# martinruenz/maskfusion

Hardware: AMD Instinct MI355X
Metric: frames/sec (640x480 RGB-D, single background model, ICP + surfel fusion) (higher is better)
Workload: dtype f32; 1 GPU; configs[1]: synthetic 640x480 RGB-D stream (S1: 600 frames, Kinect-like noise), 1 background model per GPU, icpWeight=100 (geometric ICP 4/5/10 iterations) + surfel fusion, empty masks; frames_in_hbm=600, models=1, surfels=429320, parallelism=context-per-gpu x1

## Files before the change

### maskfusion_amd/api.py

```python
from __future__ import annotations

import ctypes as C
import numpy as np

from .lib import load, MFError, Config, ModelInfo, RenderView, MF_N_TIMINGS, TIMING_LABELS, MF_N_PASSES, PASS_LABELS


class Model:

    def __init__(self, owner: "MaskFusion", index: int):
        self._o = owner
        self._i = index

    def info(self) -> ModelInfo:
        out = ModelInfo()
        self._o._chk(self._o._L.mf_model_info(self._o._h, self._i, C.byref(out)))
        return out

    def getID(self) -> int:
        return int(self.info().id)

    def getClassID(self) -> int:
        return int(self.info().class_id)

# ... 219 lines not shown

    def getBackgroundModel(self) -> Model:
        return Model(self, 0)

    def getModels(self):
        n = C.c_int32(0)
        self._chk(self._L.mf_num_models(self._h, C.byref(n)))
        return [Model(self, i) for i in range(n.value)]

    def getCurrPose(self) -> np.ndarray:
        return self.getBackgroundModel().getPose()

    def downloadSegmentation(self) -> np.ndarray:
        out = np.zeros((self.height, self.width), np.uint8)
        self._chk(self._L.mf_download_segmentation(self._h, out.ctypes.data))
        return out

    def exportSegmentation(self, path: str):
        self._chk(self._L.mf_export_segmentation_png(self._h, path.encode()))

    def getLastFillIn(self) -> bool:
        u = C.c_int32(0)
        self._chk(self._L.mf_get_last_fillin(self._h, C.byref(u)))
        return bool(u.value)

    def setParam(self, key: str, value: float):
        self._chk(self._L.mf_set_param(self._h, key.encode(), float(value)))

    def getParam(self, key: str) -> float:
        v = C.c_double(0)
        self._chk(self._L.mf_get_param(self._h, key.encode(), C.byref(v)))
        return v.value

    def setDepthCutoff(self, v): self.setParam("depthCutoff", v)
    def setIcpWeight(self, v): self.setParam("icpWeight", v)
    def setConfidenceThreshold(self, v): self.setParam("confidenceThreshold", v)
    def setOutlierCoefficient(self, v): self.setParam("outlierCoefficient", v)
    def setFastOdom(self, v): self.setParam("fastOdom", int(v))
    def setSo3(self, v): self.setParam("so3", int(v))
    def setFrameToFrameRGB(self, v): self.setParam("frameToFrameRGB", int(v))
    def setRgbOnly(self, v): self.setParam("rgbOnly", int(v))

    def trackStats(self, model: int = 0) -> dict:
        out = np.zeros(8, np.float32)
        self._chk(self._L.mf_get_track_stats(self._h, model, out.ctypes.data))
        keys = ("lastICPError", "lastICPCount", "lastRGBError", "lastRGBCount", "lastSO3Error", "lastSO3Count", "so3Iterations",
                "rejected")
        return dict(zip(keys, out.tolist()))
    def gnIllIterations(self, model: int = 0) -> int:
        n = C.c_int32(0)
        self._chk(self._L.mf_get_gn_condition(self._h, model, C.byref(n)))
        return n.value

    def setPyramid(self, v): self.setParam("pyramid", int(v))
    def setEnableMultipleModels(self, v): self.setParam("enableMultipleModels", int(v))

    def enableTimings(self, on=True):
        self.setParam("timings", 1 if on else 0)

    def timings(self) -> dict:
        t = np.zeros(MF_N_TIMINGS, np.float32)
        self._chk(self._L.mf_get_timings(self._h, t.ctypes.data))
        return dict(zip(TIMING_LABELS, t.tolist()))

    def passTimings(self) -> dict:
        t = np.zeros(MF_N_PASSES, np.float32)
        self._chk(self._L.mf_get_pass_timings(self._h, t.ctypes.data))
        return dict(zip(PASS_LABELS, t.tolist()))

    def stream(self) -> int:
        return int(self._L.mf_get_stream(self._h) or 0)

    def inputStream(self) -> int:
        return int(self._L.mf_get_input_stream(self._h) or 0)

    def defaultRenderView(self, width: int = 1280, height: int = 980, icl: bool = False) -> RenderView:
        v = RenderView()
        self._chk(self._L.mf_default_render_view(self._h, int(width), int(height), int(bool(icl)), C.byref(v)))
        return v

    def sensorRenderView(self) -> RenderView:
        v = RenderView()
        self._chk(self._L.mf_sensor_render_view(self._h, C.byref(v)))
        return v

    @staticmethod
    def defaultPalette() -> np.ndarray:
        L, n = load(), C.c_int32(0)
        if L.mf_default_palette(None, 0, C.byref(n)) != 0:
            raise MFError("mf_default_palette failed")
        out = np.zeros((n.value, 3), np.float32)
        if L.mf_default_palette(out.ctypes.data, n.value, C.byref(n)) != 0:
            raise MFError("mf_default_palette failed")
        return out

    def renderView(self, view: RenderView | None = None, palette=None, depth: bool = False, models: bool = False):
        if view is None:
            view = self.defaultRenderView()
        H, W = int(view.height), int(view.width)
        rgba = np.zeros((max(H, 1), max(W, 1), 4), np.uint8)
        dep = np.zeros((max(H, 1), max(W, 1)), np.float32) if depth else None
        mod = np.zeros((max(H, 1), max(W, 1)), np.int32) if models else None
        if palette is None:
            pal_ptr, n_pal = None, 0
        else:
            pal = np.ascontiguousarray(np.asarray(palette, np.float32).reshape(-1, 3))
            n_pal = len(pal)
            if n_pal == 0:
                pal = np.zeros((1, 3), np.float32)
            pal_ptr = pal.ctypes.data
        self._chk(self._L.mf_render_view(self._h, C.byref(view), pal_ptr, n_pal, rgba.ctypes.data,
                                         dep.ctypes.data if dep is not None else None, mod.ctypes.data if mod is not None else None))
        out = [rgba]
        if depth:
            out.append(dep)
        if models:
            out.append(mod)
        return out[0] if len(out) == 1 else tuple(out)

    def renderViewDevice(self, view: RenderView, d_rgba: int, d_depth: int = 0, d_model: int = 0, palette=None):
        pal_ptr, n_pal, keep = None, 0, None
        if palette is not None:
            keep = np.ascontiguousarray(np.asarray(palette, np.float32).reshape(-1, 3))
            pal_ptr, n_pal = keep.ctypes.data, len(keep)
        self._chk(self._L.mf_render_view_dev(self._h, C.byref(view), pal_ptr, n_pal, d_rgba, d_depth or None, d_model or None))

    def modelCloudNN(self, model: int, points, radius: float, transform=None, confThreshold=None):
        import torch
        from .lib import torch_device
        as_numpy = not isinstance(points, torch.Tensor)
        q = torch.as_tensor(np.ascontiguousarray(points, np.float32)) if as_numpy else points
        if q.dtype != torch.float32 or q.dim() != 2 or q.shape[1] < 3:
            raise MFError("modelCloudNN: points must be (n, >= 3) float32")
        q = q.to(torch_device()).contiguous()
        n = int(q.shape[0])
        dist = torch.empty(max(n, 1), dtype=torch.float32, device=q.device)
        idx = torch.empty(max(n, 1), dtype=torch.int32, device=q.device)
        thr = Model(self, model).getConfidenceThreshold() if confThreshold is None else float(confThreshold)
        T = None if transform is None else np.ascontiguousarray(np.asarray(transform, np.float32).T.reshape(16))
        if q.device.type == "cuda":
            torch.cuda.current_stream(q.device).synchronize()
        self._chk(self._L.mf_model_cloud_nn_dev(self._h, int(model), thr, q.data_ptr() if n else None, int(q.shape[1]), n,
                                                T.ctypes.data if T is not None else None, float(radius), dist.data_ptr(), idx.data_ptr()))
        dist, idx = dist[:n], idx[:n]
        if as_numpy:
            return dist.cpu().numpy(), idx.cpu().numpy()
        return dist, idx

    def debugRead(self, what: str, model: int = 0, count: int | None = None) -> np.ndarray:
        W, H = self.width, self.height
        shapes = {"depthF": ((H, W), np.float32), "pred_vertex": ((H, W, 4), np.float32),
                  "pred_normal": ((H, W, 4), np.float32), "pred_image": ((H, W, 4), np.uint8), "pred_time": ((H, W), np.uint16),
                  "index": ((H, W), np.int32), "index_vc": ((H, W, 4), np.float32), "index_nr": ((H, W, 4), np.float32),
                  "index_ct": ((H, W, 4), np.float32), "index_packed": ((W, H, 2, 4), np.float32), "icp_log": ((19, 32), np.float32), "gn_trace": ((20, 64), np.float64),
                  "icp_prof": ((19, 16), np.uint64), "splat_prof": ((((H + 15) // 16) * ((W + 15) // 16), 8), np.uint64),
                  "edge_map": ((H, W), np.float32),
                  "edge_binary": ((H, W), np.uint8), "projected_ids": ((H, W), np.uint8)}
        for i in range(3):
            shapes.update({f"gray{i}": ((H >> i, W >> i), np.uint8), f"dIdx{i}": ((H >> i, W >> i), np.int16), f"dIdy{i}": ((H >> i, W >> i), np.int16),
                           f"rgb_gate{i}": ((H >> i, W >> i), np.uint8)})
        if count is not None:
            shapes.update({"cand_op": ((count,), np.uint8), "cand_rec": ((count, 12), np.float32),
                           "clean_flags": ((count,), np.uint8), "clean_newconf": ((count,), np.float32)})
        for pre in ("vmap_g", "nmap_g", "vmap", "nmap"):
            for i in range(3):
                shapes[f"{pre}{i}"] = ((3, H >> i, W >> i), np.float32)
        shape, dt = shapes[what]
        out = np.zeros(shape, dt)
        self._chk(self._L.mf_debug_read_model(self._h, model, what.encode(), out.ctypes.data, out.nbytes))
        return out
```

### maskfusion_amd/csrc/mf_context.hip

```cpp
#include "../../include/maskfusion_amd.h"
#include "mf_internal.h"
#include "mf_labels.h"

#include <float.h>
#include <math.h>
#include <algorithm>
#include <cmath>
#include <stdio.h>
#include <string.h>
#include <memory>
#include <chrono>
#include <string>
#include <vector>

using namespace mf;

namespace {

struct SurfelBufferState {
    int cur = 0;
    bool table_valid = false;
    bool sparse = false;
    long phys_ub = -1, runs_ub = -1;
    unsigned clean_seq = 0, mirror_from = 1;
    unsigned gen = 0;

    void reset_empty() { became_dense(0); }
    void became_dense(int live) { cur = live; sparse = false; table_valid = false; phys_ub = runs_ub = -1; mirror_from = clean_seq + 1; gen++; }
    void fresh_table(int live, long n) { became_dense(live); table_valid = true; exact_count(n); }
    void exact_count(long n) { phys_ub = n; runs_ub = (n + kRun - 1) / kRun; }
    void table_built() { table_valid = true; gen++; }
    void cleaned_in_place(long cand_max, long new_runs_max) { sparse = true; table_valid = true; phys_ub += cand_max; runs_ub += new_runs_max; clean_seq++; gen++; }
    void touched() { gen++; }
};

struct ModelState : SurfelBufferState {
    int id = 0, classID = -1;
    bool isStatic = true, allowFillIn = false;
    unsigned age = 0;
    float confThr = 0.f, maxDepth = FLT_MAX;
    Surfels surf[2];
    int cap = 0;
    unsigned long long* h_append = nullptr;
    PoseDev* d_pose = nullptr; FrameDev* d_frame = nullptr;
    float4* d_predV = nullptr; float4* d_predN = nullptr; uchar4* d_predImage = nullptr; uint16_t* d_predTime = nullptr;
    uint8_t* d_predGray = nullptr; uint8_t* d_fillGray = nullptr;
    bool pred_gray_valid = false;
    float* d_vmap_g[3] = {}; float* d_nmap_g[3] = {}; GNState* d_gn = nullptr; float* d_partials[2] = {nullptr, nullptr};
    TrackModelDev* d_track = nullptr;
    int* d_track_rect = nullptr;
    float* d_icp_log = nullptr;
    double* d_gn_trace = nullptr;
    struct ObjScratch {
        unsigned long long* keys = nullptr; int* index = nullptr; float4* ivc = nullptr; float4* inr = nullptr; float4* iclean = nullptr;
        uint8_t* cand_op = nullptr; float4* cand_rec = nullptr; int* upd_first = nullptr; int* cand_best = nullptr;
        int* clean_ctl = nullptr;
        uint8_t* flags = nullptr; float* newconf = nullptr; int* block_counts = nullptr;
    } scr;
    float* d_poselog = nullptr;
    std::vector<int64_t> log_ts;
    PoseDev* h_pose = nullptr; FrameDev* h_frame = nullptr; int* h_count = nullptr;
    TrackModelDev track_host;
    std::vector<void*> allocs;
    ~ModelState() {
        for (void* p : allocs) (void)hipFree(p);
        if (h_pose) (void)hipHostFree(h_pose);
        if (h_frame) (void)hipHostFree(h_frame);
        if (h_count) (void)hipHostFree(h_count);
        if (h_append) (void)hipHostFree(h_append);
    }
};

struct LabelsScratch {
    int P = 0, table_cap = 0;
    uint8_t* ignoreMap = nullptr; uint8_t* tmp_u8 = nullptr;
    int* L = nullptr; int* compId = nullptr; int* area = nullptr; int* lab[2] = {nullptr, nullptr}; int* blockCounts = nullptr;
    int4* bbox = nullptr;
    int* compMask = nullptr; int* compModel = nullptr; int* compToMask = nullptr; int* compFollow = nullptr;
    unsigned* overlap = nullptr; void* tables = nullptr;
    int* d_small = nullptr;
    const PoseDev** d_poses = nullptr;
    int* h_small = nullptr; const PoseDev** h_poses = nullptr; int* h_result = nullptr;
    std::vector<void*> dev, host;
    ~LabelsScratch() {
        for (void* p : dev) (void)hipFree(p);
        for (void* p : host) (void)hipHostFree(p);
    }
    template <typename T> bool dalloc(T** p, size_t n) {
        void* q = nullptr;
        if (hipMalloc(&q, n * sizeof(T)) != hipSuccess) return false;
        if (hipMemset(q, 0, n * sizeof(T)) != hipSuccess) return false;
        dev.push_back(q); *p = reinterpret_cast<T*>(q);
        return true;
    }
    template <typename T> bool halloc(T** p, size_t n) {
        void* q = nullptr;
        if (hipHostMalloc(&q, n * sizeof(T)) != hipSuccess) return false;
        memset(q, 0, n * sizeof(T));
        host.push_back(q); *p = reinterpret_cast<T*>(q);
        return true;
    }
    bool init(int P_) {
        P = P_;
        table_cap = 8 << 20;
        return dalloc(&ignoreMap, (size_t)P) && dalloc(&tmp_u8, (size_t)P) && dalloc(&L, (size_t)P) && dalloc(&compId, (size_t)P) &&
               dalloc(&area, (size_t)P + 1) && dalloc(&bbox, (size_t)P + 1) && dalloc(&lab[0], (size_t)P) && dalloc(&lab[1], (size_t)P) &&
               dalloc(&blockCounts, (size_t)(P + 255) / 256) && dalloc(&compMask, (size_t)table_cap) &&
               dalloc(&compModel, (size_t)table_cap) && dalloc(&compToMask, (size_t)P + 1) && dalloc(&compFollow, (size_t)P + 1) &&
               dalloc(&overlap, (size_t)64 * 256) && dalloc((char**)&tables, labels_gpu_table_bytes()) && dalloc(&d_small, 384) &&
               dalloc(&d_poses, 64) && halloc(&h_small, 384) && halloc(&h_poses, 64) && halloc(&h_result, 4);
    }
    int enqueue(const SegParams& prm, int W, int H, const uint8_t* d_binary, const float* d_depth, const uint8_t* d_mask,
                const int32_t* class_ids, int n_masks, const uint8_t* d_proj, const std::vector<SegModelInfo>& models,
                const std::vector<const PoseDev*>& poses, int nextModelID, bool allowNew, uint8_t* d_full, hipStream_t s) {
        if (models.size() > 64 || n_masks > 256) return MF_EINVAL;
        memset(h_small, 0, 384 * sizeof(int));
        for (int k = 0; k < n_masks; ++k) h_small[k] = class_ids[k];
        for (size_t m = 0; m < models.size(); ++m) { h_small[256 + m] = models[m].id; h_small[320 + m] = models[m].classID; h_poses[m] = poses[m]; }
        if (hipMemcpyAsync(d_small, h_small, 384 * sizeof(int), hipMemcpyHostToDevice, s) != hipSuccess ||
            hipMemcpyAsync(d_poses, h_poses, 64 * sizeof(PoseDev*), hipMemcpyHostToDevice, s) != hipSuccess)
            return MF_EHIP;
        LabelsGpuArgs a;
        a.prm = prm; a.W = W; a.H = H; a.binary = d_binary; a.depth = d_depth; a.mask = d_mask; a.proj = d_proj;
        a.class_ids = d_small; a.nMasks = n_masks; a.model_ids = d_small + 256; a.model_cls = d_small + 320; a.model_poses = d_poses;
        a.nModels = (int)models.size(); a.nextModelID = nextModelID; a.allowNew = allowNew; a.ignoreMap = ignoreMap; a.full = d_full;
        a.tmp_u8 = tmp_u8; a.L = L; a.compId = compId; a.area = area; a.bbox = bbox; a.lab[0] = lab[0]; a.lab[1] = lab[1]; a.blockCounts = blockCounts;
        a.compMask = compMask; a.compModel = compModel; a.table_cap = table_cap; a.compToMask = compToMask; a.compFollow = compFollow;
        a.overlap = overlap; a.tables = tables; a.result_host = h_result;
        launch_labels_gpu(a, s);
        return MF_OK;
    }
};

}

struct RenderScratch;
static void render_free(RenderScratch* r);
struct EvalScratch;
static void eval_free(EvalScratch* e);

struct mf_ctx {
    mf_config cfg;
    int W, H, P;
    Intr K;
    hipStream_t stream = nullptr;
    bool clean_literal = true;
    bool global_tiles = true;
    bool early_bg_fusion = true;
    hipEvent_t ev_labels = nullptr;
    long frame_no = 0;
    long bg_fused_frame = -1;
    bool labels_pending = false;
    int lastF = 0;
    std::string err;
    int host_tick = 1;
    bool map_ready = false;
    bool tracked_once = false;
    bool timings_on = false, icp_prof_on = false;
    bool object_small_grids = true;
    bool object_scatter_splat = true;
#ifndef MF_DEFAULT_LITERAL_FUSION_WEIGHT
#define MF_DEFAULT_LITERAL_FUSION_WEIGHT 1
#endif
    bool weight_literal = MF_DEFAULT_LITERAL_FUSION_WEIGHT != 0;
    bool bbox_limit = true;
    bool batch_objects = true;
    static constexpr int kObjArgSlots = 8;
    ObjPassArgs* d_obj_args[kObjArgSlots] = {}; ObjPassArgs* h_obj_args[kObjArgSlots] = {}; hipEvent_t ev_obj_args[kObjArgSlots] = {};
    unsigned obj_arg_slot = 0;
    bool fused_preprocess = true;
    bool object_stream = true;
    hipStream_t stream_obj = nullptr, obj_s = nullptr;
    hipEvent_t ev_obj_dep = nullptr, ev_obj_done = nullptr;
    bool obj_dep_main = false;
    uint8_t* d_maskT_obj = nullptr;
    bool ftf_rgb = false;
    double host_us[5] = {0, 0, 0, 0, 0}; long host_calls = 0;
    bool host_lockstep = true;
    bool host_wait_upload = true;

    uint8_t* d_rgb = nullptr; float* d_depth = nullptr; uint8_t* d_mask_in = nullptr; uint8_t* d_zero_mask = nullptr;
    bool host_async = true;
    hipStream_t stream_in = nullptr;
    uint8_t* h_in[2] = {nullptr, nullptr};
    uint8_t* d_in_block[2] = {nullptr, nullptr};
    size_t in_off_rgb = 0, in_off_mask = 0, in_bytes = 0;
    uint8_t* d_in_rgb[2] = {}; float* d_in_depth[2] = {}; uint8_t* d_in_mask[2] = {};
    hipEvent_t ev_in_copied[2] = {nullptr, nullptr};
    hipEvent_t ev_in_consumed[2] = {nullptr, nullptr};
    unsigned in_slot = 0;
    uint8_t* d_mask_tex = nullptr;
    float* d_depthF[3] = {nullptr, nullptr, nullptr};
    float* d_vmap[2][3] = {}; float* d_nmap[2][3] = {};
    uint8_t* d_gray[2][3] = {};
    long gray_frame[2] = {-1, -1};
    long deriv_frame = -1;
    int16_t* d_dIdx[3] = {}; int16_t* d_dIdy[3] = {}; uint8_t* d_rgb_gate[3] = {};
    float* d_lastDepth[3] = {}; uint8_t* d_lastImage[3] = {};
    RgbCorr* d_corres = nullptr; float* d_rgb_partials[2] = {nullptr, nullptr}; int2* d_cnt[2] = {nullptr, nullptr};
    So3Result* d_so3 = nullptr; char* d_so3_scratch = nullptr;
    SplatTuning splat_tune;
    int* d_tile_count = nullptr; int* d_tile_entries = nullptr; int tile_entries_cap = 0; int tile_entries_alloc = 0; int splat_tiles = 1;
    float4* d_splat_rec0 = nullptr; float4* d_splat_rec1 = nullptr; uint2* d_splat_bbox = nullptr;
    const uint8_t* cur_rgb = nullptr;
    const float* cur_depth = nullptr;
    bool batch_solve_fused = true;
    int batch_tracking = 1;
    int model_api_packed = 0;
    std::vector<int32_t> mask_classes;
    std::vector<int> trackable;
    struct RetiredLog { int id; std::vector<int64_t> ts; std::vector<float> p; size_t arena_off = 0, n = 0; bool in_arena = false; };
    std::vector<RetiredLog> retired;
    float* d_retired = nullptr; size_t retired_cap = 0, retired_used = 0;
    std::vector<std::unique_ptr<ModelState>> pool;
    unsigned long long* d_keys = nullptr;
    int* d_index = nullptr; float4* d_ivc = nullptr; float4* d_ict = nullptr; float4* d_inr = nullptr;
    float4* d_iclean = nullptr;
    uint8_t* d_maskT = nullptr;
    uint8_t* d_cand_op = nullptr; float4* d_cand_rec = nullptr; int* d_upd_first = nullptr;
    uint8_t* d_flags = nullptr; float* d_newconf = nullptr; int* d_block_counts = nullptr;
    int* d_cand_best = nullptr;
    int* d_clean_ctl = nullptr;
    int* d_clean_list = nullptr; int* d_clean_count = nullptr;
    int* d_decay_stats = nullptr;
    int* d_run_offs = nullptr;
    int* d_vis_list = nullptr; int* d_vis_count = nullptr; int* d_cull_ctl = nullptr; int vis_max_runs = 0;
    struct { const void* model = nullptr; long frame = -1; int cur = -1; unsigned gen = 0; float max_depth = 0.f; int time_delta = 0; } vis_tag;
    int densify_count = 0;
    bool fused_rgb_pyramid = true;
    float2* d_row_z = nullptr;
    bool slab_culling = true;
    int densify_every = 0;
    bool cull_runs = true;
    int big_map_elements = 6000000;
    int in_place_elements = 1000000;
    unsigned long long* d_icp_prof = nullptr;
    unsigned long long* d_splat_prof = nullptr; bool splat_prof_on = false;
    float* d_edge = nullptr; uint8_t* d_bin = nullptr; uint8_t* d_tmp_u8 = nullptr; uint8_t* d_proj_ids = nullptr;
    uint8_t* h_bin = nullptr; uint8_t* h_ids = nullptr; float* h_depth = nullptr; uint8_t* h_mask = nullptr; uint8_t* h_full = nullptr;
    std::vector<uint8_t> ignoreMap;
    std::unique_ptr<LabelsScratch> labels;
    int gpu_labels = 1;
    SegParams seg;
    int nextID = 0, spawnOffset = 0;
    int cap_max = 0;

    std::vector<std::unique_ptr<ModelState>> models;

    hipEvent_t ev[MF_N_TIMINGS + 1] = {};
    hipEvent_t ev_mm[5] = {};
    bool mm_marked = false; float mm_host_wait_ms = 0.f;
    hipEvent_t ev_icp[2] = {nullptr, nullptr};
    bool pass_timings_on = false;
    hipEvent_t ev_pass[MF_N_PASSES][2] = {};
    bool pass_recorded[MF_N_PASSES] = {};
    float pass_ms[MF_N_PASSES] = {};
    hipEvent_t ev_icp_mid = nullptr;
    bool icp_mid_recorded = false;
    float last_ms[MF_N_TIMINGS] = {};
    std::vector<void*> allocs;
    std::vector<void*> host_allocs;
    RenderScratch* render = nullptr;
    EvalScratch* eval = nullptr;
};

#define MF_HIP(ctx, call)                                                                         \
    do {                                                                                          \
        hipError_t e_ = (call);                                                                   \
        if (e_ != hipSuccess) {                                                                   \
            char buf_[512];                                                                       \
            snprintf(buf_, sizeof(buf_), "%s failed: %s (%s:%d)", #call, hipGetErrorString(e_), __FILE__, __LINE__); \
            if (ctx) (ctx)->err = buf_;                                                           \
            return MF_EHIP;                                                                       \
        }                                                                                         \
    } while (0)

template <typename T>
static int dev_alloc(mf_ctx* c, std::vector<void*>& owner, T** p, size_t n, int fill = 0) {
    void* q = nullptr;
    MF_HIP(c, hipMalloc(&q, n * sizeof(T)));
    MF_HIP(c, hipMemsetAsync(q, fill, n * sizeof(T), c->stream));
    owner.push_back(q);
    *p = reinterpret_cast<T*>(q);
    return MF_OK;
}
template <typename T>
static int host_alloc(mf_ctx* c, T** p, size_t n) {
    void* q = nullptr;
    MF_HIP(c, hipHostMalloc(&q, n * sizeof(T)));
    memset(q, 0, n * sizeof(T));
    c->host_allocs.push_back(q);
    *p = reinterpret_cast<T*>(q);
    return MF_OK;
}

extern "C" int mf_default_config(mf_config* cfg, int32_t width, int32_t height, float fx, float fy, float cx, float cy) {
    if (!cfg) return MF_EINVAL;
    memset(cfg, 0, sizeof(*cfg));
    cfg->width = width; cfg->height = height; cfg->fx = fx; cfg->fy = fy; cfg->cx = cx; cfg->cy = cy;
    cfg->device = 0;
    cfg->time_delta = 200; cfg->conf_global = 4.f; cfg->conf_object = 2.f; cfg->depth_cutoff = 3.f;
    cfg->icp_weight = 10.f; cfg->fast_odom = 0; cfg->so3 = 1; cfg->pyramid = 1; cfg->max_depth_processed = 20.f;
    cfg->outlier_coefficient = 0.9f;
    cfg->num_gsurfels = 9437184; cfg->num_osurfels = 1048576;
    cfg->enable_multiple_models = 1;
    cfg->model_spawn_offset = 20; cfg->track_all_models = 1; cfg->max_models = 32;
    cfg->rgb_only = 0;
    cfg->pose_log_capacity = 65536;
    return MF_OK;
}

static __global__ void k_set_weight_literal(PoseDev* p, int literal, PoseDev* host_mirror) {
    if (threadIdx.x != 0 || blockIdx.x != 0) return;
    p->weightLiteral = literal;
    if (host_mirror) host_mirror->weightLiteral = literal;
}
static __global__ void k_pose_identity(PoseDev* p, int weight_literal) {
    if (threadIdx.x != 0 || blockIdx.x != 0) return;
    PoseDev q;
    memset(&q, 0, sizeof(q));
    q.weightLiteral = weight_literal;
    for (int k = 0; k < 9; ++k) q.R[k] = q.Ri[k] = q.lastR[k] = q.initR[k] = (k % 4 == 0) ? 1.f : 0.f;
    q.fusionWeight = 1.f;
    q.alive = 1;
    *p = q;
}
static __global__ void k_frame_init(FrameDev* f, int tick) {
// ... 48 lines not shown
    }
    A(dev_alloc(c, m->allocs, &m->d_pose, 1));
    A(dev_alloc(c, m->allocs, &m->d_frame, 1));
    A(dev_alloc(c, m->allocs, &m->d_predV, P));
    A(dev_alloc(c, m->allocs, &m->d_predN, P));
    A(dev_alloc(c, m->allocs, &m->d_predImage, P));
    A(dev_alloc(c, m->allocs, &m->d_predTime, P));
    A(dev_alloc(c, m->allocs, &m->d_predGray, P));
    if (allowFillIn) A(dev_alloc(c, m->allocs, &m->d_fillGray, P));
    if (c->cfg.pose_log_capacity > 0) A(dev_alloc(c, m->allocs, &m->d_poselog, (size_t)c->cfg.pose_log_capacity * 8));
    for (int i = 0; i < 3; ++i) {
        const size_t lp = (size_t)(c->W >> i) * (c->H >> i);
        A(dev_alloc(c, m->allocs, &m->d_vmap_g[i], lp * 3));
        A(dev_alloc(c, m->allocs, &m->d_nmap_g[i], lp * 3));
    }
    {
        int nbm = icp_batch_max_blocks(c->W, c->H);
        for (int i = 0; i < 3; ++i) nbm = std::max(nbm, std::max(icp_grid_blocks(c->W >> i, c->H >> i), icp_geo_grid_blocks(c->W >> i, c->H >> i)));
        const size_t nbmax = (size_t)nbm;
        for (int b = 0; b < 2; ++b) A(dev_alloc(c, m->allocs, &m->d_partials[b], nbmax * kIcpSlots));
    }
    A(dev_alloc(c, m->allocs, &m->d_gn, 2));
    A(dev_alloc(c, m->allocs, &m->d_track, 1));
    A(dev_alloc(c, m->allocs, &m->d_track_rect, 12));
    A(dev_alloc(c, m->allocs, &m->d_icp_log, (size_t)20 * 32));
    A(dev_alloc(c, m->allocs, &m->d_gn_trace, (size_t)20 * kGnTraceRow));
    if (!allowFillIn && with_scratch) A(ensure_obj_scratch(c, *m));
#undef A
    {
        TrackModelDev t;
        memset(&t, 0, sizeof(t));
        t.predV = m->d_predV; t.predN = m->d_predN; t.pose = m->d_pose; t.frame = m->d_frame;
        for (int i = 0; i < 3; ++i) { t.vm[i] = m->d_vmap_g[i]; t.nm[i] = m->d_nmap_g[i]; }
        t.partials[0] = m->d_partials[0]; t.partials[1] = m->d_partials[1]; t.st = m->d_gn;
        t.log = m->d_icp_log;
        t.trace = m->d_gn_trace;
        t.jump_limit = allowFillIn ? 0.f : 0.2f;
        t.allow_fill = allowFillIn ? 1 : 0;
        t.rect = m->d_track_rect;
        m->track_host = t;
    }
    hipLaunchKernelGGL(k_pose_identity, dim3(1), dim3(64), 0, c->stream, m->d_pose, c->weight_literal ? 1 : 0);
    hipLaunchKernelGGL(k_frame_init, dim3(1), dim3(64), 0, c->stream, m->d_frame, c->host_tick);
    if (hipHostMalloc((void**)&m->h_pose, sizeof(PoseDev)) != hipSuccess || hipHostMalloc((void**)&m->h_frame, sizeof(FrameDev)) != hipSuccess ||
        hipHostMalloc((void**)&m->h_count, sizeof(int)) != hipSuccess || hipHostMalloc((void**)&m->h_append, sizeof(unsigned long long)) != hipSuccess)
        return MF_ENOMEM;
    *m->h_append = 0ull;
    memset(m->h_pose, 0, sizeof(PoseDev));
    for (int k = 0; k < 9; ++k) m->h_pose->R[k] = m->h_pose->Ri[k] = (k % 4 == 0) ? 1.f : 0.f;
    m->h_pose->alive = 1;
    m->h_pose->fusionWeight = 1.f;
    m->h_pose->weightLiteral = c->weight_literal ? 1 : 0;
    memset(m->h_frame, 0, sizeof(FrameDev));
    m->h_frame->tick = c->host_tick;
    *m->h_count = 0;
    m->track_host.pose_host = m->h_pose;
    MF_HIP(c, hipMemcpyAsync(m->d_track, &m->track_host, sizeof(TrackModelDev), hipMemcpyHostToDevice, c->stream));
    {
        int armed[12];
        for (int q = 0; q < 12; ++q) armed[q] = (q & 2) ? (int)0x80000000 : 0x7FFFFFFF;
        MF_HIP(c, hipMemcpyAsync(m->d_track_rect, armed, sizeof(armed), hipMemcpyHostToDevice, c->stream));
    }
    MF_HIP(c, hipStreamSynchronize(c->stream));
    out = std::move(m);
    return MF_OK;
}

extern "C" int mf_create(const mf_config* cfg, mf_ctx** out) {
    if (!cfg || !out) return MF_EINVAL;
    *out = nullptr;
    if (cfg->width <= 0 || cfg->height <= 0 || (cfg->width % 8) || (cfg->height % 8)) return MF_EINVAL;
    int ndev = 0;
    if (hipGetDeviceCount(&ndev) != hipSuccess || ndev <= 0 || cfg->device >= ndev) return MF_ENODEV;
    mf_ctx* c = new mf_ctx();
    c->cfg = *cfg;
    if (c->cfg.model_spawn_offset <= 0) c->cfg.model_spawn_offset = 20;
    if (c->cfg.max_models <= 0) c->cfg.max_models = 32;
    c->W = cfg->width; c->H = cfg->height; c->P = c->W * c->H;
    c->K = Intr{cfg->fx, cfg->fy, cfg->cx, cfg->cy};
    auto fail = [&](int code) { mf_destroy(c); return code; };
    if (hipSetDevice(cfg->device) != hipSuccess) return fail(MF_ENODEV);
    if (hipStreamCreateWithFlags(&c->stream, hipStreamNonBlocking) != hipSuccess) return fail(MF_ENODEV);
    const int W = c->W, H = c->H, P = c->P;
    const int cap_bg = surfel_capacity(cfg->num_gsurfels), cap_obj = surfel_capacity(cfg->num_osurfels);
    if (cap_bg <= 0 || cap_obj <= 0) return fail(MF_EINVAL);
    c->cap_max = cap_bg > cap_obj ? cap_bg : cap_obj;
    int rc = MF_OK;
#define A(call) do { rc = (call); if (rc != MF_OK) return fail(rc); } while (0)
    auto up256 = [](size_t v) { return (v + 255) & ~(size_t)255; };
    c->in_off_rgb = up256((size_t)P * sizeof(float));
    c->in_off_mask = up256(c->in_off_rgb + (size_t)P * 3);
    c->in_bytes = up256(c->in_off_mask + (size_t)P);
    for (int i = 0; i < 2; ++i) {
        A(dev_alloc(c, c->allocs, &c->d_in_block[i], c->in_bytes));
        c->d_in_depth[i] = reinterpret_cast<float*>(c->d_in_block[i]);
        c->d_in_rgb[i] = c->d_in_block[i] + c->in_off_rgb;
        c->d_in_mask[i] = c->d_in_block[i] + c->in_off_mask;
    }
    c->d_rgb = c->d_in_rgb[0]; c->d_depth = c->d_in_depth[0]; c->d_mask_in = c->d_in_mask[0];
    for (int i = 0; i < 2; ++i) {
        A(host_alloc(c, &c->h_in[i], c->in_bytes));
        if (hipEventCreateWithFlags(&c->ev_in_copied[i], hipEventDisableTiming) != hipSuccess ||
            hipEventCreateWithFlags(&c->ev_in_consumed[i], hipEventDisableTiming) != hipSuccess) return fail(MF_EHIP);
    }
    if (hipStreamCreateWithFlags(&c->stream_in, hipStreamNonBlocking) != hipSuccess) return fail(MF_EHIP);
    if (hipStreamCreateWithFlags(&c->stream_obj, hipStreamNonBlocking) != hipSuccess) return fail(MF_EHIP);
    if (hipEventCreateWithFlags(&c->ev_obj_dep, hipEventDisableTiming) != hipSuccess ||
        hipEventCreateWithFlags(&c->ev_obj_done, hipEventDisableTiming) != hipSuccess) return fail(MF_EHIP);
    c->obj_s = c->stream;
    A(dev_alloc(c, c->allocs, &c->d_zero_mask, (size_t)P));
    A(dev_alloc(c, c->allocs, &c->d_mask_tex, (size_t)P));
    for (int b = 0; b < 3; ++b) A(dev_alloc(c, c->allocs, &c->d_depthF[b], (size_t)P));
    for (int i = 0; i < 3; ++i) {
        const size_t lp = (size_t)(W >> i) * (H >> i);
        for (int set = 0; set < 2; ++set) {
            A(dev_alloc(c, c->allocs, &c->d_vmap[set][i], lp * 3));
            A(dev_alloc(c, c->allocs, &c->d_nmap[set][i], lp * 3));
        }
    }
    for (int i = 0; i < 3; ++i) {
        const size_t lp = (size_t)(W >> i) * (H >> i);
        for (int set = 0; set < 2; ++set) A(dev_alloc(c, c->allocs, &c->d_gray[set][i], lp));
        A(dev_alloc(c, c->allocs, &c->d_dIdx[i], lp));
        A(dev_alloc(c, c->allocs, &c->d_dIdy[i], lp));
        A(dev_alloc(c, c->allocs, &c->d_rgb_gate[i], lp));
        A(dev_alloc(c, c->allocs, &c->d_lastDepth[i], lp));
        A(dev_alloc(c, c->allocs, &c->d_lastImage[i], lp));
    }
    A(dev_alloc(c, c->allocs, &c->d_corres, (size_t)P));
    for (int b = 0; b < 2; ++b) {
        A(dev_alloc(c, c->allocs, &c->d_rgb_partials[b], (size_t)icp_grid_blocks(W, H) * kIcpSlots));
        A(dev_alloc(c, c->allocs, &c->d_cnt[b], (size_t)icp_grid_blocks(W, H)));
    }
    A(dev_alloc(c, c->allocs, &c->d_so3, 1));
    A(dev_alloc(c, c->allocs, &c->d_so3_scratch, so3_scratch_bytes(W >> 2, H >> 2)));
    {
        const size_t nt = splat_tiles_scratch_ints(W, H);
        const size_t maxcap = (size_t)std::max(surfel_capacity(cfg->num_gsurfels), surfel_capacity(cfg->num_osurfels));
        A(dev_alloc(c, c->allocs, &c->d_tile_count, nt));
        c->tile_entries_cap = (int)std::min<size_t>(std::max<size_t>(4 * maxcap, (size_t)16 * P), (size_t)1 << 30);
        c->tile_entries_alloc = c->tile_entries_cap;
        A(dev_alloc(c, c->allocs, &c->d_tile_entries, (size_t)c->tile_entries_cap));
        A(dev_alloc(c, c->allocs, &c->d_splat_rec0, maxcap));
        A(dev_alloc(c, c->allocs, &c->d_splat_rec1, maxcap));
        A(dev_alloc(c, c->allocs, &c->d_splat_bbox, maxcap));
    }
    A(dev_alloc(c, c->allocs, &c->d_keys, (size_t)P, 0xFF));
    A(dev_alloc(c, c->allocs, &c->d_index, (size_t)P));
    A(dev_alloc(c, c->allocs, &c->d_ivc, (size_t)P));
    A(dev_alloc(c, c->allocs, &c->d_ict, (size_t)P));
    A(dev_alloc(c, c->allocs, &c->d_iclean, (size_t)P * 2));
    A(dev_alloc(c, c->allocs, &c->d_maskT, (size_t)P));
    A(dev_alloc(c, c->allocs, &c->d_maskT_obj, (size_t)P));
    A(dev_alloc(c, c->allocs, &c->d_inr, (size_t)P));
    A(dev_alloc(c, c->allocs, &c->d_cand_op, (size_t)P));
    A(dev_alloc(c, c->allocs, &c->d_cand_rec, (size_t)P * 3));
    A(dev_alloc(c, c->allocs, &c->d_upd_first, (size_t)c->cap_max));
    A(dev_alloc(c, c->allocs, &c->d_flags, (size_t)c->cap_max + P));
    A(dev_alloc(c, c->allocs, &c->d_newconf, (size_t)c->cap_max + P));
    A(dev_alloc(c, c->allocs, &c->d_block_counts, (size_t)kCompactBlocks));
    A(dev_alloc(c, c->allocs, &c->d_cand_best, (size_t)P));
    A(dev_alloc(c, c->allocs, &c->d_clean_ctl, (size_t)kCleanCtlInts));
    A(dev_alloc(c, c->allocs, &c->d_row_z, (size_t)(c->H + (c->H >> 1) + (c->H >> 2))));
    c->vis_max_runs = (int)run_table_runs((long)c->cap_max, (long)P);
    A(dev_alloc(c, c->allocs, &c->d_vis_list, (size_t)c->vis_max_runs));
    A(dev_alloc(c, c->allocs, &c->d_clean_list, (size_t)c->vis_max_runs));
    A(dev_alloc(c, c->allocs, &c->d_clean_count, 1));
    A(dev_alloc(c, c->allocs, &c->d_run_offs, (size_t)c->vis_max_runs + 1));
    A(dev_alloc(c, c->allocs, &c->d_decay_stats, (size_t)kDecayStats + 3));
    launch_arm_decay_stats(c->d_decay_stats, c->stream);
    A(dev_alloc(c, c->allocs, &c->d_vis_count, 1));
    A(dev_alloc(c, c->allocs, &c->d_cull_ctl, 2));
    A(dev_alloc(c, c->allocs, &c->d_icp_prof, (size_t)20 * 16));
    A(dev_alloc(c, c->allocs, &c->d_edge, (size_t)P));
    A(dev_alloc(c, c->allocs, &c->d_bin, (size_t)P));
    A(dev_alloc(c, c->allocs, &c->d_tmp_u8, (size_t)P));
    A(dev_alloc(c, c->allocs, &c->d_proj_ids, (size_t)P));
    A(host_alloc(c, &c->h_bin, (size_t)P));
    A(host_alloc(c, &c->h_ids, (size_t)P));
    A(host_alloc(c, &c->h_depth, (size_t)P));
    A(host_alloc(c, &c->h_mask, (size_t)P));
    A(host_alloc(c, &c->h_full, (size_t)P));
    launch_fill_int(c->d_upd_first, kNoUpdate, c->cap_max, c->stream);
    std::unique_ptr<ModelState> bg;
    A(create_model(c, c->nextID++, cfg->conf_global, true, cap_bg, bg));
    c->models.push_back(std::move(bg));
#undef A
    c->ignoreMap.assign(P, 0);
    c->labels.reset(new LabelsScratch());
    if (!c->labels->init(P)) return fail(MF_ENOMEM);
    for (int i = 0; i <= MF_N_TIMINGS; ++i)
        if (hipEventCreate(&c->ev[i]) != hipSuccess) return fail(MF_EHIP);
    for (int i = 0; i < 2; ++i)
        if (hipEventCreate(&c->ev_icp[i]) != hipSuccess) return fail(MF_EHIP);
    for (int i = 0; i < 5; ++i)
        if (hipEventCreate(&c->ev_mm[i]) != hipSuccess) return fail(MF_EHIP);
    if (hipEventCreate(&c->ev_icp_mid) != hipSuccess) return fail(MF_EHIP);
    for (int i = 0; i < mf_ctx::kObjArgSlots; ++i) {
        if (hipMalloc((void**)&c->d_obj_args[i], sizeof(ObjPassArgs) * 64) != hipSuccess ||
            hipHostMalloc((void**)&c->h_obj_args[i], sizeof(ObjPassArgs) * 64) != hipSuccess ||
            hipEventCreateWithFlags(&c->ev_obj_args[i], hipEventDisableTiming) != hipSuccess)
            return fail(MF_ENOMEM);
    }
    if (hipStreamSynchronize(c->stream) != hipSuccess) return fail(MF_EHIP);
    *out = c;
    return MF_OK;
}

extern "C" void mf_destroy(mf_ctx* c) {
    if (!c) return;
    if (c->stream) (void)hipStreamSynchronize(c->stream);
    c->models.clear();
    if (c->render) render_free(c->render);
    if (c->eval) eval_free(c->eval);
    for (void* p : c->allocs) (void)hipFree(p);
    if (c->d_splat_prof) (void)hipFree(c->d_splat_prof);
    for (void* p : c->host_allocs) (void)hipHostFree(p);
    for (int i = 0; i <= MF_N_TIMINGS; ++i)
        if (c->ev[i]) (void)hipEventDestroy(c->ev[i]);
    for (int i = 0; i < 2; ++i) {
        if (c->ev_icp[i]) (void)hipEventDestroy(c->ev_icp[i]);
        for (int q = 0; q < MF_N_PASSES; ++q) if (c->ev_pass[q][i]) (void)hipEventDestroy(c->ev_pass[q][i]);
    }
    if (c->ev_icp_mid) (void)hipEventDestroy(c->ev_icp_mid);
    for (int i = 0; i < 5; ++i)
        if (c->ev_mm[i]) (void)hipEventDestroy(c->ev_mm[i]);
    if (c->ev_labels) (void)hipEventDestroy(c->ev_labels);
    for (int i = 0; i < 2; ++i) {
        if (c->ev_in_copied[i]) (void)hipEventDestroy(c->ev_in_copied[i]);
        if (c->ev_in_consumed[i]) (void)hipEventDestroy(c->ev_in_consumed[i]);
    }
    if (c->stream_in) { (void)hipStreamSynchronize(c->stream_in); (void)hipStreamDestroy(c->stream_in); }
    if (c->stream_obj) { (void)hipStreamSynchronize(c->stream_obj); (void)hipStreamDestroy(c->stream_obj); }
    if (c->ev_obj_dep) (void)hipEventDestroy(c->ev_obj_dep);
    if (c->ev_obj_done) (void)hipEventDestroy(c->ev_obj_done);
    for (int i = 0; i < mf_ctx::kObjArgSlots; ++i) {
        if (c->d_obj_args[i]) (void)hipFree(c->d_obj_args[i]);
        if (c->h_obj_args[i]) (void)hipHostFree(c->h_obj_args[i]);
        if (c->ev_obj_args[i]) (void)hipEventDestroy(c->ev_obj_args[i]);
    }
    if (c->stream) (void)hipStreamDestroy(c->stream);
    delete c;
}

extern "C" const char* mf_last_error(const mf_ctx* c) { return c ? c->err.c_str() : "null context"; }

#include "mf_frame.inl"

extern "C" int mf_preallocate_models(mf_ctx* c, uint32_t count) {
    if (!c) return MF_EINVAL;
    for (uint32_t i = 0; i < count; ++i) {
        std::unique_ptr<ModelState> m;
        int rc = create_model(c, -1, c->cfg.conf_object, false, surfel_capacity(c->cfg.num_osurfels), m, c->batch_objects);
        if (rc != MF_OK) return rc;
        c->pool.push_back(std::move(m));
    }
    return check_launch(c);
}

static __global__ void k_set_tick(FrameDev* f, int tick, FrameDev* host_mirror) {
    if (threadIdx.x != 0 || blockIdx.x != 0) return;
    f->tick = tick;
    if (host_mirror) *host_mirror = *f;
}
extern "C" int mf_set_tick(mf_ctx* c, int32_t tick) {
    if (!c || tick < 1) return MF_EINVAL;
    if (!c->map_ready && tick != 1) { c->err = "setTick before the first frame would skip the map initialisation"; return MF_ESTATE; }
    c->host_tick = tick;
    for (auto& m : c->models) hipLaunchKernelGGL(k_set_tick, dim3(1), dim3(64), 0, c->stream, m->d_frame, tick, m->h_frame);
    return check_launch(c);
}

#include "mf_model_api.inl"

extern "C" int mf_get_tick(mf_ctx* c, int32_t* tick) {
    if (!c || !tick) return MF_EINVAL;
    *tick = c->host_tick;
    return MF_OK;
}
extern "C" int mf_num_models(mf_ctx* c, int32_t* n) {
    if (!c || !n) return MF_EINVAL;
    *n = (int32_t)c->models.size();
    return MF_OK;
}
static ModelState* model_at(mf_ctx* c, int32_t i) {
    if (!c || i < 0 || i >= (int32_t)c->models.size()) return nullptr;
    return c->models[i].get();
}
extern "C" int mf_get_model_ids(mf_ctx* c, int32_t* ids, int32_t capacity, int32_t* n) {
    if (!c || !ids || !n || capacity < (int32_t)c->models.size()) return MF_EINVAL;
    for (size_t i = 0; i < c->models.size(); ++i) ids[i] = c->models[i]->id;
    *n = (int32_t)c->models.size();
    return MF_OK;
}
extern "C" int mf_get_pose(mf_ctx* c, int32_t model, float* out) {
    ModelState* m = model_at(c, model);
    if (!m || !out) return MF_EINVAL;
    int rc = mf_sync(c);
    if (rc != MF_OK) return rc;
    const PoseDev& p = *m->h_pose;
    for (int r = 0; r < 3; ++r) {
        for (int col = 0; col < 3; ++col) out[col * 4 + r] = p.R[r * 3 + col];
        out[12 + r] = p.t[r];
        out[r * 4 + 3] = 0.f;
    }
    out[15] = 1.f;
// ... 188 lines not shown
    for (int y = 0; y < H; ++y) {
        raw.push_back(0);
        raw.insert(raw.end(), img + (size_t)y * W, img + (size_t)(y + 1) * W);
    }
    std::vector<uint8_t> z = {0x78, 0x01};
    uint32_t a = 1, b = 0;
    for (uint8_t v : raw) { a = (a + v) % 65521u; b = (b + a) % 65521u; }
    for (size_t off = 0; off < raw.size(); off += 65535) {
        const size_t n = std::min<size_t>(65535, raw.size() - off);
        z.push_back(off + n == raw.size() ? 1 : 0);
        z.push_back((uint8_t)(n & 255)); z.push_back((uint8_t)(n >> 8));
        z.push_back((uint8_t)(~n & 255)); z.push_back((uint8_t)((~n >> 8) & 255));
        z.insert(z.end(), raw.begin() + off, raw.begin() + off + n);
    }
    const uint32_t adler = (b << 16) | a;
    for (int k = 3; k >= 0; --k) z.push_back((uint8_t)(adler >> (8 * k)));
    std::vector<uint8_t> f = {0x89, 'P', 'N', 'G', 0x0D, 0x0A, 0x1A, 0x0A};
    std::vector<uint8_t> hdr;
    for (uint32_t v : {(uint32_t)W, (uint32_t)H}) for (int k = 3; k >= 0; --k) hdr.push_back((uint8_t)(v >> (8 * k)));
    hdr.insert(hdr.end(), {8, 0, 0, 0, 0});
    png_chunk(f, "IHDR", hdr);
    png_chunk(f, "IDAT", z);
    png_chunk(f, "IEND", {});
    FILE* fp = fopen(path, "wb");
    if (!fp) return MF_EINVAL;
    const bool ok = fwrite(f.data(), 1, f.size(), fp) == f.size();
    fclose(fp);
    return ok ? MF_OK : MF_EINVAL;
}
extern "C" int mf_export_segmentation_png(mf_ctx* c, const char* path) {
    if (!c || !path) return MF_EINVAL;
    std::vector<uint8_t> img((size_t)c->P);
    int rc = mf_download_segmentation(c, img.data());
    if (rc != MF_OK) return rc;
    for (auto& v : img) v = v > 254 ? 0 : v;
    rc = mf_write_png_gray8(path, img.data(), c->W, c->H);
    if (rc != MF_OK) c->err = std::string("cannot write ") + path;
    return rc;
}

extern "C" int mf_download_map(mf_ctx* c, int32_t model, float* out, uint32_t max_count, uint32_t* count) {
    ModelState* ms = model_at(c, model);
    if (!ms || !out || !count) return MF_EINVAL;
    require_dense(c, *ms);
    int rc = mf_sync(c);
    if (rc != MF_OK) return rc;
    const uint32_t n = (uint32_t)*ms->h_count;
    *count = n;
    const uint32_t m = n < max_count ? n : max_count;
    if (m == 0) return MF_OK;
    std::vector<float4> a(m), b(m), d(m);
    const Surfels& s = ms->surf[ms->cur];
    MF_HIP(c, hipMemcpy(a.data(), s.pc, m * sizeof(float4), hipMemcpyDeviceToHost));
    MF_HIP(c, hipMemcpy(b.data(), s.ct, m * sizeof(float4), hipMemcpyDeviceToHost));
    MF_HIP(c, hipMemcpy(d.data(), s.nr, m * sizeof(float4), hipMemcpyDeviceToHost));
    for (uint32_t i = 0; i < m; ++i) {
        memcpy(out + (size_t)i * 12, &a[i], 16);
        memcpy(out + (size_t)i * 12 + 4, &b[i], 16);
        memcpy(out + (size_t)i * 12 + 8, &d[i], 16);
    }
    return MF_OK;
}

struct ParamRef { const char* key; int kind; size_t off; };
static const ParamRef kParams[] = {
    {"depthCutoff", 0, offsetof(mf_config, depth_cutoff)},
    {"icpWeight", 0, offsetof(mf_config, icp_weight)},
    {"outlierCoefficient", 0, offsetof(mf_config, outlier_coefficient)},
    {"maxDepthProcessed", 0, offsetof(mf_config, max_depth_processed)},
    {"fastOdom", 1, offsetof(mf_config, fast_odom)},
    {"so3", 1, offsetof(mf_config, so3)},
    {"rgbOnly", 1, offsetof(mf_config, rgb_only)},
    {"pyramid", 1, offsetof(mf_config, pyramid)},
    {"timeDelta", 1, offsetof(mf_config, time_delta)},
    {"enableMultipleModels", 1, offsetof(mf_config, enable_multiple_models)},
    {"trackAllModels", 1, offsetof(mf_config, track_all_models)},
    {"modelSpawnOffset", 1, offsetof(mf_config, model_spawn_offset)},
};
struct SegRef { const char* key; int kind; size_t off; };
static const SegRef kSegParams[] = {
    {"mfThreshold", 0, offsetof(SegParams, threshold)},
    {"mfWeightDistance", 0, offsetof(SegParams, weightDistance)},
    {"mfWeightConvexity", 0, offsetof(SegParams, weightConvexity)},
    {"mfMorphEdgeIterations", 1, offsetof(SegParams, morphEdgeIterations)},
    {"mfMorphEdgeRadius", 1, offsetof(SegParams, morphEdgeRadius)},
    {"mfMorphMaskIterations", 1, offsetof(SegParams, morphMaskIterations)},
    {"mfMorphMaskRadius", 1, offsetof(SegParams, morphMaskRadius)},
    {"newModelMinRelativeSize", 0, offsetof(SegParams, minRelSizeNew)},
    {"newModelMaxRelativeSize", 0, offsetof(SegParams, maxRelSizeNew)},
};

extern "C" int mf_set_param(mf_ctx* c, const char* key, double value) {
    if (!c || !key) return MF_EINVAL;
    if (!strcmp(key, "hostProfileReset")) { for (double& v : c->host_us) v = 0; c->host_calls = 0; return MF_OK; }
    if (!strcmp(key, "timings")) { c->timings_on = value != 0; return MF_OK; }
    if (!strcmp(key, "passTimings")) {
        c->pass_timings_on = value != 0;
        for (int q = 0; q < MF_N_PASSES; ++q) { c->pass_recorded[q] = false; c->pass_ms[q] = 0.f; }
        return MF_OK;
    }
    if (!strcmp(key, "icpProfile")) { c->icp_prof_on = value != 0; return MF_OK; }
    if (!strcmp(key, "hostInputAsync")) {
        if (hipStreamSynchronize(c->stream) != hipSuccess || hipStreamSynchronize(c->stream_in) != hipSuccess) return MF_EHIP;
        c->host_async = value != 0; return MF_OK;
    }
    if (!strcmp(key, "hostLockstep")) { c->host_lockstep = value != 0; return MF_OK; }
    if (!strcmp(key, "hostWaitUpload")) { c->host_wait_upload = value != 0; return MF_OK; }
    if (!strcmp(key, "splatProfile")) {
        if (value != 0 && !c->d_splat_prof) {
            if (hipMalloc(&c->d_splat_prof, splat_tiles_scratch_ints(c->W, c->H) * 8 * sizeof(unsigned long long)) != hipSuccess) return MF_ENOMEM;
        }
        c->splat_prof_on = value != 0;
        return MF_OK;
    }
    if (!strcmp(key, "gpuLabels")) { c->gpu_labels = value != 0; return MF_OK; }
    if (!strcmp(key, "splatTiles")) { c->splat_tiles = value != 0; return MF_OK; }
    if (!strcmp(key, "splatTileEntries")) {
        const long long v = (long long)value;
        if (v < 1 || v > c->tile_entries_alloc) return MF_EINVAL;
        c->tile_entries_cap = (int)v;
        return MF_OK;
    }
    if (!strcmp(key, "batchTracking")) { c->batch_tracking = value != 0; return MF_OK; }
    if (!strcmp(key, "frameToFrameRGB")) { c->ftf_rgb = value != 0; return MF_OK; }
    if (!strcmp(key, "batchSolveInPixelPass")) { c->batch_solve_fused = value != 0; return MF_OK; }
    if (!strcmp(key, "fusedPreprocessLaunch")) { c->fused_preprocess = value != 0; return MF_OK; }
    if (!strcmp(key, "objectStream")) { c->object_stream = value != 0; return MF_OK; }
    if (!strcmp(key, "batchObjectPasses")) { c->batch_objects = value != 0; return MF_OK; }
    if (!strcmp(key, "objectBoundingBoxLimit")) { c->bbox_limit = value != 0; return MF_OK; }
    if (!strcmp(key, "literalFusionWeight")) {
        c->weight_literal = value != 0;
        for (auto& m : c->models) hipLaunchKernelGGL(k_set_weight_literal, dim3(1), dim3(64), 0, c->stream, m->d_pose, c->weight_literal ? 1 : 0, m->h_pose);
        for (auto& m : c->pool) hipLaunchKernelGGL(k_set_weight_literal, dim3(1), dim3(64), 0, c->stream, m->d_pose, c->weight_literal ? 1 : 0, m->h_pose);
        return check_launch(c);
    }
    if (!strcmp(key, "objectSmallGrids")) { c->object_small_grids = value != 0; return MF_OK; }
    if (!strcmp(key, "objectScatterSplat")) { c->object_scatter_splat = value != 0; return MF_OK; }
    if (!strcmp(key, "globalTiles")) { c->global_tiles = value != 0; return MF_OK; }
    if (!strcmp(key, "cullRuns")) { c->cull_runs = value != 0; c->vis_tag.model = nullptr; return MF_OK; }
    if (!strcmp(key, "densifyEvery")) { c->densify_every = (int)value; return MF_OK; }
    if (!strcmp(key, "slabCulling")) { c->slab_culling = value != 0; return MF_OK; }
    if (!strcmp(key, "bigMapElements")) { c->big_map_elements = (int)value; c->vis_tag.model = nullptr; return MF_OK; }
    if (!strcmp(key, "fusedRgbPyramid")) { c->fused_rgb_pyramid = value != 0; return MF_OK; }
    if (!strcmp(key, "inPlaceElements")) { c->in_place_elements = (int)value; return MF_OK; }
    if (!strcmp(key, "rebuildRunTable")) {
        ModelState& bg = *c->models[0];
        require_dense(c, bg);
        MF_HIP(c, hipStreamSynchronize(c->stream));
        launch_run_table(bg.surf[bg.cur], bg.d_frame, c->stream);
        bg.fresh_table(bg.cur, (long)*bg.h_count);
        c->vis_tag.model = nullptr;
        return check_launch(c);
    }
    if (!strcmp(key, "cleanLiteralWindow")) { c->clean_literal = value != 0; return MF_OK; }
    if (!strcmp(key, "earlyBackgroundFusion")) { c->early_bg_fusion = value != 0; return MF_OK; }
    if (!strcmp(key, "modelApiPackedIndex")) { c->model_api_packed = value != 0; return MF_OK; }
    if (!strcmp(key, "tileHeight")) { c->splat_tune.tile_h = (int)value; return MF_OK; }
    if (!strcmp(key, "tileThreads")) { c->splat_tune.tile_threads = (int)value; return MF_OK; }
    if (!strcmp(key, "spriteLanes")) { c->splat_tune.sprite_lanes = (int)value; return MF_OK; }
    if (!strcmp(key, "confidenceThreshold")) { c->cfg.conf_global = (float)value; c->models[0]->confThr = (float)value; return MF_OK; }
    for (const ParamRef& p : kParams)
        if (!strcmp(key, p.key)) {
            char* base = reinterpret_cast<char*>(&c->cfg);
            if (p.kind == 0) *reinterpret_cast<float*>(base + p.off) = (float)value;
            else *reinterpret_cast<int32_t*>(base + p.off) = (int32_t)value;
            return MF_OK;
        }
    for (const SegRef& p : kSegParams)
        if (!strcmp(key, p.key)) {
            char* base = reinterpret_cast<char*>(&c->seg);
            if (p.kind == 0) *reinterpret_cast<float*>(base + p.off) = (float)value;
            else *reinterpret_cast<int*>(base + p.off) = (int)value;
            return MF_OK;
        }
    c->err = std::string("unknown parameter: ") + key;
    return MF_EINVAL;
}
extern "C" int mf_get_param(mf_ctx* c, const char* key, double* value) {
    if (!c || !key || !value) return MF_EINVAL;
    if (!strcmp(key, "confidenceThreshold")) { *value = c->models[0]->confThr; return MF_OK; }
    if (!strcmp(key, "splatTileEntries")) { *value = c->tile_entries_cap; return MF_OK; }
    if (!strcmp(key, "cullRuns")) { *value = c->cull_runs ? 1 : 0; return MF_OK; }
    if (!strcmp(key, "densifyCount")) { *value = (float)c->densify_count; return MF_OK; }
    if (!strcmp(key, "unstampedRuns")) {
        MF_HIP(c, hipStreamSynchronize(c->stream));
        ModelState& bg = *c->models[0];
        FrameDev f; MF_HIP(c, hipMemcpy(&f, bg.d_frame, sizeof(FrameDev), hipMemcpyDeviceToHost));
        const size_t cap_runs = run_table_runs((long)bg.cap, (long)c->P);
        const size_t runs = bg.table_valid ? std::min((size_t)std::max(f.runs, 0), cap_runs) : 0;
        std::vector<int4> box(kBoxStride * runs);
        if (runs) MF_HIP(c, hipMemcpy(box.data(), bg.surf[bg.cur].box, box.size() * sizeof(int4), hipMemcpyDeviceToHost));
        int v = 0;
        for (size_t r = 0; r < runs; ++r) v += (box[kBoxStride * r + 2].x > 0 && box[kBoxStride * r + 2].z != 0) ? 1 : 0;
        *value = v;
        return MF_OK;
    }
    if (!strcmp(key, "visibleRuns") || !strcmp(key, "backgroundRuns") || !strcmp(key, "cleanRuns")) {
        MF_HIP(c, hipStreamSynchronize(c->stream));
        int v = 0;
        if (!strcmp(key, "visibleRuns")) MF_HIP(c, hipMemcpy(&v, c->d_vis_count, sizeof(int), hipMemcpyDeviceToHost));
        else if (!strcmp(key, "cleanRuns")) MF_HIP(c, hipMemcpy(&v, c->d_clean_count, sizeof(int), hipMemcpyDeviceToHost));
        else { FrameDev f; MF_HIP(c, hipMemcpy(&f, c->models[0]->d_frame, sizeof(FrameDev), hipMemcpyDeviceToHost)); v = f.runs; }
        *value = v;
        return MF_OK;
    }
    if (!strcmp(key, "hostStageUs")) { *value = c->host_calls ? c->host_us[0] / c->host_calls : 0; return MF_OK; }
    if (!strcmp(key, "hostUploadUs")) { *value = c->host_calls ? c->host_us[1] / c->host_calls : 0; return MF_OK; }
    if (!strcmp(key, "hostEnqueueUs")) { *value = c->host_calls ? c->host_us[2] / c->host_calls : 0; return MF_OK; }
    if (!strcmp(key, "hostCallUs")) { *value = c->host_calls ? c->host_us[3] / c->host_calls : 0; return MF_OK; }
    if (!strcmp(key, "hostWaitUs")) { *value = c->host_calls ? c->host_us[4] / c->host_calls : 0; return MF_OK; }
    if (!strcmp(key, "frameToFrameRGB")) { *value = c->ftf_rgb ? 1 : 0; return MF_OK; }
    if (!strcmp(key, "objectBoundingBoxLimit")) { *value = c->bbox_limit ? 1 : 0; return MF_OK; }
    for (const ParamRef& p : kParams)
        if (!strcmp(key, p.key)) {
            const char* base = reinterpret_cast<const char*>(&c->cfg);
            *value = p.kind == 0 ? (double)*reinterpret_cast<const float*>(base + p.off) : (double)*reinterpret_cast<const int32_t*>(base + p.off);
            return MF_OK;
        }
    for (const SegRef& p : kSegParams)
        if (!strcmp(key, p.key)) {
            const char* base = reinterpret_cast<const char*>(&c->seg);
            *value = p.kind == 0 ? (double)*reinterpret_cast<const float*>(base + p.off) : (double)*reinterpret_cast<const int*>(base + p.off);
            return MF_OK;
        }
    return MF_EINVAL;
}

extern "C" int mf_get_timings(mf_ctx* c, float* ms) {
    if (!c || !ms) return MF_EINVAL;
    int rc = mf_sync(c);
    if (rc != MF_OK) return rc;
    memcpy(ms, c->last_ms, sizeof(c->last_ms));
    return MF_OK;
}
extern "C" int mf_get_pass_timings(mf_ctx* c, float* ms) {
    if (!c || !ms) return MF_EINVAL;
    int rc = mf_sync(c);
    if (rc != MF_OK) return rc;
    memcpy(ms, c->pass_ms, sizeof(c->pass_ms));
    return MF_OK;
}
extern "C" void* mf_get_stream(mf_ctx* c) { return c ? (void*)c->stream : nullptr; }
extern "C" void* mf_get_input_stream(mf_ctx* c) { return c ? (void*)c->stream : nullptr; }

static int debug_read_impl(mf_ctx* c, ModelState& mdl, const char* what, void* out, uint64_t out_bytes) {
    int rc = mf_sync(c);
    if (rc != MF_OK) return rc;
    const void* src = nullptr;
    size_t bytes = 0;
    bool variable = false;
    const size_t P = (size_t)c->P;
    std::string w(what);
    auto lvl = [&](const std::string& pre, float* const arr[3]) -> bool {
        for (int i = 0; i < 3; ++i)
            if (w == pre + std::to_string(i)) {
                src = arr[i]; bytes = (size_t)(c->W >> i) * (c->H >> i) * 3 * sizeof(float);
                return true;
            }
        return false;
    };
    const int lastSet = (int)((c->frame_no + 1) & 1);
    auto img = [&](const std::string& pre, const void* const arr[3], size_t elem) -> bool {
        for (int i = 0; i < 3; ++i)
            if (w == pre + std::to_string(i)) {
                src = arr[i]; bytes = (size_t)(c->W >> i) * (c->H >> i) * elem;
                return true;
            }
        return false;
    };
    const void* const gray3[3] = {c->d_gray[lastSet][0], c->d_gray[lastSet][1], c->d_gray[lastSet][2]};
    const void* const dx3[3] = {c->d_dIdx[0], c->d_dIdx[1], c->d_dIdx[2]}, * const dy3[3] = {c->d_dIdy[0], c->d_dIdy[1], c->d_dIdy[2]};
    const void* const gate3[3] = {c->d_rgb_gate[0], c->d_rgb_gate[1], c->d_rgb_gate[2]};
    if (w == "depthF") { src = c->d_depthF[c->lastF]; bytes = P * 4; }
    else if (img("gray", gray3, 1) || img("dIdx", dx3, 2) || img("dIdy", dy3, 2) || img("rgb_gate", gate3, 1)) {}
    else if (lvl("vmap_g", mdl.d_vmap_g) || lvl("nmap_g", mdl.d_nmap_g) || lvl("vmap", c->d_vmap[lastSet]) || lvl("nmap", c->d_nmap[lastSet])) {}
    else if (w == "pred_vertex") { src = mdl.d_predV; bytes = P * 16; }
    else if (w == "pred_normal") { src = mdl.d_predN; bytes = P * 16; }
    else if (w == "pred_image") { src = mdl.d_predImage; bytes = P * 4; }
    else if (w == "pred_time") { src = mdl.d_predTime; bytes = P * 2; }
    else if (w == "index") { src = c->d_index; bytes = P * 4; }
    else if (w == "index_vc") { src = c->d_ivc; bytes = P * 16; }
    else if (w == "index_nr") { src = c->d_inr; bytes = P * 16; }
    else if (w == "index_ct") { src = c->d_ict; bytes = P * 16; }
    else if (w == "index_packed") { src = c->d_iclean; bytes = P * 32; }
    else if (w == "cand_op") { src = c->d_cand_op; bytes = P; variable = true; }
    else if (w == "cand_rec") { src = c->d_cand_rec; bytes = P * 48; variable = true; }
    else if (w == "clean_flags") { src = c->d_flags; bytes = (size_t)c->cap_max + P; variable = true; }
    else if (w == "clean_newconf") { src = c->d_newconf; bytes = ((size_t)c->cap_max + P) * 4; variable = true; }
    else if (w == "icp_log") { src = mdl.d_icp_log; bytes = 19 * 32 * 4; }
    else if (w == "gn_trace") { src = mdl.d_gn_trace; bytes = 20 * kGnTraceRow * 8; }
    else if (w == "icp_prof") { src = c->d_icp_prof; bytes = 19 * 16 * 8; }
    else if (w == "splat_prof") {
        if (!c->d_splat_prof) { c->err = "splat_prof: switch splatProfile on first"; return MF_ESTATE; }
        src = c->d_splat_prof; bytes = splat_tiles_scratch_ints(c->W, c->H) * 8 * 8;
    }
    else if (w == "edge_map") { src = c->d_edge; bytes = P * 4; }
    else if (w == "edge_binary") { src = c->d_bin; bytes = P; }
    else if (w == "projected_ids") { src = c->d_proj_ids; bytes = P; }
    else { c->err = "unknown debug tap: " + w; return MF_EINVAL; }
    if (variable) bytes = out_bytes < bytes ? (size_t)out_bytes : bytes;
    if (out_bytes < bytes) { c->err = "debug_read: buffer too small"; return MF_EINVAL; }
    MF_HIP(c, hipMemcpy(out, src, bytes, hipMemcpyDeviceToHost));
    return MF_OK;
}
extern "C" int mf_debug_read(mf_ctx* c, const char* what, void* out, uint64_t out_bytes) {
    if (!c || !what || !out) return MF_EINVAL;
    return debug_read_impl(c, *c->models[0], what, out, out_bytes);
}
extern "C" int mf_debug_read_model(mf_ctx* c, int32_t model, const char* what, void* out, uint64_t out_bytes) {
    ModelState* m = model_at(c, model);
    if (!m || !what || !out) return MF_EINVAL;
    return debug_read_impl(c, *m, what, out, out_bytes);
}

#include "mf_ktest.inl"
#include "mf_render.inl"
#include "mf_eval.inl"
```

### maskfusion_amd/csrc/mf_internal.h

```cpp
#pragma once

#include <hip/hip_runtime.h>
#include <stdint.h>

namespace mf {

constexpr int kLevels = 3;
constexpr int kIcpSlots = 32;
constexpr int kCompactBlocks = 2048;
constexpr unsigned long long kEmptyKey = 0xFFFFFFFFFFFFFFFFull;
constexpr int kNoUpdate = 0x7FFFFFFF;

struct Intr {
    float fx, fy, cx, cy;
};

struct PoseDev {
    float R[9], t[3];
    float Ri[9], ti[3];
    float lastR[9], lastT[3];
    float fusionWeight;
    float lastICPError, lastICPCount;
    float initR[9], initT[3];
    float incT[3];
// ... 30 lines not shown
    int runs;
    int cover;
    int useFillIn;
    int pad[3];
    int bbox[6], bbox_acc[6];
    int bbox_tmp[6];
    int phys;
    int first;
    int runsNext;
    int first_run;
    unsigned long long done_cover;
};

constexpr int kBBoxEmptyMin = 100000, kBBoxEmptyMax = -100000;
constexpr int kBBoxNotRun = 0x7FFFFFFF;
#define MF_FRAME_BBOX_RESET(f) do { for (int q_ = 0; q_ < 3; ++q_) { (f)->bbox[q_] = (f)->bbox_acc[q_] = (f)->bbox_tmp[q_] = mf::kBBoxEmptyMin; \
                                                                     (f)->bbox[3 + q_] = (f)->bbox_acc[3 + q_] = (f)->bbox_tmp[3 + q_] = mf::kBBoxEmptyMax; } \
                                    (f)->bbox_acc[0] = mf::kBBoxNotRun; } while (0)
#define MF_FRAME_BBOX_ADVANCE(f) do { if ((f)->bbox_acc[0] != mf::kBBoxNotRun) for (int q_ = 0; q_ < 6; ++q_) (f)->bbox[q_] = (f)->bbox_acc[q_]; \
                                      (f)->bbox_acc[0] = mf::kBBoxNotRun; } while (0)

struct Surfels {
    float4* pc;
    float4* ct;
    float4* nr;
    int cap;
    int4* box;
};
constexpr int kRun = 512;
constexpr int kBoxStride = 3;
__host__ __device__ inline int run_start(const int4* box, int r) { return box[kBoxStride * r + 1].w; }
__host__ __device__ inline int run_len(const int4* box, int r) { return box[kBoxStride * r + 2].x; }
struct VisList { const int* list; const int* count; };
constexpr int kBoxEmptyMin = 0x7FFFFFFF, kBoxEmptyMax = (int)0x80000000;

struct TrackModelDev {
    const float4* predV; const float4* predN;
    PoseDev* pose; PoseDev* pose_host; const FrameDev* frame;
    float* vm[3]; float* nm[3];
    float* partials[2]; GNState* st;
    float* log;
    double* trace;
    float jump_limit;
    int allow_fill;
    int* rect;
};
constexpr int kMaxTrackBatch = 32;
constexpr int kGnTraceRow = 64;
struct TrackBatch { const TrackModelDev* m[kMaxTrackBatch]; int n; };

void launch_bilateral_model_pyramid(const float* depth, float* depthF, const float4* predV, const float4* predN, const float* fillDepth,
                                    const FrameDev* frame, const PoseDev* pose, float* const vmaps[3], float* const nmaps[3], int W, int H, Intr k,
                                    hipStream_t s);
void launch_bilateral(const float* depth, float* out, int W, int H, hipStream_t s);
void launch_pyrdown_f(const float* src, float* dst, int sw, int sh, hipStream_t s);
void launch_vmap_nmap(const float* depth, float* vmap, float* nmap, int W, int H, Intr k, float cutoff, hipStream_t s);
void launch_frame_pyramid(const float* depth, float* const vmap[3], float* const nmap[3], int W, int H, Intr k, float cutoff,
                          hipStream_t s);

void launch_model_pyramid(const float4* predV, const float4* predN, const float* fillDepth, const FrameDev* frame,
                          const PoseDev* pose, const float* R9t3_host_or_null, float* const vmaps[3],
                          float* const nmaps[3], int W, int H, Intr k, hipStream_t s);
struct IcpLaunch {
    const float* vmap_curr; const float* nmap_curr; const float* vmap_prev; const float* nmap_prev;
    int W, H; Intr k;
    float distThres, angleThres;
    const float* partials_in; int nblocks_in;
    float* partials_out;
    const GNState* state_in; GNState* state_out;
    float* log_out;
    double* trace = nullptr; int it = 0;
    unsigned long long* prof_out = nullptr;
    const PoseDev* pose_in = nullptr;
    const So3Result* so3_in = nullptr;
};
int icp_grid_blocks(int W, int H);
int icp_geo_grid_blocks(int W, int H);
void launch_icp_iteration(const IcpLaunch& a, hipStream_t s);
int icp_batch_max_blocks(int W, int H);
int icp_batch_blocks(int W, int H, int n_models);
void launch_model_pyramid_batch(const TrackBatch& b, const float* fillDepth, int W, int H, Intr k, hipStream_t s);
void launch_bilateral_model_pyramid_batch(const float* depth, float* depthF, const TrackBatch& b, const float* fillDepth, int W, int H, Intr k,
                                          hipStream_t s);
void launch_icp_batch_solve(const TrackBatch& b, int it, int nb_in, const So3Result* so3_or_null, hipStream_t s);
void launch_icp_batch_pixels(const TrackBatch& b, int it, int level, const float* vmap_curr, const float* nmap_curr, int W, int H, Intr k,
                             float distThres, float angleThres, hipStream_t s, const float2* row_z = nullptr, bool fused = false, int nb_in = 0,
                             const So3Result* so3_or_null = nullptr);
void launch_row_zrange(const float* const vmap[3], int W, int H, float2* out, hipStream_t s);
void launch_icp_batch_finalize(const TrackBatch& b, int n_it, int nb_in, const So3Result* so3_or_null, hipStream_t s);
void launch_icp_finalize(const float* partials_in, int nblocks_in, const GNState* state_in, PoseDev* pose,
                         PoseDev* host_mirror, float* log_out, float jump_limit, const So3Result* so3, hipStream_t s,
                         double* trace = nullptr, int n_it = 0);
void launch_icp_step_standalone(const float* Rcurr, const float* tcurr, const float* vc, const float* nc,
                                const float* Rpi, const float* tprev, Intr k, const float* vp, const float* np,
                                float distThres, float angleThres, int W, int H, float* partials, GNState* st2,
                                float* out32, hipStream_t s);

struct RgbCorr { int16_t u0, v0; float diff; };

struct RgbLevel {
    const int16_t* dIdx; const int16_t* dIdy;
    const float* lastDepth; const float* nextDepth;
    const uint8_t* lastImage; const uint8_t* nextImage;
    int W, H;
    float minScale;
    float maxDepthDelta;
    const uint8_t* gate;
};

void launch_intensity(const uint8_t* img, int channels, uint8_t* dst, int n, hipStream_t s);
void launch_pyrdown_u8(const uint8_t* src, uint8_t* dst, int sw, int sh, hipStream_t s);
void launch_derivative(const uint8_t* src, int16_t* dx, int16_t* dy, int W, int H, float minScale, uint8_t* gate , hipStream_t s);
struct SmallJob { int kind; const void* src; void* dst; void* dst2; uint8_t* gate; int W, H; float minScale; };
struct SmallJobs { SmallJob j[3]; int n; };
void launch_small_jobs(const SmallJobs& a, hipStream_t s);
bool launch_rgb_pyramid(const uint8_t* rgb, int W, int H, uint8_t* const gray[3], int16_t* const dIdx[3], int16_t* const dIdy[3], uint8_t* const gate[3],
                        const float minScale[3], bool derivatives, hipStream_t s);
void launch_rgbd_last_l0(const float4* predV, const float* fillDepth, const uint8_t* predGray, const uint8_t* fillGray,
                         const FrameDev* frame, float* depth0, uint8_t* image0, int n, hipStream_t s, int frameToFrameRGB = 0);
size_t so3_scratch_bytes(int W2, int H2);
int launch_so3_prealign(const uint8_t* lastImage2, const uint8_t* nextImage2, int W2, int H2, Intr k2, So3Result* out, void* scratch,
                        hipStream_t s);
void launch_rgb_residual_only(const RgbLevel& L, const float* krk_kt, RgbCorr* corres, int* sums, hipStream_t s);
void launch_rgb_step_only(const RgbLevel& L, const RgbCorr* corres, float sigma, Intr k, float sobelScale, double* out32, hipStream_t s);
struct RgbdLaunch {
    IcpLaunch icp;
    RgbLevel L;
    RgbCorr* corres;
    const float* rgb_partials_in; float* rgb_partials_out;
    const int2* cnt_in; int2* cnt_out;
    float icpWeight; int icpOn; int rgbOnly; float sobelScale;
    int level, prev_level;
    const So3Result* so3_in;
};
void launch_rgbd_iteration(const RgbdLaunch& l, hipStream_t s);
void launch_rgbd_finalize(const float* icp_partials, const float* rgb_partials, const int2* cnt, int nb, float icpWeight, int icpOn,
                          int rgbOnly, int rgbOn, int prev_level, const GNState* st_in, const So3Result* so3, PoseDev* pose,
                          PoseDev* host_mirror, float* log_out, float jump_limit, hipStream_t s);

void launch_init_surfels(const uint8_t* rgb, const float* depthRaw, const float* depthF, int W, int H, Intr k,
                         float maxDepth, const FrameDev* frame, float4* rec , uint8_t* flags, hipStream_t s);
constexpr int kSurfelGridBlocks = 2048;
void launch_index_scatter(Surfels src, const FrameDev* frame, const PoseDev* pose, int W, int H, Intr k,
                          float maxDepth, int timeDelta, unsigned long long* keys, bool transposed , hipStream_t s,
                          int blocks = kSurfelGridBlocks, const VisList* vis = nullptr);
void launch_run_table(Surfels s, FrameDev* frame, hipStream_t st, bool refresh = false);
size_t run_table_runs(long capacity, long pixels);
size_t run_table_entries(long capacity, long pixels);
void launch_cull(Surfels s, const FrameDev* frame, const PoseDev* pose, int W, int H, Intr k, float maxDepth, int timeDelta, int* list, int* count,
                 int* ctl, int max_runs, hipStream_t st);
void launch_index_resolve(Surfels src, const FrameDev* frame, const PoseDev* pose, unsigned long long* keys, int W, int H, int* index,
                          float4* vc, float4* nr, float4* ct , float4* packed ,
                          const float* depthF, const uint8_t* mask, uint8_t* maskT ,
                          bool keys_transposed , hipStream_t s, int* decay_stats = nullptr, int maskID = 0);
void launch_fuse_data(const uint8_t* rgb, const float* depthRaw, const float* depthF, const uint8_t* mask,
                      int maskID, const FrameDev* frame, const PoseDev* pose, float weightMultiplier, float maxDepth,
                      int W, int H, Intr k, const int* index, const float4* vc, const float4* nr, uint8_t* cand_op,
                      float4* cand_rec, int* upd_first, int* cand_best, hipStream_t s, int bboxLimit = 1);
void launch_fuse_update(Surfels s, const FrameDev* frame, int* upd_first, const uint8_t* cand_op, const int* cand_best, const float4* cand_rec,
                        int W, int H, hipStream_t st);
void launch_fuse_update_copy(Surfels src, Surfels dst, const FrameDev* frame, int* upd_first, const float4* cand_rec, const PoseDev* pose,
                             int W, int H, Intr k, float maxDepth, int timeDelta, unsigned long long* keys_or_null, bool transposed,
                             hipStream_t s, int blocks = kSurfelGridBlocks);
struct CleanIn {
    FrameDev* frame; const PoseDev* pose; int W, H; Intr k; int timeDelta; float confThreshold, outlierCoeff; int maskID;
    const int* index; const float4* vc; const float4* ct;
    const float4* packed; const uint8_t* maskT;
    const float* depthF; const uint8_t* mask;
    const uint8_t* cand_op; const float4* cand_rec;
    uint8_t* flags; float* newconf; int* block_counts;
    int* host_count;
    unsigned long long* host_append; unsigned seq;
    bool transposed;
    bool literalWindow;
};
constexpr int kAppendSeqBits = 20, kAppendRunBits = 18, kAppendPhysBits = 26;
__host__ __device__ inline unsigned long long append_mirror(unsigned seq, int runs, int phys) {
    return ((unsigned long long)(seq & ((1u << kAppendSeqBits) - 1u)) << (kAppendRunBits + kAppendPhysBits)) | ((unsigned long long)(unsigned)runs << kAppendPhysBits) |
           (unsigned long long)(unsigned)phys;
}
int compact_blocks_for(long elements);
void launch_clean_small(const CleanIn& in, Surfels src, Surfels dst, hipStream_t s, int blocks = kCompactBlocks);
constexpr int kCleanGridMax = 2048;
constexpr int kCleanCtlInts = 8;
int clean_runs_grid(long elements);
void launch_clean_runs(const CleanIn& in, Surfels buf, const VisList* runs, int* ctl, int blocks, hipStream_t s);
void launch_clean_append(const CleanIn& in, Surfels buf, hipStream_t s);
constexpr int kDecayStats = 9;
void launch_arm_decay_stats(int* stats , hipStream_t st);
void launch_cull_clean(Surfels s, const FrameDev* frame, const PoseDev* pose, int W, int H, Intr k, int timeDelta, float confThreshold, int* decay_stats,
                       int* list, int* count, int* ctl, int max_runs, hipStream_t st);
void launch_densify(Surfels src, Surfels dst, FrameDev* frame, int* offs, int* host_count, hipStream_t st);
void launch_run_offsets(Surfels s, const FrameDev* frame, int* offs, int* total, hipStream_t st);
void launch_compact_records(const float4* rec, const uint8_t* flags, int n, Surfels dst, FrameDev* frame,
                            int* block_counts, int* host_count_mirror, hipStream_t s);
void launch_splat_scatter(Surfels src, const FrameDev* frame, const PoseDev* pose, int W, int H, Intr k,
                          float maxDepth, float confThreshold, int timeDelta, unsigned long long* keys,
                          hipStream_t s, int blocks = kSurfelGridBlocks);
void launch_splat_resolve(Surfels src, const PoseDev* pose, unsigned long long* keys, int W, int H, Intr k,
                          float4* predV, float4* predN, uchar4* predImage, uint16_t* predTime, FrameDev* frame,
                          const uint8_t* rgb , uint8_t* predGray , uint8_t* fillGray ,
                          hipStream_t s, int fillPassthrough = 0 );
size_t splat_tiles_scratch_ints(int W, int H);
struct SplatTuning { int sprite_lanes = 4, tile_threads = 512, tile_h = 24; };
struct FrameAdvance { FrameDev* host_mirror; const PoseDev* bg_pose; float* log_slot; };
int launch_splat_tiled(Surfels src, FrameDev* frame, const PoseDev* pose, int W, int H, Intr k, float maxDepth, float confThreshold,
                       int timeDelta, int* tile_count, int* entries , int entries_cap,
                       float4* rec0 , float4* rec1 , void* bbox , float4* predV, float4* predN,
                       uchar4* predImage, uint16_t* predTime, const uint8_t* rgb, uint8_t* predGray, uint8_t* fillGray, hipStream_t s,
                       const FrameAdvance* advance = nullptr, int fillPassthrough = 0, unsigned long long* prof = nullptr ,
                       SplatTuning tune = SplatTuning(), const VisList* vis = nullptr);
struct ObjPassArgs {
    Surfels a, b;
    FrameDev* frame; PoseDev* pose;
    int maskID; float confThreshold, fuseMaxDepth, weightMultiplier;
    unsigned long long* keys; int* index; float4* ivc; float4* inr; float4* iclean;
    uint8_t* cand_op; float4* cand_rec; int* upd_first; int* cand_best; int* clean_ctl; int* host_count;
    unsigned long long* host_append; unsigned clean_seq;
    uint8_t* flags; float* newconf; int* block_counts;
    float4* predV; float4* predN; uchar4* predImage; uint16_t* predTime; uint8_t* predGray;
    FrameDev* host_frame; float* log_slot;
    unsigned global_payload;
};
struct ObjBatch {
    const ObjPassArgs* m; int n;
    int W, H; Intr k; float maxDepthProcessed, globalMaxDepth; int timeDelta; float outlierCoeff; int cleanLiteral, bboxLimit;
    int denseSprites;
    int updateCopy;
    int cleanSmall;
    const uint8_t* rgb; const float* depthRaw; const float* depthF; const uint8_t* mask; const PoseDev* bg_pose;
    uint8_t* maskT;
    unsigned long long* global_keys;
};
void launch_obj_global_scatter(const ObjBatch& b, int blocks, hipStream_t s);
void launch_obj_fuse_clean(const ObjBatch& b, int blocks, int clean_blocks, hipStream_t s, int compact_blocks = kCompactBlocks);
void launch_obj_predict_advance(const ObjBatch& b, int blocks, hipStream_t s);
void launch_fill_keys(unsigned long long* keys, int n, hipStream_t s);
void launch_fill_int(int* p, int v, int n, hipStream_t s);
void launch_edge_map(const float* vmap, const float* nmap, float* out, int W, int H, float wD, float wC, hipStream_t s);
void launch_edge_binary(const float* edge, uint8_t* out, uint8_t* tmp, int W, int H, float threshold, int radius,
                        int iterations, hipStream_t s);
void launch_global_scatter(Surfels src, const FrameDev* frame, const PoseDev* pose, int W, int H, Intr k, float maxDepth,
                           float confThreshold, int timeDelta, int order, int id, unsigned long long* keys, hipStream_t s,
                           int blocks = kSurfelGridBlocks);
void launch_global_resolve(unsigned long long* keys, uint8_t* ids, int P, hipStream_t s);
int gn_solve_standalone(const double* sys29, const double* resultRt16, const float* Rprev9, const float* tprev3, double* x_serial, double* x_wave,
                        double* resultRt_out, float* Rcurr9, float* tcurr3, float* stats2, hipStream_t s);
int launch_global_tiled(Surfels src, FrameDev* frame, const PoseDev* pose, int W, int H, Intr k, float maxDepth, float confThreshold,
                        int timeDelta, int order, int id, int* tile_count, int* entries, int entries_cap, float4* rec0, float4* rec1, void* bbox,
                        unsigned long long* keys, hipStream_t s, SplatTuning tune = SplatTuning(), const VisList* vis = nullptr);
void launch_spawn_pose(PoseDev* obj, const PoseDev* bg, FrameDev* objFrame, const FrameDev* bgFrame, PoseDev* host_mirror,
                       hipStream_t s);
void launch_static_pose(PoseDev* obj, const PoseDev* bg, PoseDev* host_mirror, hipStream_t s);
void launch_override_pose(PoseDev* pose, const float* in_pose16_colmajor, int mode, PoseDev* host_mirror, hipStream_t s);
void launch_model_state(const PoseDev* pose, const FrameDev* frame, float* out16, hipStream_t s);

constexpr int kMaxRenderModels = 256;
struct RenderModel {
    Surfels s; const FrameDev* frame; const PoseDev* pose;
    unsigned base;
    int max_runs;
    float thr; int class_id, color_type, index, is_background;
    float M[12];
};
struct RenderView { float Vi[12]; };
struct RenderArgs {
    RenderModel* models; int n_models;
    int W, H; Intr k; float near_z, far_z;
    int drawUnstable, drawPoints, drawWindow, timeDelta;
    const FrameDev* tick_frame;
    const float* palette; int n_palette;
    uchar4 clear;
    int* work; int* work_count;
    int tilesX, tilesY, tile_cap;
    int* tile_count;
    uint2* entries;
    int* overflow;
    uchar4* out_rgba; float* out_depth; int* out_model;
};
void launch_render(RenderArgs a, const RenderView& v, const PoseDev* bg_pose, int max_runs, hipStream_t s);

uint64_t nn_workspace_bytes(int64_t n_target);
int nn_run(const float* d_target, int target_stride, int64_t n_target, const float* d_query, int query_stride, int64_t n_query,
           const float* T16 , float radius, float* d_dist, int32_t* d_idx, void* d_ws, uint64_t ws_bytes, hipStream_t s,
           const char** why);
void launch_nn_gather(Surfels s, const FrameDev* frame, const int* offs, float thr, float4* out, int n, int max_runs, hipStream_t st);

void launch_pose_log(const PoseDev* pose, const PoseDev* bg_pose , float* slot, hipStream_t s);
void launch_frame_advance(FrameDev* frame, int W, int H, FrameDev* host_mirror, const PoseDev* pose, const PoseDev* bg_pose,
                          float* log_slot, hipStream_t s);

}
```

### maskfusion_amd/csrc/mf_surfel.hip

```cpp
#pragma clang fp contract(off)
#include "mf_device.h"
#include "mf_walk.h"
#include "mf_rgbd_device.h"

namespace mf {

__global__ void k_fill_keys(unsigned long long* keys, int n) {
    for (int i = blockIdx.x * blockDim.x + threadIdx.x; i < n; i += gridDim.x * blockDim.x) keys[i] = kEmptyKey;
}
void launch_fill_keys(unsigned long long* keys, int n, hipStream_t s) {
    hipLaunchKernelGGL(k_fill_keys, dim3(min((n + 255) / 256, 2048)), dim3(256), 0, s, keys, n);
}
__global__ void k_fill_int(int* p, int v, int n) {
    for (int i = blockIdx.x * blockDim.x + threadIdx.x; i < n; i += gridDim.x * blockDim.x) p[i] = v;
}
void launch_fill_int(int* p, int v, int n, hipStream_t s) {
    hipLaunchKernelGGL(k_fill_int, dim3(min((n + 255) / 256, 2048)), dim3(256), 0, s, p, v, n);
}

__device__ __forceinline__ int cand_count(int W, int H, int tick) {
    const int par = tick & 1;
    return ((W - par + 1) / 2) * ((H - par + 1) / 2);
}

// ... 132 lines not shown
                                                   bool pretest = false) {
    const float time = (float)frame->tick;
    float Ri[9];
#pragma unroll
    for (int q = 0; q < 9; ++q) Ri[q] = pose->Ri[q];
    const float3 ti = f3(pose->ti[0], pose->ti[1], pose->ti[2]);
    for_each_surfel_slice<1>(src, frame, vis_list, vis_count, [&](int i, bool live) {
        index_scatter_one(src, i, live, time, Ri, ti, W, H, k, maxDepth, timeDelta, keys, transposed, pretest);
    });
}

__global__ __launch_bounds__(256) void k_index_scatter(Surfels src, const FrameDev* __restrict__ frame,
                                                       const PoseDev* __restrict__ pose, int W, int H, Intr k, float maxDepth,
                                                       int timeDelta, unsigned long long* __restrict__ keys, int transposed,
                                                       const int* __restrict__ vis_list, const int* __restrict__ vis_count) {
    index_scatter_body(src, frame, pose, W, H, k, maxDepth, timeDelta, keys, transposed, vis_list, vis_count);
}

void launch_index_scatter(Surfels src, const FrameDev* frame, const PoseDev* pose, int W, int H, Intr k, float maxDepth,
                          int timeDelta, unsigned long long* keys, bool transposed, hipStream_t s, int blocks, const VisList* vis) {
    hipLaunchKernelGGL(k_index_scatter, dim3(blocks), dim3(256), 0, s, src, frame, pose, W, H, k, maxDepth, timeDelta, keys,
                       transposed ? 1 : 0, vis ? vis->list : nullptr, vis ? vis->count : nullptr);
}

struct RunAcc {
    int lo[3], hi[3], tmax, cmin, unstamped;
    __device__ __forceinline__ void reset() {
        lo[0] = lo[1] = lo[2] = kBoxEmptyMin; hi[0] = hi[1] = hi[2] = kBoxEmptyMax; tmax = kBoxEmptyMax; cmin = kBoxEmptyMin; unstamped = 0;
    }
    __device__ __forceinline__ void add(float4 pc, float lastTime) {
        if (pc.x == pc.x && pc.y == pc.y && pc.z == pc.z) {
            const int ex = box_enc(pc.x), ey = box_enc(pc.y), ez = box_enc(pc.z);
            lo[0] = min(lo[0], ex); lo[1] = min(lo[1], ey); lo[2] = min(lo[2], ez);
            hi[0] = max(hi[0], ex); hi[1] = max(hi[1], ey); hi[2] = max(hi[2], ez);
        }
        tmax = max(tmax, lastTime == lastTime ? box_enc(lastTime) : 0x7F800000);
        if (pc.w == pc.w) cmin = min(cmin, box_enc(pc.w));
        if (lastTime <= 0.f) unstamped = 1;
    }
};
constexpr int kRunRed = 9;
__device__ __forceinline__ void run_box_reduce(const RunAcc& t, int (*s_red)[kRunRed]) {
    const int lane = threadIdx.x & 63, wave = threadIdx.x >> 6;
    int lo[3], hi[3];
#pragma unroll
    for (int q = 0; q < 3; ++q) { lo[q] = wave_min_i(t.lo[q]); hi[q] = wave_max_i(t.hi[q]); }
    const int tmax = wave_max_i(t.tmax), cmin = wave_min_i(t.cmin);
    const int unstamped = __ballot(t.unstamped != 0) != 0ull ? 1 : 0;
    if (lane == 0) {
#pragma unroll
        for (int q = 0; q < 3; ++q) { s_red[wave][q] = lo[q]; s_red[wave][4 + q] = hi[q]; }
        s_red[wave][3] = tmax; s_red[wave][7] = cmin; s_red[wave][8] = unstamped;
    }
}
__device__ __forceinline__ void run_box_store(int4* __restrict__ box, int r, int start, int len, const int (*s_red)[kRunRed]) {
    int4 a, b;
    a.x = min(min(s_red[0][0], s_red[1][0]), min(s_red[2][0], s_red[3][0]));
    a.y = min(min(s_red[0][1], s_red[1][1]), min(s_red[2][1], s_red[3][1]));
    a.z = min(min(s_red[0][2], s_red[1][2]), min(s_red[2][2], s_red[3][2]));
    a.w = max(max(s_red[0][3], s_red[1][3]), max(s_red[2][3], s_red[3][3]));
    b.x = max(max(s_red[0][4], s_red[1][4]), max(s_red[2][4], s_red[3][4]));
    b.y = max(max(s_red[0][5], s_red[1][5]), max(s_red[2][5], s_red[3][5]));
    b.z = max(max(s_red[0][6], s_red[1][6]), max(s_red[2][6], s_red[3][6]));
    b.w = start;
    const int cmin = min(min(s_red[0][7], s_red[1][7]), min(s_red[2][7], s_red[3][7]));
    const int unstamped = s_red[0][8] | s_red[1][8] | s_red[2][8] | s_red[3][8];
    box[kBoxStride * r] = a; box[kBoxStride * r + 1] = b; box[kBoxStride * r + 2] = make_int4(len, cmin, unstamped, 0);
}

__global__ __launch_bounds__(256) void k_run_table(Surfels s, FrameDev* __restrict__ frame, int refresh) {
    __shared__ int s_red[4][kRunRed];
    const int n = frame->count;
    const int runs = refresh ? frame->runs : (n + kRun - 1) / kRun;
    for (int r = blockIdx.x; r < runs; r += gridDim.x) {
        const int start = refresh ? run_start(s.box, r) : r * kRun, len = refresh ? run_len(s.box, r) : min(n - r * kRun, kRun);
        RunAcc acc;
        acc.reset();
        for (int i = start + (int)threadIdx.x; i < start + len; i += 256) acc.add(s.pc[i], s.ct[i].w);
        run_box_reduce(acc, s_red);
        __syncthreads();
        if (threadIdx.x == 0) run_box_store(s.box, r, start, len, s_red);
        __syncthreads();
    }
    if (blockIdx.x == 0 && threadIdx.x == 0 && !refresh) {
        frame->runs = runs; frame->phys = n; frame->first = 0; frame->first_run = 0;
    }
}
void launch_run_table(Surfels s, FrameDev* frame, hipStream_t st, bool refresh) {
    hipLaunchKernelGGL(k_run_table, dim3(1024), dim3(256), 0, st, s, frame, refresh ? 1 : 0);
}
size_t run_table_runs(long capacity, long pixels) { return (size_t)(2 * ((capacity + kRun - 1) / kRun) + 4 * ((pixels / 4 + kRun - 1) / kRun + 2) + 64); }
size_t run_table_entries(long capacity, long pixels) { return (size_t)kBoxStride * run_table_runs(capacity, pixels); }

__device__ __forceinline__ bool run_box_in_frustum(int4 a, int4 b, const PoseDev* __restrict__ pose, int W, int H, Intr k, float maxDepth, float& zlo, float& zhi,
                                                   int* outside = nullptr) {
    const float lo[3] = {box_dec(a.x), box_dec(a.y), box_dec(a.z)}, hi[3] = {box_dec(b.x), box_dec(b.y), box_dec(b.z)};
    int out_near = 1, out_far = 1, out_l = 1, out_r = 1, out_t = 1, out_b = 1;
    zlo = INFINITY; zhi = -INFINITY;
#pragma unroll
    for (int c = 0; c < 8; ++c) {
        const float3 p = f3((c & 1) ? hi[0] : lo[0], (c & 2) ? hi[1] : lo[1], (c & 4) ? hi[2] : lo[2]);
        const float3 h = mul33(pose->Ri, p) + f3(pose->ti[0], pose->ti[1], pose->ti[2]);
        zlo = fminf(zlo, h.z); zhi = fmaxf(zhi, h.z);
        out_near &= h.z < -0.01f;
        out_far &= h.z > maxDepth + 0.01f;
        out_l &= k.fx * h.x + (k.cx + 2.f) * h.z < 0.f;
        out_r &= k.fx * h.x + (k.cx - (float)W - 2.f) * h.z > 0.f;
        out_t &= k.fy * h.y + (k.cy + 2.f) * h.z < 0.f;
        out_b &= k.fy * h.y + (k.cy - (float)H - 2.f) * h.z > 0.f;
    }
    if (outside) *outside = out_l | (out_r << 1) | (out_t << 2) | (out_b << 3);
    return !(out_near | out_far | out_l | out_r | out_t | out_b);
}
__device__ __forceinline__ void run_list_append(bool listed, int r, int* __restrict__ list, int* __restrict__ count, int* __restrict__ ctl) {
    const unsigned long long m = __ballot(listed);
    int base = 0;
    if ((threadIdx.x & 63) == 0 && m) base = atomicAdd(&ctl[0], __popcll(m));
    base = __shfl(base, 0, 64);
    if (listed) list[base + lane_rank(m)] = r;
}
__device__ __forceinline__ bool run_list_finish(int* __restrict__ count, int* __restrict__ ctl) {
    __syncthreads();
    if (threadIdx.x != 0) return false;
    const int done = atomicAdd(&ctl[1], 1);
    if (done != (int)gridDim.x - 1) return false;
    count[0] = __hip_atomic_load(&ctl[0], __ATOMIC_RELAXED, __HIP_MEMORY_SCOPE_AGENT);
    __hip_atomic_store(&ctl[0], 0, __ATOMIC_RELAXED, __HIP_MEMORY_SCOPE_AGENT);
    __hip_atomic_store(&ctl[1], 0, __ATOMIC_RELAXED, __HIP_MEMORY_SCOPE_AGENT);
    return true;
}

__global__ __launch_bounds__(256) void k_cull(Surfels s, const FrameDev* __restrict__ frame, const PoseDev* __restrict__ pose, int W, int H, Intr k,
                                              float maxDepth, int timeDelta, int* __restrict__ list, int* __restrict__ count, int* __restrict__ ctl) {
    const int runs = frame->runs;
    const float time = (float)frame->tick;
    const int r = blockIdx.x * 256 + threadIdx.x;
    bool vis = false;
    if (r < runs) {
        const int4 a = s.box[kBoxStride * r], b = s.box[kBoxStride * r + 1];
        if (run_len(s.box, r) > 0 && a.x <= b.x && a.y <= b.y && a.z <= b.z && !(time - box_dec(a.w) > (float)timeDelta)) {
            float zlo, zhi;
            vis = run_box_in_frustum(a, b, pose, W, H, k, maxDepth, zlo, zhi);
        }
    }
    run_list_append(vis, r, list, count, ctl);
    (void)run_list_finish(count, ctl);
}
void launch_cull(Surfels s, const FrameDev* frame, const PoseDev* pose, int W, int H, Intr k, float maxDepth, int timeDelta, int* list, int* count,
                 int* ctl, int max_runs, hipStream_t st) {
    hipLaunchKernelGGL(k_cull, dim3((max_runs + 255) / 256), dim3(256), 0, st, s, frame, pose, W, H, k, maxDepth, timeDelta, list, count, ctl);
}

struct ResolvedTexel { int index; float4 vc, nr, ct, p0, p1; };
template <bool kPacked>
__device__ __forceinline__ ResolvedTexel resolve_texel(const Surfels& src, const PoseDev* __restrict__ pose, unsigned long long key, bool want_ct, int first) {
    ResolvedTexel r;
    r.index = 0;
    r.vc = r.nr = r.ct = r.p0 = r.p1 = make_float4(0, 0, 0, 0);
    if (key == kEmptyKey) return r;
    const int i = (int)(unsigned)(key & 0xFFFFFFFFull);
    const int id = i == first ? 0 : i;
    const float4 pc = src.pc[i];
    const float3 h = mul33(pose->Ri, f3(pc.x, pc.y, pc.z)) + f3(pose->ti[0], pose->ti[1], pose->ti[2]);
    if (kPacked) {
        const float4 c4 = src.ct[i];
        r.p0 = make_float4(h.x, h.y, h.z, pc.w);
        r.p1 = make_float4(c4.z, c4.w, __int_as_float(id), 0.f);
    } else {
        const float4 n4 = src.nr[i];
        const float3 n = normalize_gl(mul33(pose->Ri, f3(n4.x, n4.y, n4.z)));
        r.index = id;
        r.vc = make_float4(h.x, h.y, h.z, pc.w);
        r.nr = make_float4(n.x, n.y, n.z, n4.w);
        if (want_ct) r.ct = src.ct[i];
    }
    return r;
}
struct ResolveOut {
    int* index; float4* vc; float4* nr; float4* ct; float4* packed; const float* depthF; const uint8_t* mask; uint8_t* maskT;
    const FrameDev* frame;
    int* decay_stats; int maskID;
};
__device__ __forceinline__ void decay_stats_add(const ResolveOut& o, bool in_image, int x, int y, int W, int H, float depth, int maskValue) {
    if (!o.decay_stats) return;
    const bool foreign = in_image && maskValue != o.maskID && maskValue < 255 && depth == depth;
    const int e = box_enc(depth);
    const bool side[4] = {foreign && x == 0, foreign && x == W - 1, foreign && y == 0, foreign && y == H - 1};
#pragma unroll
    for (int q = 0; q < 4; ++q) {
        if (__ballot(side[q]) == 0ull) continue;
        const int lo = wave_min_i(side[q] ? e : kBoxEmptyMin), hi = wave_max_i(side[q] ? e : kBoxEmptyMax);
        if ((threadIdx.x & 63) == 0) { atomicMin(&o.decay_stats[2 * q], lo); atomicMax(&o.decay_stats[2 * q + 1], hi); }
    }
    if (__ballot(foreign) != 0ull) {
        const int amin = wave_min_i(foreign ? e : kBoxEmptyMin);
        if ((threadIdx.x & 63) == 0) atomicMin(&o.decay_stats[8], amin);
    }
}
template <bool kPacked>
__device__ __forceinline__ void index_resolve_same_body(Surfels src, const PoseDev* __restrict__ pose, unsigned long long* __restrict__ keys, int P, ResolveOut o) {
    static_assert(!kPacked, "the packed map goes through a tile kernel");
    const int p = blockIdx.x * 256 + threadIdx.x;
    if (p >= P) return;
    const unsigned long long key = keys[p];
    keys[p] = kEmptyKey;
    const ResolvedTexel r = resolve_texel<false>(src, pose, key, o.ct != nullptr, o.frame->first);
    o.index[p] = r.index; o.vc[p] = r.vc; o.nr[p] = r.nr;
    if (o.ct) o.ct[p] = r.ct;
}
constexpr int kResolveTile = 16;
template <bool kPacked>
__device__ __forceinline__ void index_resolve_transposing_body(Surfels src, const PoseDev* __restrict__ pose, unsigned long long* __restrict__ keys, int W, int H,
                                                               ResolveOut o, int tile) {
    __shared__ float4 s_a[kResolveTile][kResolveTile + 1], s_b[kResolveTile][kResolveTile + 1], s_c[kPacked ? 1 : kResolveTile][kResolveTile + 1];
    __shared__ int s_i[kPacked ? 1 : kResolveTile][kResolveTile + 1];
    __shared__ uint8_t s_mk[kPacked ? kResolveTile : 1][kResolveTile + 1];
    const int tilesX = (W + kResolveTile - 1) / kResolveTile;
    const int x0 = (tile % tilesX) * kResolveTile, y0 = (tile / tilesX) * kResolveTile;
    const int f = threadIdx.x & (kResolveTile - 1), g = threadIdx.x / kResolveTile;
    {
        const int lx = kPacked ? f : g, ly = kPacked ? g : f;
        const int x = x0 + lx, y = y0 + ly;
        ResolvedTexel r = resolve_texel<kPacked>(src, pose, kEmptyKey, false, 0);
        int mk = 0;
        if (x < W && y < H) {
            const int p = kPacked ? y * W + x : x * H + y;
            const unsigned long long key = keys[p];
            keys[p] = kEmptyKey;
            r = resolve_texel<kPacked>(src, pose, key, o.ct != nullptr, o.frame->first);
            if (kPacked) { r.p1.w = o.depthF[p]; mk = o.mask[p]; s_mk[lx][ly] = (uint8_t)mk; }
        }
        if (kPacked) decay_stats_add(o, x < W && y < H, x, y, W, H, r.p1.w, mk);
        if (kPacked) { s_a[lx][ly] = r.p0; s_b[lx][ly] = r.p1; }
        else { s_i[lx][ly] = r.index; s_a[lx][ly] = r.vc; s_b[lx][ly] = r.nr; if (o.ct) s_c[lx][ly] = r.ct; }
    }
    __syncthreads();
    {
        const int lx = kPacked ? g : f, ly = kPacked ? f : g;
        const int x = x0 + lx, y = y0 + ly;
        if (x < W && y < H) {
            if (kPacked) {
                const int tp = x * H + y;
                o.packed[2 * tp] = s_a[lx][ly];
                o.packed[2 * tp + 1] = s_b[lx][ly];
                o.maskT[tp] = s_mk[lx][ly];
            } else {
                const int p = y * W + x;
                o.index[p] = s_i[lx][ly]; o.vc[p] = s_a[lx][ly]; o.nr[p] = s_b[lx][ly];
                if (o.ct) o.ct[p] = s_c[lx][ly];
            }
        }
    }
}
__device__ __forceinline__ void index_resolve_packed_body(Surfels src, const PoseDev* __restrict__ pose, unsigned long long* __restrict__ keys, int W, int H,
                                                          ResolveOut o, int tile) {
    __shared__ float s_d[kResolveTile][kResolveTile + 1];
    __shared__ uint8_t s_mk[kResolveTile][kResolveTile + 1];
    const int tilesX = (W + kResolveTile - 1) / kResolveTile;
    const int x0 = (tile % tilesX) * kResolveTile, y0 = (tile / tilesX) * kResolveTile;
    const int f = threadIdx.x & (kResolveTile - 1), g = threadIdx.x / kResolveTile;
    {
        const int x = x0 + f, y = y0 + g;
        float d = 0.f;
        int mk = 0;
        if (x < W && y < H) { d = o.depthF[y * W + x]; mk = o.mask[y * W + x]; s_d[f][g] = d; s_mk[f][g] = (uint8_t)mk; }
        decay_stats_add(o, x < W && y < H, x, y, W, H, d, mk);
    }
    __syncthreads();
    const int x = x0 + g, y = y0 + f;
    if (x < W && y < H) {
        const int tp = x * H + y;
        const unsigned long long key = keys[tp];
        keys[tp] = kEmptyKey;
        ResolvedTexel r = resolve_texel<true>(src, pose, key, false, o.frame->first);
        r.p1.w = s_d[g][f];
        o.packed[2 * tp] = r.p0;
        o.packed[2 * tp + 1] = r.p1;
        o.maskT[tp] = s_mk[g][f];
    }
}
__global__ __launch_bounds__(256) void k_index_resolve(Surfels src, const PoseDev* __restrict__ pose, unsigned long long* __restrict__ keys, int P, ResolveOut o) {
    index_resolve_same_body<false>(src, pose, keys, P, o);
}
__global__ __launch_bounds__(256) void k_index_resolve_packed(Surfels src, const PoseDev* __restrict__ pose, unsigned long long* __restrict__ keys, int W, int H,
                                                              ResolveOut o) {
    index_resolve_packed_body(src, pose, keys, W, H, o, (int)blockIdx.x);
}
template <bool kPacked>
__global__ __launch_bounds__(256) void k_index_resolve_transposing(Surfels src, const PoseDev* __restrict__ pose, unsigned long long* __restrict__ keys, int W, int H,
                                                                   ResolveOut o) {
    index_resolve_transposing_body<kPacked>(src, pose, keys, W, H, o, (int)blockIdx.x);
}
int resolve_tiles(int W, int H) { return ((W + kResolveTile - 1) / kResolveTile) * ((H + kResolveTile - 1) / kResolveTile); }

void launch_index_resolve(Surfels src, const FrameDev* frame, const PoseDev* pose, unsigned long long* keys, int W, int H, int* index, float4* vc,
                          float4* nr, float4* ct, float4* packed, const float* depthF, const uint8_t* mask, uint8_t* maskT, bool keys_transposed,
                          hipStream_t s, int* decay_stats, int maskID) {
    const int P = W * H;
    const ResolveOut o{index, vc, nr, ct, packed, depthF, mask, maskT, frame, packed ? decay_stats : nullptr, maskID};
    const dim3 flat((P + 255) / 256), tiles(resolve_tiles(W, H));
    if (packed) {
        if (keys_transposed) hipLaunchKernelGGL(k_index_resolve_packed, tiles, dim3(256), 0, s, src, pose, keys, W, H, o);
        else hipLaunchKernelGGL(k_index_resolve_transposing<true>, tiles, dim3(256), 0, s, src, pose, keys, W, H, o);
    } else {
        if (keys_transposed) hipLaunchKernelGGL(k_index_resolve_transposing<false>, tiles, dim3(256), 0, s, src, pose, keys, W, H, o);
        else hipLaunchKernelGGL(k_index_resolve, flat, dim3(256), 0, s, src, pose, keys, P, o);
    }
}

struct FuseDataArgs {
    const uint8_t* rgb; const float* depthRaw; const float* depthF; const uint8_t* mask; int maskID;
    const FrameDev* frame; const PoseDev* pose; float weightMultiplier; float maxDepth;
    int bboxLimit;
    int W, H; Intr k;
    const int* index; const float4* vc; const float4* nr;
    uint8_t* cand_op; float4* cand_rec; int* upd_first;
    int* cand_best;
};

__device__ __forceinline__ void fuse_data_body(const FuseDataArgs& a) {
    const int time = a.frame->tick;
    const int par = time & 1;
    const int W = a.W, H = a.H;
    const int nxc = (W - par + 1) / 2, nyc = (H - par + 1) / 2;
    const int xi = blockIdx.x * 64 + (threadIdx.x & 63);
    const int yi = blockIdx.y * 4 + (threadIdx.x >> 6);
    if (xi >= nxc || yi >= nyc) return;
    const int c = xi * nyc + yi;
    const int px = 2 * xi + par, py = 2 * yi + par;
    const Intr k = a.k;
    uint8_t op = 0;
    const float x = (float)px + 0.5f, y = (float)py + 0.5f;
    const float3 vLocal = get_vertex(a.depthRaw, W, H, px, py, x, y, k);
    bool valid = a.mask[py * W + px] == a.maskID;
    valid = valid && !(texf(a.depthRaw, W, H, px - 1, py) == 0 || texf(a.depthRaw, W, H, px, py - 1) == 0 ||
                       texf(a.depthRaw, W, H, px + 1, py) == 0 || texf(a.depthRaw, W, H, px, py + 1) == 0);
    float maxDepth = a.maxDepth;
    if (a.maskID != 0 && a.bboxLimit) {
        const FrameDev* f = a.frame;
        if (f->bbox[0] <= f->bbox[3] && f->bbox[1] <= f->bbox[4] && f->bbox[2] <= f->bbox[5]) {
            const float* Ri = a.pose->Ri; const float* ti = a.pose->ti;
            const float bbscale = 0.001f;
            const float zmin = ((Ri[6] * (bbscale * (float)f->bbox[0]) + Ri[7] * (bbscale * (float)f->bbox[1])) + Ri[8] * (bbscale * (float)f->bbox[2])) + ti[2];
            const float zmax = ((Ri[6] * (bbscale * (float)f->bbox[3]) + Ri[7] * (bbscale * (float)f->bbox[4])) + Ri[8] * (bbscale * (float)f->bbox[5])) + ti[2];
            const float lo = zmin < zmax ? zmin : zmax, hi = zmin < zmax ? zmax : zmin;
            maxDepth = fminf(maxDepth, hi + 0.05f * fabsf(hi - lo));
        }
    }
    valid = valid && (vLocal.z > 0 && vLocal.z <= maxDepth);
    if (valid) {
        float R[9];
#pragma unroll
        for (int q = 0; q < 9; ++q) R[q] = a.pose->R[q];
        const float3 t = f3(a.pose->t[0], a.pose->t[1], a.pose->t[2]);
        const float3 vGlobal = mul33(R, vLocal) + t;
        const float3 vF = get_vertex(a.depthF, W, H, px, py, x, y, k);
        const float3 nLocal = get_normal_central(a.depthF, W, H, px, py, x, y, vF, k);
        const float3 nGlobal = mul33(R, nLocal);
        const uint8_t* pc = a.rgb + (size_t)(py * W + px) * 3;
        const float weighting = a.pose->fusionWeight * a.weightMultiplier;

        const float xl = (x - k.cx) * (1.0f / k.fx), yl = (y - k.cy) * (1.0f / k.fy);
        const float lambda = sqrtf(xl * xl + yl * yl + 1);
        const float3 ray = f3(xl, yl, 1);
        float bestDist = 1000;
        int best = 0;
        bool merge = false;
        int cur9[9]; float4 vc9[9], nr9[9];
#pragma unroll
        for (int q = 0; q < 9; ++q) {
            const int da = q / 3 - 1, db = q % 3 - 1;
            const int tp = clampi(py + db, 0, H - 1) * W + clampi(px + da, 0, W - 1);
            cur9[q] = a.index[tp];
            vc9[q] = a.vc[tp];
            nr9[q] = a.nr[tp];
        }
#pragma unroll
        for (int q = 0; q < 9; ++q) {
            const int current = cur9[q];
            if (current > 0) {
                const float4 vc = vc9[q];
                const float zdiff = vc.z - vLocal.z;
                if (fabsf(zdiff * lambda) < 0.05f) {
                    const float dist = norm3(cross3(ray, f3(vc.x, vc.y, vc.z)));
                    const float4 nr = nr9[q];
                    const float3 nn = f3(nr.x, nr.y, nr.z);
                    const float ang = shader_acos(dot3(nn, nLocal) / (norm3(nn) * norm3(nLocal)));
                    if (dist < bestDist && (fabsf(nr.z) < 0.75f || fabsf(ang) < 0.5f)) {
                        merge = true; bestDist = dist; best = current;
                    }
                }
            }
        }
        op = merge ? 1 : 2;
        a.cand_rec[c * 3 + 0] = make_float4(vGlobal.x, vGlobal.y, vGlobal.z, surfel_confidence(x, y, weighting, k));
        a.cand_rec[c * 3 + 1] = make_float4((float)((pc[0] << 16) + (pc[1] << 8) + pc[2]), 0.f, (float)time, merge ? -1.f : -2.f);
        a.cand_rec[c * 3 + 2] = make_float4(nGlobal.x, nGlobal.y, nGlobal.z, surfel_radius(vF.z, nLocal.z, k));
        if (merge) {
            atomicMin(&a.upd_first[best], c);
            a.cand_best[c] = best;
        }
    }
    a.cand_op[c] = op;
}

__global__ __launch_bounds__(256) void k_fuse_data(const FuseDataArgs a) { fuse_data_body(a); }

void launch_fuse_data(const uint8_t* rgb, const float* depthRaw, const float* depthF, const uint8_t* mask, int maskID,
                      const FrameDev* frame, const PoseDev* pose, float weightMultiplier, float maxDepth, int W, int H, Intr k,
                      const int* index, const float4* vc, const float4* nr, uint8_t* cand_op, float4* cand_rec, int* upd_first,
                      int* cand_best, hipStream_t s, int bboxLimit) {
    FuseDataArgs a{rgb, depthRaw, depthF, mask, maskID, frame, pose, weightMultiplier, maxDepth, bboxLimit, W, H, k,
                   index, vc, nr, cand_op, cand_rec, upd_first, cand_best};
    dim3 grid(((W + 1) / 2 + 63) / 64, ((H + 1) / 2 + 3) / 4);
    hipLaunchKernelGGL(k_fuse_data, grid, dim3(256), 0, s, a);
}

__device__ __forceinline__ void surfel_merge(float4& pc, float4& ct, float4& nr, float4 mp, float4 mc, float4 mn, float time) {
    const float c_k = pc.w, a = mp.w;
    if (mn.w < (1.0f + 0.5f) * nr.w) {
        pc = make_float4(((c_k * pc.x) + (a * mp.x)) / (c_k + a), ((c_k * pc.y) + (a * mp.y)) / (c_k + a),
                         ((c_k * pc.z) + (a * mp.z)) / (c_k + a), c_k + a);
        const float3 oc = decode_color(ct.x), nc = decode_color(mc.x);
        ct = make_float4(encode_color(((c_k * oc.x) + (a * nc.x)) / (c_k + a), ((c_k * oc.y) + (a * nc.y)) / (c_k + a),
                                      ((c_k * oc.z) + (a * nc.z)) / (c_k + a)),
                         ct.y, ct.z, time);
        const float4 av = make_float4(((c_k * nr.x) + (a * mn.x)) / (c_k + a), ((c_k * nr.y) + (a * mn.y)) / (c_k + a),
                                      ((c_k * nr.z) + (a * mn.z)) / (c_k + a), ((c_k * nr.w) + (a * mn.w)) / (c_k + a));
        const float3 nn = normalize_gl(f3(av.x, av.y, av.z));
        nr = make_float4(nn.x, nn.y, nn.z, av.w);
    } else {
        pc.w = c_k + a;
        ct.w = time;
    }
}

__device__ __forceinline__ void fuse_update_body(Surfels s, const FrameDev* __restrict__ frame, int* __restrict__ upd_first,
                                                 const uint8_t* __restrict__ cand_op, const int* __restrict__ cand_best,
                                                 const float4* __restrict__ cand_rec, int W, int H) {
    const int c = blockIdx.x * 256 + threadIdx.x;
    if (c >= cand_count(W, H, frame->tick)) return;
    if (cand_op[c] != 1) return;
    const int i = cand_best[c];
    if (i < 0 || i >= frame->phys) return;
    if (upd_first[i] != c) return;
    upd_first[i] = kNoUpdate;
    float4 pc = s.pc[i], ct = s.ct[i], nr = s.nr[i];
    surfel_merge(pc, ct, nr, cand_rec[c * 3 + 0], cand_rec[c * 3 + 1], cand_rec[c * 3 + 2], (float)frame->tick);
    s.pc[i] = pc; s.ct[i] = ct; s.nr[i] = nr;
}

struct IndexScatterArgs { const PoseDev* pose; int W, H; Intr k; float maxDepth; int timeDelta; unsigned long long* keys; int transposed; };
__device__ __forceinline__ void fuse_update_copy_body(Surfels src, Surfels dst, const FrameDev* __restrict__ frame, int* __restrict__ upd_first,
                                                      const float4* __restrict__ cand_rec, const IndexScatterArgs& ix) {
    const int n = frame->count;
    const float time = (float)frame->tick;
    float Ri[9];
    float3 ti = f3(0, 0, 0);
    if (ix.keys) {
#pragma unroll
        for (int q = 0; q < 9; ++q) Ri[q] = ix.pose->Ri[q];
        ti = f3(ix.pose->ti[0], ix.pose->ti[1], ix.pose->ti[2]);
    }
    for (int i = blockIdx.x * 256 + threadIdx.x; i < n; i += gridDim.x * 256) {
        float4 pc = src.pc[i], ct = src.ct[i], nr = src.nr[i];
        const int m = upd_first[i];
        if (m != kNoUpdate) {
            upd_first[i] = kNoUpdate;
            surfel_merge(pc, ct, nr, cand_rec[m * 3 + 0], cand_rec[m * 3 + 1], cand_rec[m * 3 + 2], time);
        }
        dst.pc[i] = pc; dst.ct[i] = ct; dst.nr[i] = nr;
        if (ix.keys) {
            const float3 h = mul33(Ri, f3(pc.x, pc.y, pc.z)) + ti;
            if (!(h.z > ix.maxDepth || h.z <= 0 || time - ct.w > (float)ix.timeDelta)) {
                const float u = ((ix.k.fx * h.x) / h.z) + ix.k.cx;
                const float v = ((ix.k.fy * h.y) / h.z) + ix.k.cy;
                if (u >= 0.f && u < (float)ix.W && v >= 0.f && v < (float)ix.H) {
                    const int p = ix.transposed ? (int)floorf(u) * ix.H + (int)floorf(v) : (int)floorf(v) * ix.W + (int)floorf(u);
                    zmin_key(&ix.keys[p], ((unsigned long long)__float_as_uint(h.z) << 32) | (unsigned)i);
                }
            }
        }
    }
}
__global__ __launch_bounds__(256) void k_fuse_update_copy(Surfels src, Surfels dst, const FrameDev* __restrict__ frame, int* __restrict__ upd_first,
                                                          const float4* __restrict__ cand_rec, const IndexScatterArgs ix) {
    fuse_update_copy_body(src, dst, frame, upd_first, cand_rec, ix);
}
void launch_fuse_update_copy(Surfels src, Surfels dst, const FrameDev* frame, int* upd_first, const float4* cand_rec, const PoseDev* pose,
                             int W, int H, Intr k, float maxDepth, int timeDelta, unsigned long long* keys_or_null, bool transposed,
                             hipStream_t s, int blocks) {
    IndexScatterArgs ix{pose, W, H, k, maxDepth, timeDelta, keys_or_null, transposed ? 1 : 0};
    hipLaunchKernelGGL(k_fuse_update_copy, dim3(blocks), dim3(256), 0, s, src, dst, frame, upd_first, cand_rec, ix);
}

__global__ __launch_bounds__(256) void k_fuse_update(Surfels s, const FrameDev* __restrict__ frame, int* __restrict__ upd_first,
                                                     const uint8_t* __restrict__ cand_op, const int* __restrict__ cand_best,
                                                     const float4* __restrict__ cand_rec, int W, int H) {
    fuse_update_body(s, frame, upd_first, cand_op, cand_best, cand_rec, W, H);
}

static inline int cand_blocks(int W, int H) { return (((W + 1) / 2) * ((H + 1) / 2) + 255) / 256; }

void launch_fuse_update(Surfels s, const FrameDev* frame, int* upd_first, const uint8_t* cand_op, const int* cand_best, const float4* cand_rec,
                        int W, int H, hipStream_t st) {
    hipLaunchKernelGGL(k_fuse_update, dim3(cand_blocks(W, H)), dim3(256), 0, st, s, frame, upd_first, cand_op, cand_best, cand_rec, W, H);
}

struct CleanArgs {
    Surfels src, dst; FrameDev* frame; const PoseDev* pose; int W, H; Intr k;
    int timeDelta; float confThreshold; float outlierCoeff; int maskID; int transposed;
    int literal;
    const int* index; const float4* vc; const float4* ct;
    const float4* packed;
    const float* depthF; const uint8_t* mask;
    const uint8_t* maskT;
    const uint8_t* cand_op; const float4* cand_rec;
    uint8_t* flags; float* newconf;
    int* block_counts;
    int* host_count;
    unsigned long long* host_append; unsigned seq;
    int append;
    const int* run_list; const int* run_count;
    int* ctl;
};

__device__ __forceinline__ void window_slots_literal(float c, int size, int (&u)[3], int (&m)[3]) {
    const float fs = (float)size;
    const float step = (1.0f / (fs * 1.0f)) * 0.5f;
    const float half = (1.0f * step) * 2.0f;
    const float end = c + half;
    u[0] = u[1] = u[2] = 0; m[0] = m[1] = m[2] = 0;
    int s = -1, last = -1;
    float i = c - half;
#pragma unroll
    for (int k = 0; k < 5; ++k) {
        if (i < end) {
            const int t = clampi((int)floorf(rintf(i * fs * 256.0f) * (1.0f / 256.0f)), 0, size - 1);
            if (t != last) { s = min(s + 1, 2); u[s] = t; last = t; }
            m[s] += 1;
        }
        i += step;
    }
}

__device__ __forceinline__ bool clean_test(const CleanArgs& a, float4 pc, float4 ct, float4 nr, float time, const float* Ri,
                                           float3 ti, float& newconf, int& decay, const float4* nr_lazy = nullptr) {
    const int W = a.W, H = a.H;
    bool test = true;
    const float3 lp = mul33(Ri, f3(pc.x, pc.y, pc.z)) + ti;
    const float x = ((a.k.fx * lp.x) / lp.z) + a.k.cx;
    const float y = ((a.k.fy * lp.y) / lp.z) + a.k.cy;
    int count = 0, zCount = 0;
    if (time - ct.w < (float)a.timeDelta && lp.z > 0 && x > 0 && y > 0 && x < (float)W && y < (float)H) {
        if (nr_lazy) nr = *nr_lazy;
        const float3 ln = normalize_gl(mul33(Ri, f3(nr.x, nr.y, nr.z)));
        int txs[4], tys[4];
        txs[0] = clampi((int)floorf(x - 1.0f), 0, W - 1); txs[1] = clampi((int)floorf(x - 0.5f), 0, W - 1);
        txs[2] = clampi((int)floorf(x), 0, W - 1);        txs[3] = clampi((int)floorf(x + 0.5f), 0, W - 1);
        tys[0] = clampi((int)floorf(y - 1.0f), 0, H - 1); tys[1] = clampi((int)floorf(y - 0.5f), 0, H - 1);
        tys[2] = clampi((int)floorf(y), 0, H - 1);        tys[3] = clampi((int)floorf(y + 0.5f), 0, H - 1);
        int ux[3] = {txs[0], txs[2], txs[3]};
        int mx[3] = {1 + (txs[1] == txs[0]), 1 + (txs[1] != txs[0]) + (txs[3] == txs[2]), (txs[3] != txs[2]) ? 1 : 0};
        int uy[3] = {tys[0], tys[2], tys[3]};
        int my[3] = {1 + (tys[1] == tys[0]), 1 + (tys[1] != tys[0]) + (tys[3] == tys[2]), (tys[3] != tys[2]) ? 1 : 0};
        if (a.literal) {
            window_slots_literal(x / (float)W, W, ux, mx);
            window_slots_literal(y / (float)H, H, uy, my);
        }
#pragma unroll
        for (int ia = 0; ia < 3; ++ia) {
#pragma unroll
            for (int ib = 0; ib < 3; ++ib) {
                const int tp = a.transposed ? ux[ia] * H + uy[ib] : uy[ib] * W + ux[ia];
                const int mult = mx[ia] * my[ib];
                if (mult <= 0) continue;
                float4 v, c;
                int idx;
                if (a.packed) {
                    v = a.packed[2 * tp];
                    const float4 r1 = a.packed[2 * tp + 1];
                    c = make_float4(0.f, 0.f, r1.x, r1.y);
                    idx = __float_as_int(r1.z);
                } else {
                    idx = a.index[tp];
                    v = a.vc[tp];
                    c = a.ct[tp];
                }
                if (idx > 0) {
                    const float dx = v.x - lp.x, dy = v.y - lp.y;
                    if (c.z < ct.z && v.w > a.confThreshold && v.z > lp.z && v.z - lp.z < 0.01f &&
                        sqrtf(dx * dx + dy * dy) < nr.w * 1.4f)
                        count += mult;
                    if (c.w == time && v.w > a.confThreshold && v.z > lp.z && v.z - lp.z > 0.01f && fabsf(ln.z) > 0.85f)
                        zCount += mult;
                }
            }
        }
    }
    if (count > 8 || zCount > 4) test = false;
    float w = ct.w;
    if (w == -2.f) w = time;
    if (w == -1.f || ((time - w) > 20 && pc.w < a.confThreshold)) test = false;
    if (w > 0 && time - w > (float)a.timeDelta) test = true;
    const int fx_ = isnan(x) ? 0 : clampi((int)fminf(fmaxf(floorf(x), -1.f), (float)W), 0, W - 1);
    const int fy_ = isnan(y) ? 0 : clampi((int)fminf(fmaxf(floorf(y), -1.f), (float)H), 0, H - 1);
    const float wDepth = a.packed ? a.packed[2 * (fx_ * H + fy_) + 1].w : a.depthF[fy_ * W + fx_];
    const int maskValue = a.packed ? a.maskT[fx_ * H + fy_] : a.mask[fy_ * W + fx_];
    newconf = pc.w;
    decay = 0;
    if (maskValue != a.maskID && maskValue < 255 && (wDepth > lp.z - 0.05f && wDepth < lp.z + 0.05f)) {
        const float kk = 0.5f + 0.5f * (1 - a.outlierCoeff / 10.0f);
        if (maskValue == 0) { newconf *= kk; decay = 1; }
        else if (a.maskID == 0) { newconf *= 0.25f * kk; decay = 2; }
        else { newconf *= kk; decay = 1; }
    }
    return test;
}
__device__ __forceinline__ float clean_decayed(const CleanArgs& a, float conf, int decay) {
    const float kk = 0.5f + 0.5f * (1 - a.outlierCoeff / 10.0f);
    if (decay == 1) conf *= kk;
    else if (decay == 2) conf *= 0.25f * kk;
    return conf;
}

__device__ __forceinline__ void clean_small_flags_body(const CleanArgs& a) {
    __shared__ int s_w[4];
    const int count = a.append ? a.frame->phys : a.frame->count;
    const int first = a.append ? count : 0;
    const int ncand = cand_count(a.W, a.H, a.frame->tick);
    const int total = count + ncand;
    const float time = (float)a.frame->tick;
    float Ri[9];
#pragma unroll
    for (int q = 0; q < 9; ++q) Ri[q] = a.pose->Ri[q];
    const float3 ti = f3(a.pose->ti[0], a.pose->ti[1], a.pose->ti[2]);
    const int chunk = chunk_size(total - first);
    const int beg = first + blockIdx.x * chunk, end = min(total, beg + chunk);
    int kept = 0;
    for (int i = beg + threadIdx.x; i < end; i += 256) {
        bool keep = false;
        float nc = 0.f;
        int dk = 0;
        if (i < count) {
            keep = clean_test(a, a.src.pc[i], a.src.ct[i], a.src.nr[i], time, Ri, ti, nc, dk);
        } else {
            const int c = i - count;
            if (a.cand_op[c] == 2)
                keep = clean_test(a, a.cand_rec[c * 3 + 0], a.cand_rec[c * 3 + 1], a.cand_rec[c * 3 + 2], time, Ri, ti, nc, dk);
        }
        a.flags[i - first] = keep ? 1 : 0;
        a.newconf[i - first] = nc;
        kept += keep ? 1 : 0;
    }
    const int tot = block_sum_i(kept, s_w);
    if (threadIdx.x == 0) {
        a.block_counts[blockIdx.x] = tot;
        if (blockIdx.x == 0) {
            a.frame->countNext = count;
            a.frame->runsNext = a.frame->runs;
            if (a.maskID != 0 && !a.append)
                for (int q = 0; q < 6; ++q) a.frame->bbox_acc[q] = q < 3 ? kBBoxEmptyMin : kBBoxEmptyMax;
        }
    }
    if (a.append) {
        const int r0 = a.frame->runs, nnew = (ncand + kRun - 1) / kRun + 1;
        for (int j = blockIdx.x * 256 + threadIdx.x; j < nnew; j += gridDim.x * 256) {
            a.dst.box[kBoxStride * (r0 + j)] = make_int4(kBoxEmptyMin, kBoxEmptyMin, kBoxEmptyMin, kBoxEmptyMax);
            a.dst.box[kBoxStride * (r0 + j) + 1] = make_int4(kBoxEmptyMax, kBoxEmptyMax, kBoxEmptyMax, count + j * kRun);
            a.dst.box[kBoxStride * (r0 + j) + 2] = make_int4(0, kBoxEmptyMin, 0, 0);
        }
    }
}

__global__ __launch_bounds__(256) void k_clean_small_flags(const CleanArgs a) { clean_small_flags_body(a); }

__device__ __forceinline__ void clean_small_compact_body(const CleanArgs& a) {
    __shared__ int s_w[4];
    __shared__ int s_bb[6];
    const bool bbox_on = a.maskID != 0;
    int bmin[3] = {kBBoxEmptyMin, kBBoxEmptyMin, kBBoxEmptyMin}, bmax[3] = {kBBoxEmptyMax, kBBoxEmptyMax, kBBoxEmptyMax};
    if (bbox_on && threadIdx.x < 6) s_bb[threadIdx.x] = threadIdx.x < 3 ? kBBoxEmptyMin : kBBoxEmptyMax;
    const int count = a.frame->countNext;
    const int first = a.append ? count : 0;
    const int total = count + cand_count(a.W, a.H, a.frame->tick);
    const int r0 = a.frame->runsNext;
    const float time = (float)a.frame->tick;
    const int chunk = chunk_size(total - first);
    const int beg = first + blockIdx.x * chunk, end = min(total, beg + chunk);
    const int lane = threadIdx.x & 63, wave = threadIdx.x >> 6;
    int base = 0;
    for (int i0 = beg; i0 < end; i0 += 256) {
        const int i = i0 + threadIdx.x;
        const bool in = i < end;
        uint8_t flag = 0;
        float nc = 0.f;
        float4 pc = make_float4(0, 0, 0, 0), ct = pc, nr = pc;
        if (in) {
            flag = a.flags[i - first];
            nc = a.newconf[i - first];
            if (i < count) { pc = a.src.pc[i]; ct = a.src.ct[i]; nr = a.src.nr[i]; }
            else { const int c = i - count; pc = a.cand_rec[c * 3 + 0]; ct = a.cand_rec[c * 3 + 1]; nr = a.cand_rec[c * 3 + 2]; }
        }
        if (i0 == beg) base = block_base(a.block_counts, s_w) + first;
        const bool keep = in && flag;
        const unsigned long long m = __ballot(keep);
        if (lane == 0) s_w[wave] = __popcll(m);
        __syncthreads();
        int off = base;
        for (int w = 0; w < wave; ++w) off += s_w[w];
        const int tot = s_w[0] + s_w[1] + s_w[2] + s_w[3];
        const int o = off + lane_rank(m);
        const bool written = keep && o < a.dst.cap;
        if (written) {
            pc.w = nc;
            if (ct.w == -2.f) ct.w = time;
            a.dst.pc[o] = pc; a.dst.ct[o] = ct; a.dst.nr[o] = nr;
            if (bbox_on && pc.w > a.confThreshold) {
                const int x = (int)(1000.f * pc.x), y = (int)(1000.f * pc.y), z = (int)(1000.f * pc.z);
                bmin[0] = min(bmin[0], x); bmin[1] = min(bmin[1], y); bmin[2] = min(bmin[2], z);
                bmax[0] = max(bmax[0], x); bmax[1] = max(bmax[1], y); bmax[2] = max(bmax[2], z);
            }
        }
        if (a.append) {
            const int j = written ? (o - count) / kRun : 0x7FFFFFFF;
            const int j0 = wave_min_i(j);
            if (j0 != 0x7FFFFFFF) {
                for (int g = 0; g < 2; ++g) {
                    const bool mine = written && j == j0 + g;
                    const unsigned long long mm = __ballot(mine);
                    if (mm == 0ull) continue;
                    RunAcc acc;
                    acc.reset();
                    if (mine) acc.add(pc, ct.w);
                    int v[8] = {acc.lo[0], acc.lo[1], acc.lo[2], acc.tmax, acc.hi[0], acc.hi[1], acc.hi[2], acc.cmin};
#pragma unroll
                    for (int q = 0; q < 8; ++q) v[q] = (q < 3 || q == 7) ? wave_min_i(v[q]) : wave_max_i(v[q]);
                    const bool unstamped = __ballot(acc.unstamped != 0) != 0ull;
                    if (lane == 0) {
                        int* e = reinterpret_cast<int*>(&a.dst.box[kBoxStride * (r0 + j0 + g)]);
                        atomicMin(&e[0], v[0]); atomicMin(&e[1], v[1]); atomicMin(&e[2], v[2]); atomicMax(&e[3], v[3]);
                        atomicMax(&e[4], v[4]); atomicMax(&e[5], v[5]); atomicMax(&e[6], v[6]);
                        atomicAdd(&e[8], __popcll(mm)); atomicMin(&e[9], v[7]);
                        if (unstamped) atomicMax(&e[10], 1);
                    }
                }
            }
        }
        base += tot;
        __syncthreads();
    }
    if (bbox_on) {
        if (beg < end) {
#pragma unroll
            for (int q = 0; q < 3; ++q) {
                if (bmin[q] != kBBoxEmptyMin) atomicMin(&s_bb[q], bmin[q]);
                if (bmax[q] != kBBoxEmptyMax) atomicMax(&s_bb[3 + q], bmax[q]);
            }
            __syncthreads();
            if (threadIdx.x < 3 && s_bb[threadIdx.x] != kBBoxEmptyMin) atomicMin(&a.frame->bbox_acc[threadIdx.x], s_bb[threadIdx.x]);
            else if (threadIdx.x >= 3 && threadIdx.x < 6 && s_bb[threadIdx.x] != kBBoxEmptyMax) atomicMax(&a.frame->bbox_acc[threadIdx.x], s_bb[threadIdx.x]);
        }
    }
    if (blockIdx.x != gridDim.x - 1) return;
    if (beg >= end) base = block_base(a.block_counts, s_w) + first;
    if (threadIdx.x == 0) {
        const int end_slot = min(base, a.dst.cap);
        if (a.append) {
            const int n = a.frame->count + (end_slot - count);
            a.frame->count = n;
            a.frame->phys = end_slot;
            a.frame->runs = r0 + (end_slot - count + kRun - 1) / kRun;
            int fr = a.frame->first_run;
            while (fr < r0 && run_len(a.dst.box, fr) == 0) ++fr;
            a.frame->first_run = fr;
            a.frame->first = fr < r0 ? run_start(a.dst.box, fr) : count;
            if (a.host_count) *a.host_count = n;
            if (a.host_append) *a.host_append = append_mirror(a.seq, r0 + (end_slot - count + kRun - 1) / kRun, end_slot);
        } else {
            a.frame->count = a.frame->phys = end_slot;
            a.frame->runs = 0;
            a.frame->first = 0; a.frame->first_run = 0;
            if (a.host_count) *a.host_count = end_slot;
        }
    }
}

__global__ __launch_bounds__(256) void k_clean_small_compact(const CleanArgs a) { clean_small_compact_body(a); }

__global__ __launch_bounds__(256) void k_cull_clean(Surfels s, const FrameDev* __restrict__ frame, const PoseDev* __restrict__ pose, int W, int H, Intr k,
                                                    int timeDelta, float confThreshold, int* __restrict__ decay_stats, int* __restrict__ list,
                                                    int* __restrict__ count, int* __restrict__ ctl) {
    const int runs = frame->runs;
    const float time = (float)frame->tick;
    const int r = blockIdx.x * 256 + threadIdx.x;
    int e_side[8];
#pragma unroll
    for (int q = 0; q < 8; ++q) e_side[q] = decay_stats[q];
    const int e_amin = decay_stats[8];
    const bool has_any = e_amin != kBoxEmptyMin;
    bool visit = false;
    if (r < runs) {
        const int4 a = s.box[kBoxStride * r], b = s.box[kBoxStride * r + 1], c = s.box[kBoxStride * r + 2];
        if (c.x > 0) {
            const bool recent = !(time - box_dec(a.w) > (float)timeDelta);
            if (c.y != kBoxEmptyMin && box_dec(c.y) < confThreshold && recent) visit = true;
            else if (c.z != 0) visit = true;
            else if (a.x <= b.x && a.y <= b.y && a.z <= b.z) {
                float zlo, zhi;
                int outside = 0;
                if (run_box_in_frustum(a, b, pose, W, H, k, INFINITY, zlo, zhi, &outside)) visit = true;
                else if (zlo > 0.06f) {
                    visit = true;
#pragma unroll
                    for (int q = 0; q < 4; ++q)
                        if ((outside >> q) & 1) {
                            const bool has = e_side[2 * q] != kBoxEmptyMin;
                            if (!has || box_dec(e_side[2 * q + 1]) <= zlo - 0.06f || box_dec(e_side[2 * q]) >= zhi + 0.06f) visit = false;
                        }
                    if (outside == 0) visit = has_any;
                } else if (zhi < -0.06f)
                    visit = has_any && box_dec(e_amin) < zhi + 0.06f;
                else visit = has_any;
            }
        }
    }
    run_list_append(visit, r, list, count, ctl);
    if (run_list_finish(count, ctl)) {
        for (int q = 0; q < kDecayStats; ++q)
            __hip_atomic_store(&decay_stats[q], (q == 8 || (q & 1) == 0) ? kBoxEmptyMin : kBoxEmptyMax, __ATOMIC_RELAXED, __HIP_MEMORY_SCOPE_AGENT);
    }
}
__global__ void k_arm_decay_stats(int* st) {
    if (threadIdx.x == 0 && blockIdx.x == 0)
        for (int q = 0; q < kDecayStats; ++q) st[q] = (q == 8 || (q & 1) == 0) ? kBoxEmptyMin : kBoxEmptyMax;
}
void launch_arm_decay_stats(int* stats, hipStream_t st) { hipLaunchKernelGGL(k_arm_decay_stats, dim3(1), dim3(64), 0, st, stats); }
void launch_cull_clean(Surfels s, const FrameDev* frame, const PoseDev* pose, int W, int H, Intr k, int timeDelta, float confThreshold, int* decay_stats,
                       int* list, int* count, int* ctl, int max_runs, hipStream_t st) {
    hipLaunchKernelGGL(k_cull_clean, dim3((max_runs + 255) / 256), dim3(256), 0, st, s, frame, pose, W, H, k, timeDelta, confThreshold, decay_stats, list,
                       count, ctl);
}

__device__ __forceinline__ void clean_runs_body(const CleanArgs& a) {
    __shared__ int s_cnt[2][4];
    __shared__ int s_red[4][kRunRed];
    __shared__ int s_bb[6];
    static_assert(kRun == 512, "two slots per thread");
    const bool bbox_on = a.maskID != 0;
    int bmin[3] = {kBBoxEmptyMin, kBBoxEmptyMin, kBBoxEmptyMin}, bmax[3] = {kBBoxEmptyMax, kBBoxEmptyMax, kBBoxEmptyMax};
    if (bbox_on && threadIdx.x < 6) s_bb[threadIdx.x] = threadIdx.x < 3 ? kBBoxEmptyMin : kBBoxEmptyMax;
    const int nlist = a.run_list ? *a.run_count : a.frame->runs;
    const float time = (float)a.frame->tick;
    float Ri[9];
#pragma unroll
    for (int q = 0; q < 9; ++q) Ri[q] = a.pose->Ri[q];
    const float3 ti = f3(a.pose->ti[0], a.pose->ti[1], a.pose->ti[2]);
    const int lane = threadIdx.x & 63, wave = threadIdx.x >> 6;
    int wg_died = 0;
    for (int v = blockIdx.x; v < nlist; v += gridDim.x) {
        const int r = a.run_list ? a.run_list[v] : v;
        const int start = run_start(a.src.box, r), len = run_len(a.src.box, r);
        const int off0 = (int)threadIdx.x, off1 = 256 + (int)threadIdx.x;
        const bool live0 = off0 < len, live1 = off1 < len;
        float4 pc0 = make_float4(0, 0, 0, 0), pc1 = pc0;
        float2 tm0 = make_float2(0, 0), tm1 = tm0;
        if (live0) { pc0 = a.src.pc[start + off0]; tm0 = *reinterpret_cast<const float2*>(reinterpret_cast<const float*>(&a.src.ct[start + off0]) + 2); }
        if (live1) { pc1 = a.src.pc[start + off1]; tm1 = *reinterpret_cast<const float2*>(reinterpret_cast<const float*>(&a.src.ct[start + off1]) + 2); }
        float nc0 = 0.f, nc1 = 0.f;
        int dk = 0;
        const bool keep0 = live0 && clean_test(a, pc0, make_float4(0.f, 0.f, tm0.x, tm0.y), make_float4(0, 0, 0, 0), time, Ri, ti, nc0, dk, &a.src.nr[start + off0]);
        const bool keep1 = live1 && clean_test(a, pc1, make_float4(0.f, 0.f, tm1.x, tm1.y), make_float4(0, 0, 0, 0), time, Ri, ti, nc1, dk, &a.src.nr[start + off1]);
        RunAcc acc;
        acc.reset();
        const bool st0 = keep0 && tm0.y == -2.f, st1 = keep1 && tm1.y == -2.f;
        if (keep0) acc.add(make_float4(pc0.x, pc0.y, pc0.z, nc0), st0 ? time : tm0.y);
        if (keep1) acc.add(make_float4(pc1.x, pc1.y, pc1.z, nc1), st1 ? time : tm1.y);
        const unsigned long long m0 = __ballot(keep0), m1 = __ballot(keep1);
        if (lane == 0) { s_cnt[0][wave] = __popcll(m0); s_cnt[1][wave] = __popcll(m1); }
        int o0 = lane_rank(m0), o1 = lane_rank(m1);
        run_box_reduce(acc, s_red);
        __syncthreads();
        const int c0 = s_cnt[0][0] + s_cnt[0][1] + s_cnt[0][2] + s_cnt[0][3];
        const int kept = c0 + s_cnt[1][0] + s_cnt[1][1] + s_cnt[1][2] + s_cnt[1][3];
        for (int w = 0; w < wave; ++w) { o0 += s_cnt[0][w]; o1 += s_cnt[1][w]; }
        o1 += c0;
        const bool conf0 = keep0 && __float_as_int(nc0) != __float_as_int(pc0.w), conf1 = keep1 && __float_as_int(nc1) != __float_as_int(pc1.w);
        if (kept != len) {
            const bool mv0 = keep0 && o0 != off0, mv1 = keep1 && o1 != off1;
            float4 c40 = make_float4(0, 0, 0, 0), n40 = c40, c41 = c40, n41 = c40;
            if (mv0) { c40 = a.src.ct[start + off0]; n40 = a.src.nr[start + off0]; }
            if (mv1) { c41 = a.src.ct[start + off1]; n41 = a.src.nr[start + off1]; }
            asm volatile("s_waitcnt vmcnt(0)" ::: "memory");
            __syncthreads();
            if (st0) c40.w = time;
            if (st1) c41.w = time;
            if (mv0) { a.src.pc[start + o0] = make_float4(pc0.x, pc0.y, pc0.z, nc0); a.src.ct[start + o0] = c40; a.src.nr[start + o0] = n40; }
            else {
                if (conf0) reinterpret_cast<float*>(&a.src.pc[start + off0])[3] = nc0;
                if (st0) reinterpret_cast<float*>(&a.src.ct[start + off0])[3] = time;
            }
            if (mv1) { a.src.pc[start + o1] = make_float4(pc1.x, pc1.y, pc1.z, nc1); a.src.ct[start + o1] = c41; a.src.nr[start + o1] = n41; }
            else {
                if (conf1) reinterpret_cast<float*>(&a.src.pc[start + off1])[3] = nc1;
                if (st1) reinterpret_cast<float*>(&a.src.ct[start + off1])[3] = time;
            }
        } else {
            if (conf0) reinterpret_cast<float*>(&a.src.pc[start + off0])[3] = nc0;
            if (conf1) reinterpret_cast<float*>(&a.src.pc[start + off1])[3] = nc1;
            if (st0) reinterpret_cast<float*>(&a.src.ct[start + off0])[3] = time;
            if (st1) reinterpret_cast<float*>(&a.src.ct[start + off1])[3] = time;
        }
        if (threadIdx.x == 0) {
            run_box_store(a.src.box, r, start, kept, s_red);
            wg_died += len - kept;
        }
        if (bbox_on) {
            if (keep0 && nc0 > a.confThreshold) {
                const int x = (int)(1000.f * pc0.x), y = (int)(1000.f * pc0.y), z = (int)(1000.f * pc0.z);
                bmin[0] = min(bmin[0], x); bmin[1] = min(bmin[1], y); bmin[2] = min(bmin[2], z);
                bmax[0] = max(bmax[0], x); bmax[1] = max(bmax[1], y); bmax[2] = max(bmax[2], z);
            }
            if (keep1 && nc1 > a.confThreshold) {
                const int x = (int)(1000.f * pc1.x), y = (int)(1000.f * pc1.y), z = (int)(1000.f * pc1.z);
                bmin[0] = min(bmin[0], x); bmin[1] = min(bmin[1], y); bmin[2] = min(bmin[2], z);
                bmax[0] = max(bmax[0], x); bmax[1] = max(bmax[1], y); bmax[2] = max(bmax[2], z);
            }
        }
        __syncthreads();
    }
    if (bbox_on) {
#pragma unroll
        for (int q = 0; q < 3; ++q) {
            if (bmin[q] != kBBoxEmptyMin) atomicMin(&s_bb[q], bmin[q]);
            if (bmax[q] != kBBoxEmptyMax) atomicMax(&s_bb[3 + q], bmax[q]);
        }
        __syncthreads();
        int seen = 0;
        if (threadIdx.x < 3 && s_bb[threadIdx.x] != kBBoxEmptyMin) seen = atomicMin(&a.frame->bbox_tmp[threadIdx.x], s_bb[threadIdx.x]);
        else if (threadIdx.x >= 3 && threadIdx.x < 6 && s_bb[threadIdx.x] != kBBoxEmptyMax) seen = atomicMax(&a.frame->bbox_tmp[threadIdx.x], s_bb[threadIdx.x]);
        if (threadIdx.x < 6) s_bb[threadIdx.x] = seen;
    }
    __syncthreads();
    if (threadIdx.x == 0) {
        unsigned long long* done64 = reinterpret_cast<unsigned long long*>(a.ctl + 2);
        const unsigned long long old = atomicAdd(done64, (1ull << 32) | (unsigned long long)(unsigned)wg_died);
        if ((unsigned)(old >> 32) == gridDim.x - 1u) {
            const int n = a.frame->count - ((int)(unsigned)(old & 0xFFFFFFFFull) + wg_died);
            a.frame->count = n;
            if (a.host_count) *a.host_count = n;
            if (bbox_on) {
                for (int q = 0; q < 6; ++q) {
                    a.frame->bbox_acc[q] = __hip_atomic_load(&a.frame->bbox_tmp[q], __ATOMIC_RELAXED, __HIP_MEMORY_SCOPE_AGENT);
                    __hip_atomic_store(&a.frame->bbox_tmp[q], q < 3 ? kBBoxEmptyMin : kBBoxEmptyMax, __ATOMIC_RELAXED, __HIP_MEMORY_SCOPE_AGENT);
                }
            }
            __hip_atomic_store(done64, 0ull, __ATOMIC_RELAXED, __HIP_MEMORY_SCOPE_AGENT);
        }
    }
}

__global__ __launch_bounds__(256) void k_clean_runs(const CleanArgs a) { clean_runs_body(a); }

int clean_runs_grid(long elements) {
    const long runs = (elements + kRun - 1) / kRun;
    return (int)(runs < 64 ? 64 : (runs > kCleanGridMax ? kCleanGridMax : runs));
}

__global__ __launch_bounds__(1024) void k_run_offsets(Surfels s, const FrameDev* __restrict__ frame, int* __restrict__ offs, int* __restrict__ total) {
    __shared__ int s_w[16];
    const int runs = frame->runs;
    const int lane = threadIdx.x & 63, wave = threadIdx.x >> 6;
    int carry = 0;
    for (int base = 0; base < runs; base += 1024) {
        const int r = base + (int)threadIdx.x;
        const int v = r < runs ? run_len(s.box, r) : 0;
        const int x = wave_scan(v, lane);
        if (lane == 63) s_w[wave] = x;
        __syncthreads();
        int before = 0, sum = 0;
        for (int w = 0; w < 16; ++w) { if (w < wave) before += s_w[w]; sum += s_w[w]; }
        if (r < runs) offs[r] = carry + before + x - v;
        carry += sum;
        __syncthreads();
    }
    if (threadIdx.x == 0) {
        offs[runs] = carry;
        if (total) *total = runs > 0 ? carry : frame->count;
    }
}
void launch_run_offsets(Surfels s, const FrameDev* frame, int* offs, int* total, hipStream_t st) {
    hipLaunchKernelGGL(k_run_offsets, dim3(1), dim3(1024), 0, st, s, frame, offs, total);
}
__global__ __launch_bounds__(256) void k_densify(Surfels src, Surfels dst, const FrameDev* __restrict__ frame, const int* __restrict__ offs) {
    for_each_live_ordered(src, frame, offs, dst.cap, [&](int from, int to) {
        dst.pc[to] = src.pc[from]; dst.ct[to] = src.ct[from]; dst.nr[to] = src.nr[from];
    });
}
__global__ void k_densify_finish(FrameDev* __restrict__ frame, const int* __restrict__ offs, int cap, int* __restrict__ host_count) {
    if (threadIdx.x != 0 || blockIdx.x != 0) return;
    const int n = min(offs[frame->runs], cap);
    frame->count = frame->phys = n;
    frame->runs = 0; frame->first = 0; frame->first_run = 0;
    if (host_count) *host_count = n;
}
void launch_densify(Surfels src, Surfels dst, FrameDev* frame, int* offs, int* host_count, hipStream_t st) {
    launch_run_offsets(src, frame, offs, nullptr, st);
    hipLaunchKernelGGL(k_densify, dim3(2048), dim3(256), 0, st, src, dst, frame, offs);
    hipLaunchKernelGGL(k_densify_finish, dim3(1), dim3(64), 0, st, frame, offs, dst.cap, host_count);
}


template <int kLanes>
__device__ __forceinline__ void splat_scatter_body(Surfels src, const FrameDev* __restrict__ frame,
                                                   const PoseDev* __restrict__ pose, int W, int H, Intr k, float maxDepth,
                                                   float confThreshold, int timeDelta, unsigned long long* __restrict__ keys, bool pretest = false) {
    const float time = (float)frame->tick;
    float Ri[9];
#pragma unroll
    for (int q = 0; q < 9; ++q) Ri[q] = pose->Ri[q];
    const float3 ti = f3(pose->ti[0], pose->ti[1], pose->ti[2]);
    constexpr int kLX = kLanes >= 2 ? 2 : 1, kLY = kLanes / kLX;
    const int sub = threadIdx.x % kLanes, sx = sub % kLX, sy = sub / kLX;
    for_each_surfel_slice<kLanes>(src, frame, nullptr, nullptr, [&](int i, bool live) {
        if (!live) return;
        const float4 pc = src.pc[i];
        if (pc.w < confThreshold) return;
        const float lastTime = src.ct[i].w;
        const float3 h = mul33(Ri, f3(pc.x, pc.y, pc.z)) + ti;
        if (h.z > maxDepth || h.z < 0 || time - lastTime > (float)timeDelta || lastTime > time) return;
        const float u = ((k.fx * h.x) / h.z) + k.cx, v = ((k.fy * h.y) / h.z) + k.cy;
        if (!(u >= 0.f && u <= (float)W && v >= 0.f && v <= (float)H)) return;
        const float4 n4 = src.nr[i];
        const float3 nrm = normalize_gl(mul33(Ri, f3(n4.x, n4.y, n4.z)));
        const float rad = n4.w;
        const float3 x1 = normalize_gl(f3(nrm.y - nrm.z, -nrm.x, nrm.x)) * (rad * 1.41421356f);
        const float3 y1 = cross3(nrm, x1);
        float xs0 = INFINITY, xs1 = -INFINITY, ys0 = INFINITY, ys1 = -INFINITY;
        const float3 corners[4] = {h + x1, h + y1, h - y1, h - x1};
#pragma unroll
        for (int q = 0; q < 4; ++q) {
            const float pxq = ((k.fx * corners[q].x) / corners[q].z) + k.cx;
            const float pyq = ((k.fy * corners[q].y) / corners[q].z) + k.cy;
            xs0 = fminf(xs0, pxq); xs1 = fmaxf(xs1, pxq);
            ys0 = fminf(ys0, pyq); ys1 = fmaxf(ys1, pyq);
        }
        float size = fmaxf(0.f, fmaxf(fabsf(xs1 - xs0), fabsf(ys1 - ys0)));
        if (!(size > 0.f)) return;
        size = fminf(fmaxf(size, 1.0f), 64.0f);
        const float half = size * 0.5f;
        const int px0 = max(0, (int)ceilf(u - half - 0.5f)), px1 = min(W - 1, (int)ceilf(u + half - 0.5f) - 1);
        const int py0 = max(0, (int)ceilf(v - half - 0.5f)), py1 = min(H - 1, (int)ceilf(v + half - 0.5f) - 1);
        const float sqrRad = rad * rad;
        const float pn = dot3(h, nrm);
        for (int py = py0 + sy; py <= py1; py += kLY) {
            for (int px = px0 + sx; px <= px1; px += kLX) {
                const float fcx = (float)px + 0.5f, fcy = (float)py + 0.5f;
                const float3 l = normalize_gl(f3((fcx - k.cx) / k.fx, (fcy - k.cy) / k.fy, 1.0f));
                const float3 cp = l * (pn / dot3(l, nrm));
                const float3 diff = cp - h;
                if (!(dot3(diff, diff) <= sqrRad)) continue;
                if (!(cp.z > 0.f)) continue;
                const unsigned long long key = ((unsigned long long)__float_as_uint(cp.z) << 32) | (unsigned)i;
                if (pretest) zmin_key_pretested(&keys[py * W + px], key);
                else zmin_key(&keys[py * W + px], key);
            }
        }
    });
}

__global__ __launch_bounds__(256) void k_splat_scatter(Surfels src, const FrameDev* __restrict__ frame,
                                                       const PoseDev* __restrict__ pose, int W, int H, Intr k, float maxDepth,
                                                       float confThreshold, int timeDelta, unsigned long long* __restrict__ keys) {
    splat_scatter_body<1>(src, frame, pose, W, H, k, maxDepth, confThreshold, timeDelta, keys);
}

void launch_splat_scatter(Surfels src, const FrameDev* frame, const PoseDev* pose, int W, int H, Intr k, float maxDepth,
                          float confThreshold, int timeDelta, unsigned long long* keys, hipStream_t s, int blocks) {
    hipLaunchKernelGGL(k_splat_scatter, dim3(blocks), dim3(256), 0, s, src, frame, pose, W, H, k, maxDepth, confThreshold,
                       timeDelta, keys);
}

__device__ __forceinline__ void splat_resolve_body(Surfels src, const PoseDev* __restrict__ pose,
                                                   unsigned long long* __restrict__ keys, int W, int H, Intr k,
                                                   float4* __restrict__ predV, float4* __restrict__ predN,
                                                   uchar4* __restrict__ predImage, uint16_t* __restrict__ predTime,
                                                   FrameDev* __restrict__ frame, const uint8_t* __restrict__ rgb,
                                                   uint8_t* __restrict__ predGray, uint8_t* __restrict__ fillGray, int fillPassthrough) {
    const int px = blockIdx.x * 64 + (threadIdx.x & 63);
    const int py = blockIdx.y * 4 + (threadIdx.x >> 6);
    if (px >= W || py >= H) return;
    const int p = py * W + px;
    const unsigned long long key = keys[p];
    keys[p] = kEmptyKey;
    if (key == kEmptyKey) {
        predV[p] = predN[p] = make_float4(0, 0, 0, 0);
        predImage[p] = make_uchar4(0, 0, 0, 0);
        predTime[p] = 0;
        if (predGray) predGray[p] = 0;
        if (fillGray && rgb) fillGray[p] = intensity_of((float)rgb[p * 3], (float)rgb[p * 3 + 1], (float)rgb[p * 3 + 2]);
        return;
    }
    const int i = (int)(unsigned)(key & 0xFFFFFFFFull);
    const float z = __uint_as_float((unsigned)(key >> 32));
    const float4 pc = src.pc[i], c4 = src.ct[i], n4 = src.nr[i];
    const float3 n = normalize_gl(mul33(pose->Ri, f3(n4.x, n4.y, n4.z)));
    const float fcx = (float)px + 0.5f, fcy = (float)py + 0.5f;
    predV[p] = make_float4((fcx - k.cx) * z * (1.f / k.fx), (fcy - k.cy) * z * (1.f / k.fy), z, pc.w);
    predN[p] = make_float4(n.x, n.y, n.z, n4.w);
    const int ci = (int)c4.x;
    const uchar4 col = make_uchar4((ci >> 16) & 0xFF, (ci >> 8) & 0xFF, ci & 0xFF, 255);
    predImage[p] = col;
    predTime[p] = (uint16_t)(unsigned)c4.z;
    if (predGray || fillGray) {
        const uint8_t gv = intensity_of((float)col.x, (float)col.y, (float)col.z);
        if (predGray) predGray[p] = gv;
        if (fillGray) {
            const bool empty = (col.x == 0 && col.y == 0 && col.z == 0) || fillPassthrough != 0;
            fillGray[p] = (empty && rgb) ? intensity_of((float)rgb[p * 3], (float)rgb[p * 3 + 1], (float)rgb[p * 3 + 2]) : gv;
        }
    }
    if ((px % 20) == 10 && (py % 20) == 10 && px / 20 < W / 20 && py / 20 < H / 20 && col.x > 0 && col.y > 0 && col.z > 0)
        atomicAdd(&frame->cover, 1);
}

__global__ __launch_bounds__(256) void k_splat_resolve(Surfels src, const PoseDev* __restrict__ pose,
                                                       unsigned long long* __restrict__ keys, int W, int H, Intr k,
                                                       float4* __restrict__ predV, float4* __restrict__ predN,
                                                       uchar4* __restrict__ predImage, uint16_t* __restrict__ predTime,
                                                       FrameDev* __restrict__ frame, const uint8_t* __restrict__ rgb,
                                                       uint8_t* __restrict__ predGray, uint8_t* __restrict__ fillGray, int fillPassthrough) {
    splat_resolve_body(src, pose, keys, W, H, k, predV, predN, predImage, predTime, frame, rgb, predGray, fillGray, fillPassthrough);
}

void launch_splat_resolve(Surfels src, const PoseDev* pose, unsigned long long* keys, int W, int H, Intr k, float4* predV,
                          float4* predN, uchar4* predImage, uint16_t* predTime, FrameDev* frame, const uint8_t* rgb,
                          uint8_t* predGray, uint8_t* fillGray, hipStream_t s, int fillPassthrough) {
    dim3 grid((W + 63) / 64, (H + 3) / 4);
    hipLaunchKernelGGL(k_splat_resolve, grid, dim3(256), 0, s, src, pose, keys, W, H, k, predV, predN, predImage, predTime, frame, rgb,
                       predGray, fillGray, fillPassthrough);
}

__device__ __forceinline__ void frame_advance_body(FrameDev* frame, int W, int H, FrameDev* host_mirror, const PoseDev* pose, const PoseDev* bg_pose,
                                                   float* log_slot) {
    if (threadIdx.x != 0 || blockIdx.x != 0) return;
    if (log_slot) pose_log_entry(pose, bg_pose, log_slot);
    const int rw = W / 20, rh = H / 20;
    frame->pad[0] = frame->useFillIn;
    frame->useFillIn = ((float)frame->cover / (float)(rw * rh) < 0.75f) ? 1 : 0;
    frame->cover = 0;
    frame->tick += 1;
    MF_FRAME_BBOX_ADVANCE(frame);
    if (host_mirror) *host_mirror = *frame;
}
__global__ void k_frame_advance(FrameDev* frame, int W, int H, FrameDev* host_mirror, const PoseDev* pose, const PoseDev* bg_pose,
                                float* log_slot) {
    frame_advance_body(frame, W, H, host_mirror, pose, bg_pose, log_slot);
}
void launch_frame_advance(FrameDev* frame, int W, int H, FrameDev* host_mirror, const PoseDev* pose, const PoseDev* bg_pose,
                          float* log_slot, hipStream_t s) {
    hipLaunchKernelGGL(k_frame_advance, dim3(1), dim3(64), 0, s, frame, W, H, host_mirror, pose, bg_pose, log_slot);
}

__global__ void k_pose_log(const PoseDev* __restrict__ pose, const PoseDev* __restrict__ bg_pose, float* __restrict__ slot) {
    if (threadIdx.x == 0 && blockIdx.x == 0) pose_log_entry(pose, bg_pose, slot);
}
void launch_pose_log(const PoseDev* pose, const PoseDev* bg_pose, float* slot, hipStream_t s) {
    hipLaunchKernelGGL(k_pose_log, dim3(1), dim3(64), 0, s, pose, bg_pose, slot);
}

static CleanArgs clean_args(const CleanIn& in, Surfels src, Surfels dst) {
    CleanArgs a;
    a.transposed = in.transposed ? 1 : 0;
    a.literal = in.literalWindow ? 1 : 0;
    a.src = src; a.dst = dst; a.frame = in.frame; a.pose = in.pose; a.W = in.W; a.H = in.H; a.k = in.k; a.timeDelta = in.timeDelta;
    a.confThreshold = in.confThreshold; a.outlierCoeff = in.outlierCoeff; a.maskID = in.maskID; a.index = in.index; a.vc = in.vc; a.ct = in.ct;
    a.packed = in.packed;
    a.depthF = in.depthF; a.mask = in.mask; a.maskT = in.maskT; a.cand_op = in.cand_op; a.cand_rec = in.cand_rec;
    a.flags = in.flags; a.newconf = in.newconf; a.block_counts = in.block_counts; a.host_count = in.host_count;
    a.host_append = in.host_append; a.seq = in.seq;
    a.append = 0; a.run_list = nullptr; a.run_count = nullptr; a.ctl = nullptr;
    return a;
}
int compact_blocks_for(long elements) { return elements >= 1500000L ? kCompactBlocks / 2 : kCompactBlocks; }
void launch_clean_small(const CleanIn& in, Surfels src, Surfels dst, hipStream_t s, int blocks) {
    const CleanArgs a = clean_args(in, src, dst);
    hipLaunchKernelGGL(k_clean_small_flags, dim3(blocks), dim3(256), 0, s, a);
    hipLaunchKernelGGL(k_clean_small_compact, dim3(blocks), dim3(256), 0, s, a);
}
void launch_clean_runs(const CleanIn& in, Surfels buf, const VisList* runs, int* ctl, int blocks, hipStream_t s) {
    CleanArgs a = clean_args(in, buf, buf);
    a.run_list = runs ? runs->list : nullptr; a.run_count = runs ? runs->count : nullptr; a.ctl = ctl;
    hipLaunchKernelGGL(k_clean_runs, dim3(blocks), dim3(256), 0, s, a);
}
void launch_clean_append(const CleanIn& in, Surfels buf, hipStream_t s) {
    CleanArgs a = clean_args(in, buf, buf);
    a.append = 1;
    hipLaunchKernelGGL(k_clean_small_flags, dim3(kCompactBlocks), dim3(256), 0, s, a);
    hipLaunchKernelGGL(k_clean_small_compact, dim3(kCompactBlocks), dim3(256), 0, s, a);
}

__global__ __launch_bounds__(256) void k_obj_index_scatter(const ObjBatch b) {
    const ObjPassArgs& m = b.m[blockIdx.z];
    index_scatter_body(m.a, m.frame, m.pose, b.W, b.H, b.k, b.maxDepthProcessed, b.timeDelta, m.keys, 0, nullptr, nullptr, true);
}
__global__ __launch_bounds__(256) void k_obj_index_resolve(const ObjBatch b) {
    const ObjPassArgs& m = b.m[blockIdx.z];
    index_resolve_same_body<false>(m.a, m.pose, m.keys, b.W * b.H, ResolveOut{m.index, m.ivc, m.inr, nullptr, nullptr, nullptr, nullptr, nullptr, m.frame, nullptr, 0});
}
__global__ __launch_bounds__(256) void k_obj_index_resolve_packed(const ObjBatch b) {
    const ObjPassArgs& m = b.m[blockIdx.z];
    index_resolve_transposing_body<true>(b.updateCopy ? m.b : m.a, m.pose, m.keys, b.W, b.H,
                                         ResolveOut{nullptr, nullptr, nullptr, nullptr, m.iclean, b.depthF, b.mask, b.maskT, m.frame, nullptr, 0}, (int)blockIdx.x);
}
__global__ __launch_bounds__(256) void k_obj_fuse_data(const ObjBatch b) {
    const ObjPassArgs& m = b.m[blockIdx.z];
    const FuseDataArgs a{b.rgb, b.depthRaw, b.depthF, b.mask, m.maskID, m.frame, m.pose, m.weightMultiplier, m.fuseMaxDepth, b.bboxLimit, b.W, b.H, b.k,
                         m.index, m.ivc, m.inr, m.cand_op, m.cand_rec, m.upd_first, m.cand_best};
    fuse_data_body(a);
}
__global__ __launch_bounds__(256) void k_obj_fuse_update(const ObjBatch b) {
    const ObjPassArgs& m = b.m[blockIdx.z];
    fuse_update_body(m.a, m.frame, m.upd_first, m.cand_op, m.cand_best, m.cand_rec, b.W, b.H);
}
__global__ __launch_bounds__(256) void k_obj_fuse_update_copy(const ObjBatch b) {
    const ObjPassArgs& m = b.m[blockIdx.z];
    const IndexScatterArgs ix{m.pose, b.W, b.H, b.k, b.maxDepthProcessed, b.timeDelta, m.keys, 0};
    fuse_update_copy_body(m.a, m.b, m.frame, m.upd_first, m.cand_rec, ix);
}
__device__ __forceinline__ CleanArgs obj_clean_args(const ObjBatch& b, const ObjPassArgs& m, int append) {
    CleanArgs a;
    a.src = b.updateCopy ? m.b : m.a; a.dst = b.updateCopy ? m.a : (b.cleanSmall ? m.b : m.a);
    a.frame = m.frame; a.pose = m.pose; a.W = b.W; a.H = b.H; a.k = b.k; a.timeDelta = b.timeDelta;
    a.confThreshold = m.confThreshold; a.outlierCoeff = b.outlierCoeff; a.maskID = m.maskID; a.transposed = 1; a.literal = b.cleanLiteral;
    a.index = m.index; a.vc = m.ivc; a.ct = nullptr; a.packed = m.iclean; a.depthF = b.depthF; a.mask = b.mask; a.maskT = b.maskT;
    a.cand_op = m.cand_op; a.cand_rec = m.cand_rec; a.flags = m.flags; a.newconf = m.newconf;
    a.block_counts = m.block_counts; a.host_count = m.host_count;
    a.host_append = m.host_append; a.seq = m.clean_seq;
    a.append = append; a.run_list = nullptr; a.run_count = nullptr; a.ctl = m.clean_ctl;
    return a;
}
__global__ __launch_bounds__(256) void k_obj_clean_runs(const ObjBatch b) { clean_runs_body(obj_clean_args(b, b.m[blockIdx.z], 0)); }
__global__ __launch_bounds__(256) void k_obj_clean_small_flags(const ObjBatch b) { clean_small_flags_body(obj_clean_args(b, b.m[blockIdx.z], b.cleanSmall ? 0 : 1)); }
__global__ __launch_bounds__(256) void k_obj_clean_small_compact(const ObjBatch b) { clean_small_compact_body(obj_clean_args(b, b.m[blockIdx.z], b.cleanSmall ? 0 : 1)); }
__global__ __launch_bounds__(256) void k_obj_splat_scatter(const ObjBatch b) {
    const ObjPassArgs& m = b.m[blockIdx.z];
    if (b.denseSprites) splat_scatter_body<1>(m.a, m.frame, m.pose, b.W, b.H, b.k, b.maxDepthProcessed, m.confThreshold, b.timeDelta, m.keys, true);
    else splat_scatter_body<4>(m.a, m.frame, m.pose, b.W, b.H, b.k, b.maxDepthProcessed, m.confThreshold, b.timeDelta, m.keys, true);
}
__global__ __launch_bounds__(256) void k_obj_splat_resolve(const ObjBatch b) {
    const ObjPassArgs& m = b.m[blockIdx.z];
    splat_resolve_body(m.a, m.pose, m.keys, b.W, b.H, b.k, m.predV, m.predN, m.predImage, m.predTime, m.frame, b.rgb, m.predGray, nullptr, 0);
}
__global__ void k_obj_frame_advance(const ObjBatch b) {
    const ObjPassArgs& m = b.m[blockIdx.z];
    frame_advance_body(m.frame, b.W, b.H, m.host_frame, m.pose, b.bg_pose, m.log_slot);
}

void launch_obj_fuse_clean(const ObjBatch& b, int blocks, int clean_blocks, hipStream_t s, int compact_blocks) {
    const int P = b.W * b.H;
    const dim3 surfels(blocks, 1, b.n), pixels((P + 255) / 256, 1, b.n), compact(clean_blocks, 1, b.n);
    const dim3 cands(((b.W + 1) / 2 + 63) / 64, ((b.H + 1) / 2 + 3) / 4, b.n);
    hipLaunchKernelGGL(k_obj_index_scatter, surfels, dim3(256), 0, s, b);
    hipLaunchKernelGGL(k_obj_index_resolve, pixels, dim3(256), 0, s, b);
    hipLaunchKernelGGL(k_obj_fuse_data, cands, dim3(256), 0, s, b);
    if (b.updateCopy) {
        hipLaunchKernelGGL(k_obj_fuse_update_copy, surfels, dim3(256), 0, s, b);
    } else {
        hipLaunchKernelGGL(k_obj_fuse_update, dim3(cand_blocks(b.W, b.H), 1, b.n), dim3(256), 0, s, b);
        hipLaunchKernelGGL(k_obj_index_scatter, surfels, dim3(256), 0, s, b);
    }
    hipLaunchKernelGGL(k_obj_index_resolve_packed, dim3(resolve_tiles(b.W, b.H), 1, b.n), dim3(256), 0, s, b);
    if (!b.cleanSmall) hipLaunchKernelGGL(k_obj_clean_runs, compact, dim3(256), 0, s, b);
    hipLaunchKernelGGL(k_obj_clean_small_flags, dim3(compact_blocks, 1, b.n), dim3(256), 0, s, b);
    hipLaunchKernelGGL(k_obj_clean_small_compact, dim3(compact_blocks, 1, b.n), dim3(256), 0, s, b);
}
void launch_obj_predict_advance(const ObjBatch& b, int blocks, hipStream_t s) {
    hipLaunchKernelGGL(k_obj_splat_scatter, dim3(blocks, 1, b.n), dim3(256), 0, s, b);
    hipLaunchKernelGGL(k_obj_splat_resolve, dim3((b.W + 63) / 64, (b.H + 3) / 4, b.n), dim3(256), 0, s, b);
    hipLaunchKernelGGL(k_obj_frame_advance, dim3(1, 1, b.n), dim3(64), 0, s, b);
}

}
```

Measured before the change: 3335 frames/s.

## Pack clean index into 16-byte texels and spread fuse taps over lane quads

The packed index used by the clean pass shrinks from two float4 per texel to one. Liveness, threshold and current-tick state are folded into the sign or NaN of z, and depth moves to a separate transposed float array, so the clean kernels read less memory per tap. Fuse_data gains a 4-lane mode in which each quad of lanes loads three of the nine neighbour taps, and whole waves exit early when no pixel matches the mask. The encoding adds special-value logic that has to match what the clean kernels expect, and the quad mode computes normals and colour before the validity check.

```diff
diff --git a/maskfusion_amd/api.py b/maskfusion_amd/api.py
--- a/maskfusion_amd/api.py
+++ b/maskfusion_amd/api.py
@@ -395,7 +395,7 @@
         shapes = {"depthF": ((H, W), np.float32), "pred_vertex": ((H, W, 4), np.float32),
                   "pred_normal": ((H, W, 4), np.float32), "pred_image": ((H, W, 4), np.uint8), "pred_time": ((H, W), np.uint16),
                   "index": ((H, W), np.int32), "index_vc": ((H, W, 4), np.float32), "index_nr": ((H, W, 4), np.float32),
-                  "index_ct": ((H, W, 4), np.float32), "index_packed": ((W, H, 2, 4), np.float32), "icp_log": ((19, 32), np.float32), "gn_trace": ((20, 64), np.float64),
+                  "index_ct": ((H, W, 4), np.float32), "index_packed": ((W, H, 2, 4), np.float32),  "icp_log": ((19, 32), np.float32), "gn_trace": ((20, 64), np.float64),
                   "icp_prof": ((19, 16), np.uint64), "splat_prof": ((((H + 15) // 16) * ((W + 15) // 16), 8), np.uint64),
                   "edge_map": ((H, W), np.float32),
                   "edge_binary": ((H, W), np.uint8), "projected_ids": ((H, W), np.uint8)}
@@ -408,6 +408,8 @@
         for pre in ("vmap_g", "nmap_g", "vmap", "nmap"):
             for i in range(3):
                 shapes[f"{pre}{i}"] = ((3, H >> i, W >> i), np.float32)
+        if what == "index_packed" and int(self.getParam("indexPackedTexelBytes")) == 16:
+            shapes[what] = ((W, H, 4), np.float32)
         shape, dt = shapes[what]
         out = np.zeros(shape, dt)
         self._chk(self._L.mf_debug_read_model(self._h, model, what.encode(), out.ctypes.data, out.nbytes))
diff --git a/maskfusion_amd/csrc/mf_context.hip b/maskfusion_amd/csrc/mf_context.hip
--- a/maskfusion_amd/csrc/mf_context.hip
+++ b/maskfusion_amd/csrc/mf_context.hip
@@ -144,6 +144,9 @@
     int W, H, P;
     Intr K;
     hipStream_t stream = nullptr;
+    bool clean_tap16 = true;
+    bool iclean_is_tap16 = false;
+    int fuse_lanes = 4;
     bool clean_literal = true;
     bool global_tiles = true;
     bool early_bg_fusion = true;
@@ -173,6 +176,8 @@
     hipStream_t stream_obj = nullptr, obj_s = nullptr;
     hipEvent_t ev_obj_dep = nullptr, ev_obj_done = nullptr;
     bool obj_dep_main = false;
+    float* d_depthT = nullptr;
+    float* d_depthT_obj = nullptr;
     uint8_t* d_maskT_obj = nullptr;
     bool ftf_rgb = false;
     double host_us[5] = {0, 0, 0, 0, 0}; long host_calls = 0;
@@ -527,6 +532,8 @@
     A(dev_alloc(c, c->allocs, &c->d_iclean, (size_t)P * 2));
     A(dev_alloc(c, c->allocs, &c->d_maskT, (size_t)P));
     A(dev_alloc(c, c->allocs, &c->d_maskT_obj, (size_t)P));
+    A(dev_alloc(c, c->allocs, &c->d_depthT, (size_t)P));
+    A(dev_alloc(c, c->allocs, &c->d_depthT_obj, (size_t)P));
     A(dev_alloc(c, c->allocs, &c->d_inr, (size_t)P));
     A(dev_alloc(c, c->allocs, &c->d_cand_op, (size_t)P));
     A(dev_alloc(c, c->allocs, &c->d_cand_rec, (size_t)P * 3));
@@ -1021,6 +1028,12 @@
         c->vis_tag.model = nullptr;
         return check_launch(c);
     }
+    if (!strcmp(key, "cleanTap16")) { c->clean_tap16 = value != 0; return MF_OK; }
+    if (!strcmp(key, "fuseLanes")) {
+        if ((int)value != 1 && (int)value != 4) { c->err = "fuseLanes: 1 or 4"; return MF_EINVAL; }
+        c->fuse_lanes = (int)value;
+        return MF_OK;
+    }
     if (!strcmp(key, "cleanLiteralWindow")) { c->clean_literal = value != 0; return MF_OK; }
     if (!strcmp(key, "earlyBackgroundFusion")) { c->early_bg_fusion = value != 0; return MF_OK; }
     if (!strcmp(key, "modelApiPackedIndex")) { c->model_api_packed = value != 0; return MF_OK; }
@@ -1050,6 +1063,9 @@
     if (!strcmp(key, "confidenceThreshold")) { *value = c->models[0]->confThr; return MF_OK; }
     if (!strcmp(key, "splatTileEntries")) { *value = c->tile_entries_cap; return MF_OK; }
     if (!strcmp(key, "cullRuns")) { *value = c->cull_runs ? 1 : 0; return MF_OK; }
+    if (!strcmp(key, "cleanTap16")) { *value = c->clean_tap16 ? 1 : 0; return MF_OK; }
+    if (!strcmp(key, "fuseLanes")) { *value = c->fuse_lanes; return MF_OK; }
+    if (!strcmp(key, "indexPackedTexelBytes")) { *value = c->iclean_is_tap16 ? 16 : 32; return MF_OK; }
     if (!strcmp(key, "densifyCount")) { *value = (float)c->densify_count; return MF_OK; }
     if (!strcmp(key, "unstampedRuns")) {
         MF_HIP(c, hipStreamSynchronize(c->stream));
@@ -1151,7 +1167,7 @@
     else if (w == "index_vc") { src = c->d_ivc; bytes = P * 16; }
     else if (w == "index_nr") { src = c->d_inr; bytes = P * 16; }
     else if (w == "index_ct") { src = c->d_ict; bytes = P * 16; }
-    else if (w == "index_packed") { src = c->d_iclean; bytes = P * 32; }
+    else if (w == "index_packed") { src = c->d_iclean; bytes = c->iclean_is_tap16 ? P * 16 : P * 32; variable = true; }
     else if (w == "cand_op") { src = c->d_cand_op; bytes = P; variable = true; }
     else if (w == "cand_rec") { src = c->d_cand_rec; bytes = P * 48; variable = true; }
     else if (w == "clean_flags") { src = c->d_flags; bytes = (size_t)c->cap_max + P; variable = true; }
diff --git a/maskfusion_amd/csrc/mf_internal.h b/maskfusion_amd/csrc/mf_internal.h
--- a/maskfusion_amd/csrc/mf_internal.h
+++ b/maskfusion_amd/csrc/mf_internal.h
@@ -206,11 +206,13 @@
 void launch_index_resolve(Surfels src, const FrameDev* frame, const PoseDev* pose, unsigned long long* keys, int W, int H, int* index,
                           float4* vc, float4* nr, float4* ct , float4* packed ,
                           const float* depthF, const uint8_t* mask, uint8_t* maskT ,
-                          bool keys_transposed , hipStream_t s, int* decay_stats = nullptr, int maskID = 0);
+                          bool keys_transposed , hipStream_t s, int* decay_stats = nullptr, int maskID = 0,
+                          float* depthT = nullptr , float tapThreshold = 0.f);
 void launch_fuse_data(const uint8_t* rgb, const float* depthRaw, const float* depthF, const uint8_t* mask,
                       int maskID, const FrameDev* frame, const PoseDev* pose, float weightMultiplier, float maxDepth,
                       int W, int H, Intr k, const int* index, const float4* vc, const float4* nr, uint8_t* cand_op,
-                      float4* cand_rec, int* upd_first, int* cand_best, hipStream_t s, int bboxLimit = 1);
+                      float4* cand_rec, int* upd_first, int* cand_best, hipStream_t s, int bboxLimit = 1,
+                      int lanes = 4 );
 void launch_fuse_update(Surfels s, const FrameDev* frame, int* upd_first, const uint8_t* cand_op, const int* cand_best, const float4* cand_rec,
                         int W, int H, hipStream_t st);
 void launch_fuse_update_copy(Surfels src, Surfels dst, const FrameDev* frame, int* upd_first, const float4* cand_rec, const PoseDev* pose,
@@ -220,6 +222,7 @@
     FrameDev* frame; const PoseDev* pose; int W, H; Intr k; int timeDelta; float confThreshold, outlierCoeff; int maskID;
     const int* index; const float4* vc; const float4* ct;
     const float4* packed; const uint8_t* maskT;
+    const float* depthT = nullptr;
     const float* depthF; const uint8_t* mask;
     const uint8_t* cand_op; const float4* cand_rec;
     uint8_t* flags; float* newconf; int* block_counts;
@@ -284,6 +287,8 @@
     int cleanSmall;
     const uint8_t* rgb; const float* depthRaw; const float* depthF; const uint8_t* mask; const PoseDev* bg_pose;
     uint8_t* maskT;
+    float* depthT;
+    int fuseLanes;
     unsigned long long* global_keys;
 };
 void launch_obj_global_scatter(const ObjBatch& b, int blocks, hipStream_t s);
diff --git a/maskfusion_amd/csrc/mf_surfel.hip b/maskfusion_amd/csrc/mf_surfel.hip
--- a/maskfusion_amd/csrc/mf_surfel.hip
+++ b/maskfusion_amd/csrc/mf_surfel.hip
@@ -308,11 +308,18 @@
 }
 
 struct ResolvedTexel { int index; float4 vc, nr, ct, p0, p1; };
+struct Tap16 { float thr, time; };
+__device__ __forceinline__ float4 tap16_encode(float3 h, float conf, float initTime, float lastTime, int id, Tap16 t) {
+    const bool live = id > 0 && conf > t.thr && h.z > 0;
+    return make_float4(h.x, h.y, live ? (lastTime == t.time ? -h.z : h.z) : __int_as_float(0x7fc00000), initTime);
+}
 template <bool kPacked>
-__device__ __forceinline__ ResolvedTexel resolve_texel(const Surfels& src, const PoseDev* __restrict__ pose, unsigned long long key, bool want_ct, int first) {
+__device__ __forceinline__ ResolvedTexel resolve_texel(const Surfels& src, const PoseDev* __restrict__ pose, unsigned long long key, bool want_ct, int first,
+                                                       const Tap16* tap16 = nullptr) {
     ResolvedTexel r;
     r.index = 0;
     r.vc = r.nr = r.ct = r.p0 = r.p1 = make_float4(0, 0, 0, 0);
+    if (kPacked && tap16) r.p0.z = __int_as_float(0x7fc00000);
     if (key == kEmptyKey) return r;
     const int i = (int)(unsigned)(key & 0xFFFFFFFFull);
     const int id = i == first ? 0 : i;
@@ -320,7 +327,7 @@
     const float3 h = mul33(pose->Ri, f3(pc.x, pc.y, pc.z)) + f3(pose->ti[0], pose->ti[1], pose->ti[2]);
     if (kPacked) {
         const float4 c4 = src.ct[i];
-        r.p0 = make_float4(h.x, h.y, h.z, pc.w);
+        r.p0 = tap16 ? tap16_encode(h, pc.w, c4.z, c4.w, id, *tap16) : make_float4(h.x, h.y, h.z, pc.w);
         r.p1 = make_float4(c4.z, c4.w, __int_as_float(id), 0.f);
     } else {
         const float4 n4 = src.nr[i];
@@ -334,6 +341,7 @@
 }
 struct ResolveOut {
     int* index; float4* vc; float4* nr; float4* ct; float4* packed; const float* depthF; const uint8_t* mask; uint8_t* maskT;
+    float* depthT; float tapThreshold;
     const FrameDev* frame;
     int* decay_stats; int maskID;
 };
@@ -377,13 +385,15 @@
     {
         const int lx = kPacked ? f : g, ly = kPacked ? g : f;
         const int x = x0 + lx, y = y0 + ly;
-        ResolvedTexel r = resolve_texel<kPacked>(src, pose, kEmptyKey, false, 0);
+        const Tap16 t16{o.tapThreshold, (float)o.frame->tick};
+        const Tap16* tap = (kPacked && o.depthT) ? &t16 : nullptr;
+        ResolvedTexel r = resolve_texel<kPacked>(src, pose, kEmptyKey, false, 0, tap);
         int mk = 0;
         if (x < W && y < H) {
             const int p = kPacked ? y * W + x : x * H + y;
             const unsigned long long key = keys[p];
             keys[p] = kEmptyKey;
-            r = resolve_texel<kPacked>(src, pose, key, o.ct != nullptr, o.frame->first);
+            r = resolve_texel<kPacked>(src, pose, key, o.ct != nullptr, o.frame->first, tap);
             if (kPacked) { r.p1.w = o.depthF[p]; mk = o.mask[p]; s_mk[lx][ly] = (uint8_t)mk; }
         }
         if (kPacked) decay_stats_add(o, x < W && y < H, x, y, W, H, r.p1.w, mk);
@@ -397,8 +407,8 @@
         if (x < W && y < H) {
             if (kPacked) {
                 const int tp = x * H + y;
-                o.packed[2 * tp] = s_a[lx][ly];
-                o.packed[2 * tp + 1] = s_b[lx][ly];
+                if (o.depthT) { o.packed[tp] = s_a[lx][ly]; o.depthT[tp] = s_b[lx][ly].w; }
+                else { o.packed[2 * tp] = s_a[lx][ly]; o.packed[2 * tp + 1] = s_b[lx][ly]; }
                 o.maskT[tp] = s_mk[lx][ly];
             } else {
                 const int p = y * W + x;
@@ -428,10 +438,11 @@
         const int tp = x * H + y;
         const unsigned long long key = keys[tp];
         keys[tp] = kEmptyKey;
-        ResolvedTexel r = resolve_texel<true>(src, pose, key, false, o.frame->first);
+        const Tap16 t16{o.tapThreshold, (float)o.frame->tick};
+        ResolvedTexel r = resolve_texel<true>(src, pose, key, false, o.frame->first, o.depthT ? &t16 : nullptr);
         r.p1.w = s_d[g][f];
-        o.packed[2 * tp] = r.p0;
-        o.packed[2 * tp + 1] = r.p1;
+        if (o.depthT) { o.packed[tp] = r.p0; o.depthT[tp] = r.p1.w; }
+        else { o.packed[2 * tp] = r.p0; o.packed[2 * tp + 1] = r.p1; }
         o.maskT[tp] = s_mk[g][f];
     }
 }
@@ -451,9 +462,9 @@
 
 void launch_index_resolve(Surfels src, const FrameDev* frame, const PoseDev* pose, unsigned long long* keys, int W, int H, int* index, float4* vc,
                           float4* nr, float4* ct, float4* packed, const float* depthF, const uint8_t* mask, uint8_t* maskT, bool keys_transposed,
-                          hipStream_t s, int* decay_stats, int maskID) {
+                          hipStream_t s, int* decay_stats, int maskID, float* depthT, float tapThreshold) {
     const int P = W * H;
-    const ResolveOut o{index, vc, nr, ct, packed, depthF, mask, maskT, frame, packed ? decay_stats : nullptr, maskID};
+    const ResolveOut o{index, vc, nr, ct, packed, depthF, mask, maskT, packed ? depthT : nullptr, tapThreshold, frame, packed ? decay_stats : nullptr, maskID};
     const dim3 flat((P + 255) / 256), tiles(resolve_tiles(W, H));
     if (packed) {
         if (keys_transposed) hipLaunchKernelGGL(k_index_resolve_packed, tiles, dim3(256), 0, s, src, pose, keys, W, H, o);
@@ -474,12 +485,16 @@
     int* cand_best;
 };
 
+template <int kLanes>
 __device__ __forceinline__ void fuse_data_body(const FuseDataArgs& a) {
+    static_assert(kLanes == 1 || kLanes == 4, "one lane or a quad per candidate");
+    constexpr int kPerWave = 64 / kLanes, kTaps = kLanes == 1 ? 9 : 3;
     const int time = a.frame->tick;
     const int par = time & 1;
     const int W = a.W, H = a.H;
     const int nxc = (W - par + 1) / 2, nyc = (H - par + 1) / 2;
-    const int xi = blockIdx.x * 64 + (threadIdx.x & 63);
+    const int ql = (int)threadIdx.x & (kLanes - 1);
+    const int xi = blockIdx.x * kPerWave + ((threadIdx.x & 63) / kLanes);
     const int yi = blockIdx.y * 4 + (threadIdx.x >> 6);
     if (xi >= nxc || yi >= nyc) return;
     const int c = xi * nyc + yi;
@@ -487,6 +502,23 @@
     const Intr k = a.k;
     uint8_t op = 0;
     const float x = (float)px + 0.5f, y = (float)py + 0.5f;
+    int cur9[kTaps]; float4 vc9[kTaps], nr9[kTaps];
+    if (kLanes == 4 && a.maskID != 0) {
+        if (__ballot(a.mask[py * W + px] == a.maskID) == 0ull) {
+            if (ql == 0) a.cand_op[c] = 0;
+            return;
+        }
+    }
+    if (kLanes == 4) {
+#pragma unroll
+        for (int j = 0; j < kTaps; ++j) {
+            const int da = min(ql, 2) - 1, db = j - 1;
+            const int tp = clampi(py + db, 0, H - 1) * W + clampi(px + da, 0, W - 1);
+            cur9[j] = a.index[tp];
+            vc9[j] = a.vc[tp];
+            nr9[j] = a.nr[tp];
+        }
+    }
     const float3 vLocal = get_vertex(a.depthRaw, W, H, px, py, x, y, k);
     bool valid = a.mask[py * W + px] == a.maskID;
     valid = valid && !(texf(a.depthRaw, W, H, px - 1, py) == 0 || texf(a.depthRaw, W, H, px, py - 1) == 0 ||
@@ -504,37 +536,49 @@
         }
     }
     valid = valid && (vLocal.z > 0 && vLocal.z <= maxDepth);
+    float bestDist = 1000;
+    int best = 0;
+    bool merge = false;
+    float3 vGlobal = f3(0, 0, 0), nGlobal = vGlobal, vF = vGlobal, nLocal = vGlobal;
+    float weighting = 0.f, colour = 0.f;
+    if (kLanes == 4) {
+        vF = get_vertex(a.depthF, W, H, px, py, x, y, k);
+        nLocal = get_normal_central(a.depthF, W, H, px, py, x, y, vF, k);
+        const uint8_t* pc = a.rgb + (size_t)(py * W + px) * 3;
+        colour = (float)((pc[0] << 16) + (pc[1] << 8) + pc[2]);
+    }
     if (valid) {
         float R[9];
 #pragma unroll
         for (int q = 0; q < 9; ++q) R[q] = a.pose->R[q];
         const float3 t = f3(a.pose->t[0], a.pose->t[1], a.pose->t[2]);
-        const float3 vGlobal = mul33(R, vLocal) + t;
-        const float3 vF = get_vertex(a.depthF, W, H, px, py, x, y, k);
-        const float3 nLocal = get_normal_central(a.depthF, W, H, px, py, x, y, vF, k);
-        const float3 nGlobal = mul33(R, nLocal);
-        const uint8_t* pc = a.rgb + (size_t)(py * W + px) * 3;
-        const float weighting = a.pose->fusionWeight * a.weightMultiplier;
+        vGlobal = mul33(R, vLocal) + t;
+        if (kLanes == 1) {
+            vF = get_vertex(a.depthF, W, H, px, py, x, y, k);
+            nLocal = get_normal_central(a.depthF, W, H, px, py, x, y, vF, k);
+            const uint8_t* pc = a.rgb + (size_t)(py * W + px) * 3;
+            colour = (float)((pc[0] << 16) + (pc[1] << 8) + pc[2]);
+        }
+        nGlobal = mul33(R, nLocal);
+        weighting = a.pose->fusionWeight * a.weightMultiplier;
 
         const float xl = (x - k.cx) * (1.0f / k.fx), yl = (y - k.cy) * (1.0f / k.fy);
         const float lambda = sqrtf(xl * xl + yl * yl + 1);
         const float3 ray = f3(xl, yl, 1);
-        float bestDist = 1000;
-        int best = 0;
-        bool merge = false;
-        int cur9[9]; float4 vc9[9], nr9[9];
-#pragma unroll
-        for (int q = 0; q < 9; ++q) {
-            const int da = q / 3 - 1, db = q % 3 - 1;
-            const int tp = clampi(py + db, 0, H - 1) * W + clampi(px + da, 0, W - 1);
-            cur9[q] = a.index[tp];
-            vc9[q] = a.vc[tp];
-            nr9[q] = a.nr[tp];
-        }
-#pragma unroll
-        for (int q = 0; q < 9; ++q) {
+        if (kLanes == 1) {
+#pragma unroll
+            for (int q = 0; q < kTaps; ++q) {
+                const int da = q / 3 - 1, db = q % 3 - 1;
+                const int tp = clampi(py + db, 0, H - 1) * W + clampi(px + da, 0, W - 1);
+                cur9[q] = a.index[tp];
+                vc9[q] = a.vc[tp];
+                nr9[q] = a.nr[tp];
+            }
+        }
+#pragma unroll
+        for (int q = 0; q < kTaps; ++q) {
             const int current = cur9[q];
-            if (current > 0) {
+            if (current > 0 && ql < 3) {
                 const float4 vc = vc9[q];
                 const float zdiff = vc.z - vLocal.z;
                 if (fabsf(zdiff * lambda) < 0.05f) {
@@ -548,9 +592,23 @@
                 }
             }
         }
+    }
+    if (kLanes == 4) {
+        const float myDist = bestDist;
+        const int myBest = best;
+        bestDist = 1000; best = 0; merge = false;
+#pragma unroll
+        for (int l = 0; l < 3; ++l) {
+            const float d = __shfl(myDist, l, 4);
+            const int b = __shfl(myBest, l, 4);
+            if (d < bestDist) { merge = true; bestDist = d; best = b; }
+        }
+        if (ql != 0) return;
+    }
+    if (valid) {
         op = merge ? 1 : 2;
         a.cand_rec[c * 3 + 0] = make_float4(vGlobal.x, vGlobal.y, vGlobal.z, surfel_confidence(x, y, weighting, k));
-        a.cand_rec[c * 3 + 1] = make_float4((float)((pc[0] << 16) + (pc[1] << 8) + pc[2]), 0.f, (float)time, merge ? -1.f : -2.f);
+        a.cand_rec[c * 3 + 1] = make_float4(colour, 0.f, (float)time, merge ? -1.f : -2.f);
         a.cand_rec[c * 3 + 2] = make_float4(nGlobal.x, nGlobal.y, nGlobal.z, surfel_radius(vF.z, nLocal.z, k));
         if (merge) {
             atomicMin(&a.upd_first[best], c);
@@ -560,16 +618,19 @@
     a.cand_op[c] = op;
 }
 
-__global__ __launch_bounds__(256) void k_fuse_data(const FuseDataArgs a) { fuse_data_body(a); }
+template <int kLanes>
+__global__ __launch_bounds__(256) void k_fuse_data(const FuseDataArgs a) { fuse_data_body<kLanes>(a); }
 
 void launch_fuse_data(const uint8_t* rgb, const float* depthRaw, const float* depthF, const uint8_t* mask, int maskID,
                       const FrameDev* frame, const PoseDev* pose, float weightMultiplier, float maxDepth, int W, int H, Intr k,
                       const int* index, const float4* vc, const float4* nr, uint8_t* cand_op, float4* cand_rec, int* upd_first,
-                      int* cand_best, hipStream_t s, int bboxLimit) {
+                      int* cand_best, hipStream_t s, int bboxLimit, int lanes) {
     FuseDataArgs a{rgb, depthRaw, depthF, mask, maskID, frame, pose, weightMultiplier, maxDepth, bboxLimit, W, H, k,
                    index, vc, nr, cand_op, cand_rec, upd_first, cand_best};
-    dim3 grid(((W + 1) / 2 + 63) / 64, ((H + 1) / 2 + 3) / 4);
-    hipLaunchKernelGGL(k_fuse_data, grid, dim3(256), 0, s, a);
+    const int per_wave = lanes == 4 ? 16 : 64;
+    dim3 grid(((W + 1) / 2 + per_wave - 1) / per_wave, ((H + 1) / 2 + 3) / 4);
+    if (lanes == 4) hipLaunchKernelGGL(k_fuse_data<4>, grid, dim3(256), 0, s, a);
+    else hipLaunchKernelGGL(k_fuse_data<1>, grid, dim3(256), 0, s, a);
 }
 
 __device__ __forceinline__ void surfel_merge(float4& pc, float4& ct, float4& nr, float4 mp, float4 mc, float4 mn, float time) {
@@ -671,6 +732,7 @@
     const float4* packed;
     const float* depthF; const uint8_t* mask;
     const uint8_t* maskT;
+    const float* depthT;
     const uint8_t* cand_op; const float4* cand_rec;
     uint8_t* flags; float* newconf;
     int* block_counts;
@@ -700,6 +762,7 @@
     }
 }
 
+template <bool kTap16>
 __device__ __forceinline__ bool clean_test(const CleanArgs& a, float4 pc, float4 ct, float4 nr, float time, const float* Ri,
                                            float3 ti, float& newconf, int& decay, const float4* nr_lazy = nullptr) {
     const int W = a.W, H = a.H;
@@ -733,7 +796,14 @@
                 if (mult <= 0) continue;
                 float4 v, c;
                 int idx;
-                if (a.packed) {
+                bool upd = false;
+                if (kTap16) {
+                    const float4 t = a.packed[tp];
+                    idx = isnan(t.z) ? 0 : 1;
+                    upd = __float_as_int(t.z) < 0;
+                    v = make_float4(t.x, t.y, fabsf(t.z), 0.f);
+                    c = make_float4(0.f, 0.f, t.w, 0.f);
+                } else if (a.packed) {
                     v = a.packed[2 * tp];
                     const float4 r1 = a.packed[2 * tp + 1];
                     c = make_float4(0.f, 0.f, r1.x, r1.y);
@@ -745,10 +815,10 @@
                 }
                 if (idx > 0) {
                     const float dx = v.x - lp.x, dy = v.y - lp.y;
-                    if (c.z < ct.z && v.w > a.confThreshold && v.z > lp.z && v.z - lp.z < 0.01f &&
+                    if (c.z < ct.z && (kTap16 || v.w > a.confThreshold) && v.z > lp.z && v.z - lp.z < 0.01f &&
                         sqrtf(dx * dx + dy * dy) < nr.w * 1.4f)
                         count += mult;
-                    if (c.w == time && v.w > a.confThreshold && v.z > lp.z && v.z - lp.z > 0.01f && fabsf(ln.z) > 0.85f)
+                    if ((kTap16 ? upd : c.w == time) && (kTap16 || v.w > a.confThreshold) && v.z > lp.z && v.z - lp.z > 0.01f && fabsf(ln.z) > 0.85f)
                         zCount += mult;
                 }
             }
@@ -761,7 +831,7 @@
     if (w > 0 && time - w > (float)a.timeDelta) test = true;
     const int fx_ = isnan(x) ? 0 : clampi((int)fminf(fmaxf(floorf(x), -1.f), (float)W), 0, W - 1);
     const int fy_ = isnan(y) ? 0 : clampi((int)fminf(fmaxf(floorf(y), -1.f), (float)H), 0, H - 1);
-    const float wDepth = a.packed ? a.packed[2 * (fx_ * H + fy_) + 1].w : a.depthF[fy_ * W + fx_];
+    const float wDepth = kTap16 ? a.depthT[fx_ * H + fy_] : a.packed ? a.packed[2 * (fx_ * H + fy_) + 1].w : a.depthF[fy_ * W + fx_];
     const int maskValue = a.packed ? a.maskT[fx_ * H + fy_] : a.mask[fy_ * W + fx_];
     newconf = pc.w;
     decay = 0;
@@ -780,6 +850,7 @@
     return conf;
 }
 
+template <bool kTap16>
 __device__ __forceinline__ void clean_small_flags_body(const CleanArgs& a) {
     __shared__ int s_w[4];
     const int count = a.append ? a.frame->phys : a.frame->count;
@@ -799,11 +870,11 @@
         float nc = 0.f;
         int dk = 0;
         if (i < count) {
-            keep = clean_test(a, a.src.pc[i], a.src.ct[i], a.src.nr[i], time, Ri, ti, nc, dk);
+            keep = clean_test<kTap16>(a, a.src.pc[i], a.src.ct[i], make_float4(0, 0, 0, 0), time, Ri, ti, nc, dk, &a.src.nr[i]);
         } else {
             const int c = i - count;
             if (a.cand_op[c] == 2)
-                keep = clean_test(a, a.cand_rec[c * 3 + 0], a.cand_rec[c * 3 + 1], a.cand_rec[c * 3 + 2], time, Ri, ti, nc, dk);
+                keep = clean_test<kTap16>(a, a.cand_rec[c * 3 + 0], a.cand_rec[c * 3 + 1], make_float4(0, 0, 0, 0), time, Ri, ti, nc, dk, &a.cand_rec[c * 3 + 2]);
         }
         a.flags[i - first] = keep ? 1 : 0;
         a.newconf[i - first] = nc;
@@ -829,7 +900,8 @@
     }
 }
 
-__global__ __launch_bounds__(256) void k_clean_small_flags(const CleanArgs a) { clean_small_flags_body(a); }
+template <bool kTap16>
+__global__ __launch_bounds__(256) void k_clean_small_flags(const CleanArgs a) { clean_small_flags_body<kTap16>(a); }
 
 __device__ __forceinline__ void clean_small_compact_body(const CleanArgs& a) {
     __shared__ int s_w[4];
@@ -998,6 +1070,7 @@
                        count, ctl);
 }
 
+template <bool kTap16>
 __device__ __forceinline__ void clean_runs_body(const CleanArgs& a) {
     __shared__ int s_cnt[2][4];
     __shared__ int s_red[4][kRunRed];
@@ -1025,8 +1098,8 @@
         if (live1) { pc1 = a.src.pc[start + off1]; tm1 = *reinterpret_cast<const float2*>(reinterpret_cast<const float*>(&a.src.ct[start + off1]) + 2); }
         float nc0 = 0.f, nc1 = 0.f;
         int dk = 0;
-        const bool keep0 = live0 && clean_test(a, pc0, make_float4(0.f, 0.f, tm0.x, tm0.y), make_float4(0, 0, 0, 0), time, Ri, ti, nc0, dk, &a.src.nr[start + off0]);
-        const bool keep1 = live1 && clean_test(a, pc1, make_float4(0.f, 0.f, tm1.x, tm1.y), make_float4(0, 0, 0, 0), time, Ri, ti, nc1, dk, &a.src.nr[start + off1]);
+        const bool keep0 = live0 && clean_test<kTap16>(a, pc0, make_float4(0.f, 0.f, tm0.x, tm0.y), make_float4(0, 0, 0, 0), time, Ri, ti, nc0, dk, &a.src.nr[start + off0]);
+        const bool keep1 = live1 && clean_test<kTap16>(a, pc1, make_float4(0.f, 0.f, tm1.x, tm1.y), make_float4(0, 0, 0, 0), time, Ri, ti, nc1, dk, &a.src.nr[start + off1]);
         RunAcc acc;
         acc.reset();
         const bool st0 = keep0 && tm0.y == -2.f, st1 = keep1 && tm1.y == -2.f;
@@ -1116,7 +1189,8 @@
     }
 }
 
-__global__ __launch_bounds__(256) void k_clean_runs(const CleanArgs a) { clean_runs_body(a); }
+template <bool kTap16>
+__global__ __launch_bounds__(256) void k_clean_runs(const CleanArgs a) { clean_runs_body<kTap16>(a); }
 
 int clean_runs_grid(long elements) {
     const long runs = (elements + kRun - 1) / kRun;
@@ -1331,7 +1405,7 @@
     a.literal = in.literalWindow ? 1 : 0;
     a.src = src; a.dst = dst; a.frame = in.frame; a.pose = in.pose; a.W = in.W; a.H = in.H; a.k = in.k; a.timeDelta = in.timeDelta;
     a.confThreshold = in.confThreshold; a.outlierCoeff = in.outlierCoeff; a.maskID = in.maskID; a.index = in.index; a.vc = in.vc; a.ct = in.ct;
-    a.packed = in.packed;
+    a.packed = in.packed; a.depthT = in.packed ? in.depthT : nullptr;
     a.depthF = in.depthF; a.mask = in.mask; a.maskT = in.maskT; a.cand_op = in.cand_op; a.cand_rec = in.cand_rec;
     a.flags = in.flags; a.newconf = in.newconf; a.block_counts = in.block_counts; a.host_count = in.host_count;
     a.host_append = in.host_append; a.seq = in.seq;
@@ -1341,18 +1415,21 @@
 int compact_blocks_for(long elements) { return elements >= 1500000L ? kCompactBlocks / 2 : kCompactBlocks; }
 void launch_clean_small(const CleanIn& in, Surfels src, Surfels dst, hipStream_t s, int blocks) {
     const CleanArgs a = clean_args(in, src, dst);
-    hipLaunchKernelGGL(k_clean_small_flags, dim3(blocks), dim3(256), 0, s, a);
+    if (a.depthT) hipLaunchKernelGGL(k_clean_small_flags<true>, dim3(blocks), dim3(256), 0, s, a);
+    else hipLaunchKernelGGL(k_clean_small_flags<false>, dim3(blocks), dim3(256), 0, s, a);
     hipLaunchKernelGGL(k_clean_small_compact, dim3(blocks), dim3(256), 0, s, a);
 }
 void launch_clean_runs(const CleanIn& in, Surfels buf, const VisList* runs, int* ctl, int blocks, hipStream_t s) {
     CleanArgs a = clean_args(in, buf, buf);
     a.run_list = runs ? runs->list : nullptr; a.run_count = runs ? runs->count : nullptr; a.ctl = ctl;
-    hipLaunchKernelGGL(k_clean_runs, dim3(blocks), dim3(256), 0, s, a);
+    if (a.depthT) hipLaunchKernelGGL(k_clean_runs<true>, dim3(blocks), dim3(256), 0, s, a);
+    else hipLaunchKernelGGL(k_clean_runs<false>, dim3(blocks), dim3(256), 0, s, a);
 }
 void launch_clean_append(const CleanIn& in, Surfels buf, hipStream_t s) {
     CleanArgs a = clean_args(in, buf, buf);
     a.append = 1;
-    hipLaunchKernelGGL(k_clean_small_flags, dim3(kCompactBlocks), dim3(256), 0, s, a);
+    if (a.depthT) hipLaunchKernelGGL(k_clean_small_flags<true>, dim3(kCompactBlocks), dim3(256), 0, s, a);
+    else hipLaunchKernelGGL(k_clean_small_flags<false>, dim3(kCompactBlocks), dim3(256), 0, s, a);
     hipLaunchKernelGGL(k_clean_small_compact, dim3(kCompactBlocks), dim3(256), 0, s, a);
 }
 
@@ -1362,18 +1439,19 @@
 }
 __global__ __launch_bounds__(256) void k_obj_index_resolve(const ObjBatch b) {
     const ObjPassArgs& m = b.m[blockIdx.z];
-    index_resolve_same_body<false>(m.a, m.pose, m.keys, b.W * b.H, ResolveOut{m.index, m.ivc, m.inr, nullptr, nullptr, nullptr, nullptr, nullptr, m.frame, nullptr, 0});
+    index_resolve_same_body<false>(m.a, m.pose, m.keys, b.W * b.H, ResolveOut{m.index, m.ivc, m.inr, nullptr, nullptr, nullptr, nullptr, nullptr, nullptr, 0.f, m.frame, nullptr, 0});
 }
 __global__ __launch_bounds__(256) void k_obj_index_resolve_packed(const ObjBatch b) {
     const ObjPassArgs& m = b.m[blockIdx.z];
     index_resolve_transposing_body<true>(b.updateCopy ? m.b : m.a, m.pose, m.keys, b.W, b.H,
-                                         ResolveOut{nullptr, nullptr, nullptr, nullptr, m.iclean, b.depthF, b.mask, b.maskT, m.frame, nullptr, 0}, (int)blockIdx.x);
-}
+                                         ResolveOut{nullptr, nullptr, nullptr, nullptr, m.iclean, b.depthF, b.mask, b.maskT, b.depthT, m.confThreshold, m.frame, nullptr, 0}, (int)blockIdx.x);
+}
+template <int kLanes>
 __global__ __launch_bounds__(256) void k_obj_fuse_data(const ObjBatch b) {
     const ObjPassArgs& m = b.m[blockIdx.z];
     const FuseDataArgs a{b.rgb, b.depthRaw, b.depthF, b.mask, m.maskID, m.frame, m.pose, m.weightMultiplier, m.fuseMaxDepth, b.bboxLimit, b.W, b.H, b.k,
                          m.index, m.ivc, m.inr, m.cand_op, m.cand_rec, m.upd_first, m.cand_best};
-    fuse_data_body(a);
+    fuse_data_body<kLanes>(a);
 }
 __global__ __launch_bounds__(256) void k_obj_fuse_update(const ObjBatch b) {
     const ObjPassArgs& m = b.m[blockIdx.z];
@@ -1389,15 +1467,17 @@
     a.src = b.updateCopy ? m.b : m.a; a.dst = b.updateCopy ? m.a : (b.cleanSmall ? m.b : m.a);
     a.frame = m.frame; a.pose = m.pose; a.W = b.W; a.H = b.H; a.k = b.k; a.timeDelta = b.timeDelta;
     a.confThreshold = m.confThreshold; a.outlierCoeff = b.outlierCoeff; a.maskID = m.maskID; a.transposed = 1; a.literal = b.cleanLiteral;
-    a.index = m.index; a.vc = m.ivc; a.ct = nullptr; a.packed = m.iclean; a.depthF = b.depthF; a.mask = b.mask; a.maskT = b.maskT;
+    a.index = m.index; a.vc = m.ivc; a.ct = nullptr; a.packed = m.iclean; a.depthT = b.depthT; a.depthF = b.depthF; a.mask = b.mask; a.maskT = b.maskT;
     a.cand_op = m.cand_op; a.cand_rec = m.cand_rec; a.flags = m.flags; a.newconf = m.newconf;
     a.block_counts = m.block_counts; a.host_count = m.host_count;
     a.host_append = m.host_append; a.seq = m.clean_seq;
     a.append = append; a.run_list = nullptr; a.run_count = nullptr; a.ctl = m.clean_ctl;
     return a;
 }
-__global__ __launch_bounds__(256) void k_obj_clean_runs(const ObjBatch b) { clean_runs_body(obj_clean_args(b, b.m[blockIdx.z], 0)); }
-__global__ __launch_bounds__(256) void k_obj_clean_small_flags(const ObjBatch b) { clean_small_flags_body(obj_clean_args(b, b.m[blockIdx.z], b.cleanSmall ? 0 : 1)); }
+template <bool kTap16>
+__global__ __launch_bounds__(256) void k_obj_clean_runs(const ObjBatch b) { clean_runs_body<kTap16>(obj_clean_args(b, b.m[blockIdx.z], 0)); }
+template <bool kTap16>
+__global__ __launch_bounds__(256) void k_obj_clean_small_flags(const ObjBatch b) { clean_small_flags_body<kTap16>(obj_clean_args(b, b.m[blockIdx.z], b.cleanSmall ? 0 : 1)); }
 __global__ __launch_bounds__(256) void k_obj_clean_small_compact(const ObjBatch b) { clean_small_compact_body(obj_clean_args(b, b.m[blockIdx.z], b.cleanSmall ? 0 : 1)); }
 __global__ __launch_bounds__(256) void k_obj_splat_scatter(const ObjBatch b) {
     const ObjPassArgs& m = b.m[blockIdx.z];
@@ -1416,10 +1496,12 @@
 void launch_obj_fuse_clean(const ObjBatch& b, int blocks, int clean_blocks, hipStream_t s, int compact_blocks) {
     const int P = b.W * b.H;
     const dim3 surfels(blocks, 1, b.n), pixels((P + 255) / 256, 1, b.n), compact(clean_blocks, 1, b.n);
-    const dim3 cands(((b.W + 1) / 2 + 63) / 64, ((b.H + 1) / 2 + 3) / 4, b.n);
+    const int per_wave = b.fuseLanes == 4 ? 16 : 64;
+    const dim3 cands(((b.W + 1) / 2 + per_wave - 1) / per_wave, ((b.H + 1) / 2 + 3) / 4, b.n);
     hipLaunchKernelGGL(k_obj_index_scatter, surfels, dim3(256), 0, s, b);
     hipLaunchKernelGGL(k_obj_index_resolve, pixels, dim3(256), 0, s, b);
-    hipLaunchKernelGGL(k_obj_fuse_data, cands, dim3(256), 0, s, b);
+    if (b.fuseLanes == 4) hipLaunchKernelGGL(k_obj_fuse_data<4>, cands, dim3(256), 0, s, b);
+    else hipLaunchKernelGGL(k_obj_fuse_data<1>, cands, dim3(256), 0, s, b);
     if (b.updateCopy) {
         hipLaunchKernelGGL(k_obj_fuse_update_copy, surfels, dim3(256), 0, s, b);
     } else {
@@ -1427,8 +1509,13 @@
         hipLaunchKernelGGL(k_obj_index_scatter, surfels, dim3(256), 0, s, b);
     }
     hipLaunchKernelGGL(k_obj_index_resolve_packed, dim3(resolve_tiles(b.W, b.H), 1, b.n), dim3(256), 0, s, b);
-    if (!b.cleanSmall) hipLaunchKernelGGL(k_obj_clean_runs, compact, dim3(256), 0, s, b);
-    hipLaunchKernelGGL(k_obj_clean_small_flags, dim3(compact_blocks, 1, b.n), dim3(256), 0, s, b);
+    if (b.depthT) {
+        if (!b.cleanSmall) hipLaunchKernelGGL(k_obj_clean_runs<true>, compact, dim3(256), 0, s, b);
+        hipLaunchKernelGGL(k_obj_clean_small_flags<true>, dim3(compact_blocks, 1, b.n), dim3(256), 0, s, b);
+    } else {
+        if (!b.cleanSmall) hipLaunchKernelGGL(k_obj_clean_runs<false>, compact, dim3(256), 0, s, b);
+        hipLaunchKernelGGL(k_obj_clean_small_flags<false>, dim3(compact_blocks, 1, b.n), dim3(256), 0, s, b);
+    }
     hipLaunchKernelGGL(k_obj_clean_small_compact, dim3(compact_blocks, 1, b.n), dim3(256), 0, s, b);
 }
 void launch_obj_predict_advance(const ObjBatch& b, int blocks, hipStream_t s) {
```

Measured after the change: 3446 frames/s (median of 6 runs). +3.3%, better.
